# obeychoi0120/wseg

Measured on AMD Instinct MI355X. Metric: training images/sec at B=16x448x448 (contrast_train step), higher is better.
Workload: dtype bf16; 1 GPU; ResNet-38 contrast, synthetic VOC 448x448, B=16/GPU, procedural weights, dropout on, fused HIP loss; global_batch=16, parallelism=dp1, seed=0

## Files before the change

include/wseg_hip.h:

```cpp
#ifndef WSEG_HIP_H
#define WSEG_HIP_H
#include <stddef.h>
#include <stdint.h>
#ifdef __cplusplus
extern "C" {
#endif

#define WSEG_F32 0
#define WSEG_BF16 1
#define WSEG_F32X3 2

int wseg_version(void);
size_t wseg_sizeof_conv_desc(void);
size_t wseg_sizeof_wgrad_desc(void);
const char* wseg_last_error(void);

typedef struct wseg_conv_desc {
  const void* in;  const void* w;  void* out;  void* out2;
  const void* r_pre;  const void* r_post;  const void* mask;
  const float* scale;  const float* shift;  const float* drop;
  int32_t N, IH, IW, IC, ld_in;
  int32_t OH, OW, OC, ld_out, ld_out2;
  int32_t ld_rpre, ld_rpost, ld_mask;
  int32_t KH, KW, stride, dil, pad;
  int32_t mode, epi, dtype;
  int32_t relu_out2;
  int32_t relu_lt;
  int32_t bm_hint;
  int32_t IH2, IW2, OH2, OW2;
  const void* in2;
  int32_t ld_in2, IC2;
  int32_t w_rows;
} wseg_conv_desc;
int wseg_conv_igemm(const wseg_conv_desc* d, void* stream);

typedef struct wseg_wgrad_desc {
  const void* x;  const void* dy;  float* dw;
  int32_t N, IH, IW, IC, ld_x;
  int32_t OH, OW, OC, ld_dy;
  int32_t KH, KW, stride, dil, pad;
  int32_t dtype, split_k;
  int32_t IC_dw, OC_dw;
  int32_t tile_hint;
  int32_t IH2, IW2, OH2, OW2;
  int32_t dw_rot;
} wseg_wgrad_desc;
int wseg_conv_wgrad(const wseg_wgrad_desc* d, void* stream);

#define WSEG_CONV_64x128 1
#define WSEG_CONV_128x128 2
#define WSEG_CONV_224x256 3
#define WSEG_CONV_256x256 4
#define WSEG_CONV_512x128 5
#define WSEG_WGRAD_128x128 6
#define WSEG_WGRAD_256x256 7
typedef struct wseg_launch_plan {
  int32_t family;
  int32_t tile_rows, tile_cols;
  int32_t nwg;
  int32_t perm;
  int32_t tapf;
  int32_t nsplit;
  int32_t unit;
} wseg_launch_plan;
int wseg_conv_plan(const wseg_conv_desc* d, wseg_launch_plan* out);
int wseg_wgrad_plan(const wseg_wgrad_desc* d, wseg_launch_plan* out);

int wseg_conv_bwd_pair(const wseg_conv_desc* dg, const wseg_wgrad_desc* wg, void* stream);
int wseg_conv_bwd_pair_plan(const wseg_conv_desc* dg, const wseg_wgrad_desc* wg, wseg_launch_plan* dg_plan, wseg_launch_plan* wg_plan);

int wseg_pack_weights(const float* master, void* fwd, void* tr, int OC, int T, int IC,
                      int OCp, int ICp, int ic_rot, int dtype, void* stream);
int wseg_copy2d_batch(const void* src, void* dst, const long* table, int npieces, long total_chunks, void* stream);
int wseg_pack_transposed_batch(const float* master, void* out, const long* table, int nlayers, long total_tiles, int dtype, void* stream);
int wseg_pack_transposed_batch_bf16(const void* mirror, void* out, const long* table, int nlayers, long total_tiles, void* stream);
int wseg_dropout_scale(const float* u, float* out, long total, long split_at, float p0, float p1, void* stream);

int wseg_stem_conv(const float* x_nchw, const float* w ,
                   const float* scale, const float* shift, void* raw, void* act,
                   int N, int H, int W, int dtype, void* stream);
int wseg_stem_conv_kc(const float* x, const float* w_kc, const float* scale, const float* shift,
                      void* raw, void* act, int N, int H, int W, int dtype, void* stream);

int wseg_head_split(const void* head, int ld, int c0, float* cam_low, float* cmax, int N, int hw, int dtype, void* stream);
int wseg_cam_gate(const float* cam_low, const float* cmax, float* G, int N, int hw, void* stream);
int wseg_pcm_xs(const float* x_nchw, void* feat, int ld, int c_xs, int c_end, int N, int H, int W, int h, int w, int dtype, void* stream);
int wseg_head_grad_rows(const float* d_fproj, const float* d_cam_low, const void* head, void* d_head, int ld, int N, int hw, int dtype, void* stream);

int wseg_resize_planar_fwd(const float* in, float* out, const float* plane_mul, long planes, int ih, int iw, int oh, int ow, int align,
                           int flip_x, int accumulate, void* stream);
int wseg_resize_planar_bwd(const float* d_out, float* d_in, const float* plane_mul, const float* plane_add, long planes, int ih, int iw, int oh, int ow, int align, int accumulate, void* stream);

int wseg_infer_finish(const float* sum_cam, const float* stats, float alpha, float* norm_cam, unsigned char* pred, int npix, void* stream);

int wseg_l2norm_forward(const void* F, int ldf, float* Fh, float* nrm, long rows, int dtype, void* stream);
int wseg_l2norm_backward(const void* F, int ldf, const float* dFh, const float* nrm, void* dF, int lddf, long rows, int dtype, void* stream);
int wseg_pcm_forward(const float* Fh, const float* G, float* cam_rv, float* den, int N, int hw, void* stream);
int wseg_pcm_backward(const float* Fh, const float* G, const float* d_cam_rv, const float* cam_rv, const float* den,
                      float* DN, float* dFh, int N, int hw, void* stream);
int wseg_pack_x3(const float* src, void* dst, long numel, void* stream);
int wseg_split_bf16(const float* in, void* hi, void* lo, long total, void* stream);
int wseg_to_bf16(const float* in, void* out, long total, void* stream);
int wseg_pcm_forward_bf16(const void* Fb, const void* Gb, float* cam_rv, float* den, int N, int hw, void* stream);
int wseg_pcm_backward_bf16(const void* Fb, const void* Gb, const void* Gl, const float* d_cam_rv, const float* cam_rv, const float* den,
                           float* DN, void* DNb, void* DNl, float* dFh, int N, int hw, void* stream);

size_t wseg_plane_stats_workspace_bytes(long planes);
int wseg_plane_stats(const float* U, float* stats, long planes, int npix, void* workspace, void* stream);
int wseg_up_plane_stats(const float* low, float* stats, long planes, int h, int w, int S, const float* label20 , void* workspace, void* stream);
int wseg_up_rvmin_values(const float* low, const float* label20, float* q, unsigned char* argc, int N, int h, int w, int S, void* stream);
int wseg_up_norm_resize_forward(const float* low, const float* stats, const float* label20, float* out, int N, int h, int w, int S, int OS, void* stream);
int wseg_resize_adjoint_ones(float* wvec, int h, int S, void* stream);
int wseg_up_maps_backward(const float* G, const float* low, const float* stats, const float* label20, const float* plane_bias,
                          const float* wvec_y, const float* wvec_x, const float* q, const unsigned char* argc, const float* res,
                          int k, float coef, float* d_low, int N, int h, int w, int S, int OS, void* stream);
int wseg_cls_loss(const float* stats, const float* label20, float* loss_out, float* plane_bias, int N, int npix, float coef, void* stream);
size_t wseg_select_workspace_bytes(int rows);
int wseg_select_kth(const float* vals, int rows, int n, int k, int largest, int use_abs, int relu_vals, float* res, void* workspace, void* stream);
int wseg_select_finish(const float* res, int rows, int k, int relu_vals, float scale, float* loss_out, void* stream);
int wseg_loss_finish(const float* acc, float er_coef, float* out8, void* stream);
int wseg_er_ecr_prep(const float* c1, const float* c2, const float* r1, const float* r2, float* Gc1, float* Gc2, float* dlt1, float* dlt2,
                     float* er_sum, int N, int npix, float er_coef, void* stream);
int wseg_ecr_backward(const float* dlt, const float* res, float* Gr, int N, int per_row, int k, float coef, void* stream);
int wseg_rows_resize_forward(const void* head, int ld, float* F, int N, int ih, int iw, int oh, int ow, int dtype, void* stream);
int wseg_head_grad_fused(const float* dF, const float* d_cam_low, const void* head, void* d_head, int ld, int N, int ih, int iw, int oh, int ow, int dtype, void* stream);
int wseg_pseudo_label(const float* R, const float* label20, float bg_thr, int* y, float* ncam, int N, int npix, void* stream);
int wseg_proto_candidates(const float* ncam, const float* F, const int* tie_idx, float* cand_val, float* cand_feat, int* cand_const, int N, int npix, int K, void* stream);
int wseg_proto_merge(const float* cand_val, const float* cand_feat, const int* cand_const, float* protos, int world, int K,
                     long rank_stride , void* stream);
int wseg_intra_weights(const int* y, const float* S_own, int ld_s, const float* rkey, const unsigned char* rand_flag, float* w, int P, void* stream);
int wseg_intra_weights_global(const float* rec, float* w, int P, int ranks, int own_rank, float scale, long rank_stride, void* stream);

typedef struct {
  const float* F;
  const float* p_own;
  const float* p_oth;
  const int32_t* y_own;
  const int32_t* y_oth;
  const float* w_intra;
  const float* rkey;
  float* rec;
  float* dF;
} wseg_nce_view;
int wseg_nce_records(const wseg_nce_view* views, int nviews, int P, int split_bf16, void* stream);
int wseg_nce_fused(const wseg_nce_view* views, int nviews, int P, float coef_cross, float coef_intra, float* sums , void* stream);

typedef struct {
  const uint8_t* src; int32_t H, W;
  int32_t rh, rw;
  const int32_t* xb; const int32_t* xk; int32_t xks;
  const int32_t* yb; const int32_t* yk; int32_t yks;
  uint8_t* tmp; uint8_t* img;
  int32_t flip;
  int32_t op[4];
  float factor[4];
  int32_t hue_shift;
  int32_t cont_top, cont_left, img_top, img_left, ch, cw;
  float* out;
} wseg_aug_desc;
size_t wseg_sizeof_aug_desc(void);
int wseg_augment_batch(const wseg_aug_desc* descs_dev, int n, int max_pixels , const float* lut ,
                       int crop, unsigned long long* lum_sums , void* stream);

int wseg_sgd_step(float* params, const float* grads, float* momentum_buf, long numel,
                  const long* seg_begin, const long* seg_end, const float* seg_lr, const float* seg_wd, int nseg,
                  float momentum, float grad_scale, int first_step, void* bf16_mirror, void* stream);

#define WSEG_AFF_MAX_OFFSETS 64
#define WSEG_RW_MAX_PLANE 8192
int wseg_aff_num_offsets(int radius);
int wseg_aff_pairs(const void* feat, int ld, int C, float* aff, int N, int h, int w, int radius, int dtype, void* stream);
int wseg_aff_to_dense(const float* aff, float* dense, int h, int w, int radius, void* stream);
int wseg_rw_prepare(const float* aff, float* wgt, float* rsum, int N, int h, int w, int radius, int beta, void* stream);
int wseg_random_walk(const float* wgt, const float* rsum, const float* v_in, float* v_out, int N, int planes, int h, int w, int radius,
                     int logt, void* stream);
int wseg_rw_pool(const float* cams, const int* src, float bg, float* pooled, int H, int W, int dh, int dw, void* stream);
int wseg_rw_finish(const float* cam_rw, unsigned char* pred, int planes, int dh, int dw, int H, int W, void* stream);

long wseg_aff_loss_workspace_bytes(int N, int h, int w, int radius);
int wseg_aff_loss_forward(const void* feat, int ld, int C, const unsigned char* label, float* aff, void* workspace, float* out7, int N,
                          int h, int w, int radius, int dtype, void* stream);
int wseg_aff_loss_backward(const void* feat, int ld, int C, const unsigned char* label, const float* aff, const float* out7,
                           const float* gscale, float* d_feat, int ld_d, int N, int h, int w, int radius, int dtype, void* stream);

int wseg_elu_backward_rows(const void* g, int ld_g, int g_dtype, const void* y, int ld_y, int y_dtype, const float* gscale, void* dz,
                           int ld_dz, int dz_dtype, long M, int C, void* stream);

#define WSEG_CRF_PIX_ALIGN 128
#define WSEG_CRF_MAX_LABELS 32
#define WSEG_CRF_MAX_COLUMNS 64
#define WSEG_CRF_MAX_RADIUS 128
#define WSEG_CRF_BG_CONST 0
#define WSEG_CRF_BG_POWER 1
int wseg_crf_padded_pixels(int npix);
int wseg_crf_columns(int S, int n_labels);
int wseg_crf_labels(const float* cams, const int* src, int n_labels, int rule, float param, unsigned char* labels, int npix, void* stream);
int wseg_crf_prepare(const unsigned char* img, int H, int W, float gauss_sxy, float* feat, float* ones, float* ng, void* stream);
int wseg_crf_bilateral(const float* feat, const float* Qn, float* out, int npix, int ncols, float sxy, float srgb, void* stream);
int wseg_crf_rsqrt(const float* sums, int stride, float* n, int npix, void* stream);
int wseg_crf_gaussian(const float* in, float* tmp, float* out, int planes, int H, int W, float sxy, void* stream);
int wseg_crf_update(const unsigned char* labels, const float* outb, const float* outg, const float* nb, const float* ng, float* Qn,
                    float* Qg, float* Qout, float* logits, unsigned char* amax, int S, int n_labels, int npix, float gt_prob,
                    float w_bilateral, float w_gaussian, void* stream);

#ifdef __cplusplus
}
#endif
#endif
```

wseg_amd/_lib.py:

```python
import contextlib
import ctypes as C
import os

import torch

_HERE = os.path.dirname(os.path.abspath(__file__))
LIB_PATH = os.environ.get("WSEG_LIB") or os.path.join(_HERE, "libwseg_hip.so")

F32, BF16, F32X3 = 0, 1, 2
PROFILE_WGRAD = None
PROFILE = None
PROFILE_STRIDE = 1
_profile_idx = 0
_profile_phase = 0


def profile_begin_step(step):
    global _profile_idx, _profile_phase
    _profile_idx, _profile_phase = 0, step % max(1, PROFILE_STRIDE)


def _profile_sample():
    global _profile_idx
    i = _profile_idx
    _profile_idx += 1
    return (i + _profile_phase) % max(1, PROFILE_STRIDE) == 0, i
TORCH_DTYPE = {F32: torch.float32, BF16: torch.bfloat16, F32X3: torch.float32}


class ConvDesc(C.Structure):
    _fields_ = [("inp", C.c_void_p), ("w", C.c_void_p), ("out", C.c_void_p), ("out2", C.c_void_p),
                ("r_pre", C.c_void_p), ("r_post", C.c_void_p), ("mask", C.c_void_p),
                ("scale", C.c_void_p), ("shift", C.c_void_p), ("drop", C.c_void_p),
                ("N", C.c_int32), ("IH", C.c_int32), ("IW", C.c_int32), ("IC", C.c_int32), ("ld_in", C.c_int32),
                ("OH", C.c_int32), ("OW", C.c_int32), ("OC", C.c_int32), ("ld_out", C.c_int32), ("ld_out2", C.c_int32),
                ("ld_rpre", C.c_int32), ("ld_rpost", C.c_int32), ("ld_mask", C.c_int32),
                ("KH", C.c_int32), ("KW", C.c_int32), ("stride", C.c_int32), ("dil", C.c_int32), ("pad", C.c_int32),
                ("mode", C.c_int32), ("epi", C.c_int32), ("dtype", C.c_int32), ("relu_out2", C.c_int32),
                ("relu_lt", C.c_int32), ("bm_hint", C.c_int32),
                ("IH2", C.c_int32), ("IW2", C.c_int32), ("OH2", C.c_int32), ("OW2", C.c_int32),
                ("in2", C.c_void_p), ("ld_in2", C.c_int32), ("IC2", C.c_int32), ("w_rows", C.c_int32)]


class WgradDesc(C.Structure):
    _fields_ = [("x", C.c_void_p), ("dy", C.c_void_p), ("dw", C.c_void_p),
                ("N", C.c_int32), ("IH", C.c_int32), ("IW", C.c_int32), ("IC", C.c_int32), ("ld_x", C.c_int32),
                ("OH", C.c_int32), ("OW", C.c_int32), ("OC", C.c_int32), ("ld_dy", C.c_int32),
                ("KH", C.c_int32), ("KW", C.c_int32), ("stride", C.c_int32), ("dil", C.c_int32), ("pad", C.c_int32),
                ("dtype", C.c_int32), ("split_k", C.c_int32), ("IC_dw", C.c_int32), ("OC_dw", C.c_int32),
                ("tile_hint", C.c_int32),
                ("IH2", C.c_int32), ("IW2", C.c_int32), ("OH2", C.c_int32), ("OW2", C.c_int32), ("dw_rot", C.c_int32)]


def _load():
    if not os.path.exists(LIB_PATH):
        raise ImportError(
            f"{LIB_PATH} not found: build it with `python -c 'import __graft_entry__ as g; g.build()'` "
            "(wseg_amd has no CPU/eager fallback)")
    lib = C.CDLL(LIB_PATH)
    lib.wseg_last_error.restype = C.c_char_p
    lib.wseg_version.restype = C.c_int
    for fn in ("wseg_sizeof_conv_desc", "wseg_sizeof_wgrad_desc", "wseg_select_workspace_bytes", "wseg_plane_stats_workspace_bytes"):
        getattr(lib, fn).restype = C.c_size_t
    if lib.wseg_sizeof_conv_desc() != C.sizeof(ConvDesc) or lib.wseg_sizeof_wgrad_desc() != C.sizeof(WgradDesc):
        raise ImportError(f"{LIB_PATH} was built from another include/wseg_hip.h (descriptor sizes "
                          f"{lib.wseg_sizeof_conv_desc()}/{lib.wseg_sizeof_wgrad_desc()} vs {C.sizeof(ConvDesc)}/{C.sizeof(WgradDesc)}): rebuild it")
    return lib


lib = _load()


def _ptr(t):
    return t.data_ptr() if torch.is_tensor(t) else t


def stream_ptr():
    return torch.cuda.current_stream().cuda_stream


def check(status, what):
    if status != 0:
        raise RuntimeError(f"{what} failed ({status}): {lib.wseg_last_error().decode()}")


def _v(x):
    return C.c_void_p(_ptr(x))


def _s():
    return C.c_void_p(stream_ptr())


def _f(x):
    return C.c_float(x)


def _call(name, *args):
    check(getattr(lib, name)(*args, _s()), name)


def dtype_code(t):
    if t.dtype == torch.float32:
        return F32
    if t.dtype == torch.bfloat16:
        return BF16
    raise TypeError(f"unsupported dtype {t.dtype}")


def _flops_label(kind, *, N, IH, IW, IC, OH, OW, OC, KH, KW, stride=1, dil=1, seg2=None, mode=0, IC2=None, **_):
    oh, ow = (OH, OW) if mode == 0 else (IH, IW)
    pix = N * oh * ow
    if seg2 is not None:
        pix += N * (seg2[2] * seg2[3] if mode == 0 else seg2[0] * seg2[1])
    kin = IC * KH * KW + (IC2 or 0)
    return 2.0 * pix * kin * OC, f"{kind} {IC}{('+%d' % IC2) if IC2 else ''}->{OC} k{KH} s{stride} d{dil} {OH}x{OW}"


@contextlib.contextmanager
def _timed(sink, entry):
    if sink is None:
        yield
        return
    ev0, ev1 = torch.cuda.Event(enable_timing=True), torch.cuda.Event(enable_timing=True)
    ev0.record()
    yield
    ev1.record()
    sink.append((ev0, ev1) + tuple(entry()))


def conv_igemm(inp, w, out=None, out2=None, *, pair_wgrad=None, **kw):
    d = _conv_desc(inp, w, out, out2, **kw)
    ic2 = (d.IC2 or d.IC) if d.in2 else 0
    krow, wrows = d.KH * d.KW * d.IC + ic2, max(d.OC, d.w_rows)
    if w.numel() < wrows * krow:
        raise RuntimeError(f"conv_igemm: weight buffer has {w.numel()} elements, the launch reads {wrows} x {krow}")
    sampled, launch_idx = _profile_sample() if PROFILE is not None else (False, 0)

    def entry():
        kind = "fwd" if d.mode == 0 else ("dgrad+wgrad" if pair_wgrad is not None else "dgrad")
        flops, label = _flops_label(kind, **{**kw, "IC2": ic2})
        wflops = _flops_label("wgrad", **pair_wgrad[3])[0] if pair_wgrad is not None else 0.0
        return flops + wflops, label, launch_idx

    with _timed(PROFILE if sampled else None, entry):
        if pair_wgrad is not None:
            wx, wdy, wdw, wkw = pair_wgrad
            _call("wseg_conv_bwd_pair", C.byref(d), C.byref(_wgrad_desc(wx, wdy, wdw, **wkw)))
        else:
            _call("wseg_conv_igemm", C.byref(d))


def _conv_desc(inp, w, out, out2, *, N, IH, IW, IC, OH, OW, OC, KH, KW, stride=1, dil=1, pad=0,
               mode=0, epi=0, r_pre=None, r_post=None, mask=None, scale=None, shift=None, drop=None,
               ld_in=None, ld_out=None, ld_out2=None, ld_rpre=None, ld_rpost=None, ld_mask=None, relu_out2=1,
               relu_lt=0, bm_hint=0, seg2=None, in2=None, ld_in2=None, IC2=0, dtype=None, w_rows=0):
    d = ConvDesc()
    d.inp, d.w, d.out, d.out2 = _ptr(inp), _ptr(w), _ptr(out), _ptr(out2)
    d.r_pre, d.r_post, d.mask = _ptr(r_pre), _ptr(r_post), _ptr(mask)
    d.scale, d.shift, d.drop = _ptr(scale), _ptr(shift), _ptr(drop)
    d.N, d.IH, d.IW, d.IC, d.ld_in = N, IH, IW, IC, ld_in or IC
    d.OH, d.OW, d.OC, d.ld_out, d.ld_out2 = OH, OW, OC, ld_out or OC, ld_out2 or OC
    d.ld_rpre, d.ld_rpost, d.ld_mask = ld_rpre or OC, ld_rpost or OC, ld_mask or OC
    d.KH, d.KW, d.stride, d.dil, d.pad = KH, KW, stride, dil, pad
    d.mode, d.epi, d.dtype, d.relu_out2, d.relu_lt, d.bm_hint = mode, epi, (dtype_code(inp) if dtype is None else dtype), relu_out2, relu_lt, bm_hint
    if seg2 is not None:
        d.IH2, d.IW2, d.OH2, d.OW2 = seg2
    ic2 = (IC2 or IC) if in2 is not None else 0
    if in2 is not None:
        d.in2, d.IC2, d.ld_in2 = _ptr(in2), IC2, ld_in2 or ic2
    d.w_rows = w_rows
    return d


def _wgrad_desc(x, dy, dw, *, N, IH, IW, IC, OH, OW, OC, KH, KW, stride=1, dil=1, pad=0,
                ld_x=None, ld_dy=None, split_k=0, IC_dw=None, OC_dw=None, tile_hint=0, seg2=None, dtype=None, dw_rot=0):
    d = WgradDesc()
    d.x, d.dy, d.dw = _ptr(x), _ptr(dy), _ptr(dw)
    d.N, d.IH, d.IW, d.IC, d.ld_x = N, IH, IW, IC, ld_x or IC
    d.OH, d.OW, d.OC, d.ld_dy = OH, OW, OC, ld_dy or OC
    d.KH, d.KW, d.stride, d.dil, d.pad = KH, KW, stride, dil, pad
    d.dtype, d.split_k = (dtype_code(x) if dtype is None else dtype), split_k
    d.IC_dw, d.OC_dw, d.tile_hint = IC_dw or IC, OC_dw or OC, tile_hint
    d.dw_rot = dw_rot
    if seg2 is not None:
        d.IH2, d.IW2, d.OH2, d.OW2 = seg2
    assert not torch.is_tensor(dw) or dw.dtype == torch.float32
    return d


def conv_wgrad(x, dy, dw, **kw):
    d = _wgrad_desc(x, dy, dw, **kw)
    with _timed(PROFILE_WGRAD, lambda: _flops_label("wgrad", **kw)):
        _call("wseg_conv_wgrad", C.byref(d))


CONV_64x128, CONV_128x128, CONV_224x256, CONV_256x256, CONV_512x128, WGRAD_128x128, WGRAD_256x256 = range(1, 8)
_ANY = 64


class LaunchPlan(C.Structure):
    _fields_ = [(k, C.c_int32) for k in ("family", "tile_rows", "tile_cols", "nwg", "perm", "tapf", "nsplit", "unit")]

    def __repr__(self):
        return "LaunchPlan(" + ", ".join(f"{k}={getattr(self, k)}" for k, _t in self._fields_) + ")"


def _plan_dtype(t, dtype):
    return dtype if dtype is not None else (dtype_code(t) if torch.is_tensor(t) else BF16)


def conv_plan(inp=_ANY, w=_ANY, out=_ANY, out2=None, *, dtype=None, **kw):
    plan = LaunchPlan()
    check(lib.wseg_conv_plan(C.byref(_conv_desc(inp, w, out, out2, dtype=_plan_dtype(inp, dtype), **kw)), C.byref(plan)), "wseg_conv_plan")
    return plan


def wgrad_plan(x=_ANY, dy=_ANY, dw=_ANY, *, dtype=None, **kw):
    plan = LaunchPlan()
    check(lib.wseg_wgrad_plan(C.byref(_wgrad_desc(x, dy, dw, dtype=_plan_dtype(x, dtype), **kw)), C.byref(plan)), "wseg_wgrad_plan")
    return plan


def conv_pair_plan(wgrad_kw, inp=_ANY, w=_ANY, out=_ANY, out2=None, *, dtype=None, **kw):
    dg, wg = LaunchPlan(), LaunchPlan()
    dtype = _plan_dtype(inp, dtype)
    wdtype = dtype if wgrad_kw.get("dtype") is None else wgrad_kw["dtype"]
    fused = lib.wseg_conv_bwd_pair_plan(C.byref(_conv_desc(inp, w, out, out2, dtype=dtype, **kw)),
                                        C.byref(_wgrad_desc(_ANY, _ANY, _ANY, **{**wgrad_kw, "dtype": wdtype})), C.byref(dg), C.byref(wg))
    if fused < 0:
        check(fused, "wseg_conv_bwd_pair_plan")
    return fused, dg, wg


def pack_weights(master, fwd, tr, OC, T, IC, OCp, ICp, dtype, ic_rot=0):
    _call("wseg_pack_weights", _v(master), _v(fwd), _v(tr), OC, T, IC, OCp, ICp, ic_rot, dtype)


def copy2d_batch(src, dst, table, npieces, total_chunks):
    _call("wseg_copy2d_batch", _v(src), _v(dst), _v(table), npieces, C.c_long(total_chunks))


def pack_transposed_batch(master, out, table, nlayers, total_tiles, dtype):
    _call("wseg_pack_transposed_batch", _v(master), _v(out), _v(table), nlayers, C.c_long(total_tiles), dtype)


def pack_transposed_batch_bf16(mirror, out, table, nlayers, total_tiles):
    _call("wseg_pack_transposed_batch_bf16", _v(mirror), _v(out), _v(table), nlayers, C.c_long(total_tiles))


def dropout_scale(u, out, split_at, p0, p1):
    _call("wseg_dropout_scale", _v(u), _v(out), C.c_long(u.numel()), C.c_long(split_at), _f(p0), _f(p1))


def stem_conv_kc(x, w_kc, scale, shift, raw, act, N, H, W, dtype):
    if w_kc.numel() != 27 * 64 or w_kc.dtype != torch.float32:
        raise RuntimeError("stem_conv_kc: weights must be f32 [27][64]")
    _call("wseg_stem_conv_kc", _v(x), _v(w_kc), _v(scale), _v(shift), _v(raw), _v(act), N, H, W, dtype)


def stem_conv(x, w, scale, shift, raw, act, N, H, W, dtype):
    _call("wseg_stem_conv", _v(x), _v(w), _v(scale), _v(shift), _v(raw), _v(act), N, H, W, dtype)


def head_split(head, ld, c0, cam_low, cmax, N, hw):
    check(lib.wseg_head_split(_v(head), ld, c0, _v(cam_low), _v(cmax), N, hw, dtype_code(head), _s()), "wseg_head_split")


def cam_gate(cam_low, cmax, G, N, hw):
    check(lib.wseg_cam_gate(_v(cam_low), _v(cmax), _v(G), N, hw, _s()), "wseg_cam_gate")


def pcm_xs(x, feat, ld, c_xs, c_end, N, H, W, h, w):
    check(lib.wseg_pcm_xs(_v(x), _v(feat), ld, c_xs, c_end, N, H, W, h, w, dtype_code(feat), _s()), "wseg_pcm_xs")


def head_grad_rows(d_fproj, d_cam_low, head, d_head, ld, N, hw):
    check(lib.wseg_head_grad_rows(_v(d_fproj), _v(d_cam_low), _v(head), _v(d_head), ld, N, hw, dtype_code(head), _s()), "wseg_head_grad_rows")


def resize_planar_fwd(inp, out, planes, ih, iw, oh, ow, align, plane_mul=None, flip_x=False, accumulate=False):
    check(lib.wseg_resize_planar_fwd(_v(inp), _v(out), _v(plane_mul), C.c_long(planes), ih, iw, oh, ow, int(align), int(flip_x), int(accumulate), _s()), "wseg_resize_planar_fwd")


def infer_finish(sum_cam, stats, alpha, norm_cam, pred, npix):
    check(lib.wseg_infer_finish(_v(sum_cam), _v(stats), C.c_float(alpha), _v(norm_cam), _v(pred), npix, _s()), "wseg_infer_finish")


def resize_planar_bwd(d_out, d_in, planes, ih, iw, oh, ow, align, accumulate=False, plane_mul=None, plane_add=None):
    check(lib.wseg_resize_planar_bwd(_v(d_out), _v(d_in), _v(plane_mul), _v(plane_add), C.c_long(planes), ih, iw, oh, ow, int(align), int(accumulate), _s()), "wseg_resize_planar_bwd")


def l2norm_forward(F, ldf, Fh, nrm, rows):
    check(lib.wseg_l2norm_forward(_v(F), ldf, _v(Fh), _v(nrm), C.c_long(rows), dtype_code(F), _s()), "wseg_l2norm_forward")


def l2norm_backward(F, ldf, dFh, nrm, dF, lddf, rows):
    check(lib.wseg_l2norm_backward(_v(F), ldf, _v(dFh), _v(nrm), _v(dF), lddf, C.c_long(rows), dtype_code(F), _s()), "wseg_l2norm_backward")


def pcm_forward(Fh, G, cam_rv, den, N, hw):
    check(lib.wseg_pcm_forward(_v(Fh), _v(G), _v(cam_rv), _v(den), N, hw, _s()), "wseg_pcm_forward")


def pcm_backward(Fh, G, d_cam_rv, cam_rv, den, DN, dFh, N, hw):
    check(lib.wseg_pcm_backward(_v(Fh), _v(G), _v(d_cam_rv), _v(cam_rv), _v(den), _v(DN), _v(dFh), N, hw, _s()), "wseg_pcm_backward")


def sgd_step(params, grads, buf, segs, momentum, grad_scale, first_step, bf16_mirror=None):
    n = len(segs)
    LongArr, FloatArr = C.c_long * n, C.c_float * n
    b = LongArr(*[s[0] for s in segs]); e = LongArr(*[s[1] for s in segs])
    lr = FloatArr(*[s[2] for s in segs]); wd = FloatArr(*[s[3] for s in segs])
    check(lib.wseg_sgd_step(_v(params), _v(grads), _v(buf), C.c_long(params.numel()), b, e, lr, wd, n,
                            C.c_float(momentum), C.c_float(grad_scale), int(first_step), _v(bf16_mirror), _s()), "wseg_sgd_step")


def plane_stats(U, stats, planes, npix):
    ws = torch.empty(int(lib.wseg_plane_stats_workspace_bytes(C.c_long(planes))), device=U.device, dtype=torch.uint8)
    _call("wseg_plane_stats", _v(U), _v(stats), C.c_long(planes), npix, _v(ws))
def cls_loss(stats, label20, loss_out, plane_bias, N, npix, coef): _call("wseg_cls_loss", _v(stats), _v(label20), _v(loss_out), _v(plane_bias), N, npix, _f(coef))
def select_workspace_bytes(rows): return int(lib.wseg_select_workspace_bytes(rows))
def select_kth(vals, rows, n, k, largest, use_abs, relu_vals, res, ws): _call("wseg_select_kth", _v(vals), rows, n, k, int(largest), int(use_abs), int(relu_vals), _v(res), _v(ws))
def loss_finish(acc, er_coef, out8): _call("wseg_loss_finish", _v(acc), _f(er_coef), _v(out8))
def select_finish(res, rows, k, relu_vals, scale, loss_out): _call("wseg_select_finish", _v(res), rows, k, int(relu_vals), _f(scale), _v(loss_out))
def er_ecr_prep(c1, c2, r1, r2, Gc1, Gc2, dlt1, dlt2, er_sum, N, npix, er_coef): _call("wseg_er_ecr_prep", _v(c1), _v(c2), _v(r1), _v(r2), _v(Gc1), _v(Gc2), _v(dlt1), _v(dlt2), _v(er_sum), N, npix, _f(er_coef))
def ecr_backward(dlt, res, Gr, N, per_row, k, coef): _call("wseg_ecr_backward", _v(dlt), _v(res), _v(Gr), N, per_row, k, _f(coef))
def rows_resize_forward(head, ld, F, N, ih, iw, oh, ow): _call("wseg_rows_resize_forward", _v(head), ld, _v(F), N, ih, iw, oh, ow, dtype_code(head))
def head_grad_fused(dF, d_cam_low, head, d_head, ld, N, ih, iw, oh, ow): _call("wseg_head_grad_fused", _v(dF), _v(d_cam_low), _v(head), _v(d_head), ld, N, ih, iw, oh, ow, dtype_code(head))
def pseudo_label(R, label20, bg_thr, y, ncam, N, npix): _call("wseg_pseudo_label", _v(R), _v(label20), _f(bg_thr), _v(y), _v(ncam), N, npix)
def proto_candidates(ncam, F, tie_idx, cand_val, cand_feat, cand_const, N, npix, K): _call("wseg_proto_candidates", _v(ncam), _v(F), _v(tie_idx), _v(cand_val), _v(cand_feat), _v(cand_const), N, npix, K)
def proto_merge(cand_val, cand_feat, cand_const, protos, world, K, rank_stride=0): _call("wseg_proto_merge", _v(cand_val), _v(cand_feat), _v(cand_const), _v(protos), world, K, C.c_long(rank_stride))
def intra_weights(y, S_own, rkey, rand_flag, w, P, ld_s=21): _call("wseg_intra_weights", _v(y), _v(S_own), ld_s, _v(rkey), _v(rand_flag), _v(w), P)
def intra_weights_global(rec, w, P, ranks, own_rank, scale, rank_stride): _call("wseg_intra_weights_global", _v(rec), _v(w), P, ranks, own_rank, _f(scale), C.c_long(rank_stride))


class NceView(C.Structure):
    _fields_ = [("F", C.c_void_p), ("p_own", C.c_void_p), ("p_oth", C.c_void_p), ("y_own", C.c_void_p), ("y_oth", C.c_void_p),
                ("w_intra", C.c_void_p), ("rkey", C.c_void_p), ("rec", C.c_void_p), ("dF", C.c_void_p)]


def _nce_views(views):
    arr = (NceView * len(views))()
    for i, v in enumerate(views):
        for k, _t in NceView._fields_:
            setattr(arr[i], k, _ptr(v.get(k)))
    return arr


def nce_records(views, P, split_bf16=False):
    _call("wseg_nce_records", _nce_views(views), len(views), P, int(split_bf16))


def nce_fused(views, P, coef_cross, coef_intra, sums):
    _call("wseg_nce_fused", _nce_views(views), len(views), P, _f(coef_cross), _f(coef_intra), _v(sums))


def up_plane_stats(low, stats, planes, h, w, S, label20=None):
    ws = torch.empty(int(lib.wseg_plane_stats_workspace_bytes(C.c_long(planes))), device=low.device, dtype=torch.uint8)
    _call("wseg_up_plane_stats", _v(low), _v(stats), C.c_long(planes), h, w, S, _v(label20), _v(ws))
def up_rvmin_values(low, label20, q, argc, N, h, w, S): _call("wseg_up_rvmin_values", _v(low), _v(label20), _v(q), _v(argc), N, h, w, S)
def up_norm_resize_forward(low, stats, label20, out, N, h, w, S, OS): _call("wseg_up_norm_resize_forward", _v(low), _v(stats), _v(label20), _v(out), N, h, w, S, OS)
def resize_adjoint_ones(wvec, h, S): _call("wseg_resize_adjoint_ones", _v(wvec), h, S)
def up_maps_backward(G, low, stats, label20, plane_bias, wvec_y, wvec_x, q, argc, res, k, coef, d_low, N, h, w, S, OS):
    _call("wseg_up_maps_backward", _v(G), _v(low), _v(stats), _v(label20), _v(plane_bias), _v(wvec_y), _v(wvec_x), _v(q), _v(argc), _v(res),
          k, _f(coef), _v(d_low), N, h, w, S, OS)


def gemm256_probe(A, B, Cout, M, N, K, variant=0):
    if not hasattr(lib, "wseg_gemm256_probe"):
        raise RuntimeError("wseg_gemm256_probe is a development probe: rebuild with `WSEG_PROBES=1 bash wseg_amd/csrc/build.sh`")
    check(lib.wseg_gemm256_probe(_v(A), _v(B), _v(Cout), M, N, K, variant, _s()), "wseg_gemm256_probe")


def debug_stamps(n_wg):
    if not hasattr(lib, "wseg_debug_stamps"):
        raise RuntimeError("wseg_debug_stamps exists in probe builds only: rebuild with `WSEG_PROBES=1 bash wseg_amd/csrc/build.sh`")
    import numpy as np
    torch.cuda.synchronize()
    buf = np.zeros((min(n_wg, 4096), 24), dtype=np.uint64)
    lib.wseg_debug_stamps.argtypes = [C.c_void_p, C.c_size_t]
    check(lib.wseg_debug_stamps(buf.ctypes.data_as(C.c_void_p), C.c_size_t(buf.nbytes)), "wseg_debug_stamps")
    return buf


def debug_set_diag(v):
    if not hasattr(lib, "wseg_debug_set_diag"):
        raise RuntimeError("wseg_debug_set_diag exists in probe builds only")
    check(lib.wseg_debug_set_diag(int(v)), "wseg_debug_set_diag")


def to_bf16(inp, out): _call("wseg_to_bf16", _v(inp), _v(out), C.c_long(inp.numel()))
def split_bf16(inp, hi, lo): _call("wseg_split_bf16", _v(inp), _v(hi), _v(lo), C.c_long(inp.numel()))
def pack_x3(src, dst): _call("wseg_pack_x3", _v(src), _v(dst), C.c_long(src.numel()))
def pcm_forward_bf16(Fb, Gb, cam_rv, den, N, hw): _call("wseg_pcm_forward_bf16", _v(Fb), _v(Gb), _v(cam_rv), _v(den), N, hw)
def pcm_backward_bf16(Fb, Gb, Gl, d_cam_rv, cam_rv, den, DN, DNb, DNl, dFh, N, hw): _call("wseg_pcm_backward_bf16", _v(Fb), _v(Gb), _v(Gl), _v(d_cam_rv), _v(cam_rv), _v(den), _v(DN), _v(DNb), _v(DNl), _v(dFh), N, hw)


RW_MAX_PLANE = 8192


def aff_num_offsets(radius): return int(lib.wseg_aff_num_offsets(radius))
def aff_pairs(feat, ld, C_, aff, N, h, w, radius): _call("wseg_aff_pairs", _v(feat), ld, C_, _v(aff), N, h, w, radius, dtype_code(feat))
def aff_to_dense(aff, dense, h, w, radius): _call("wseg_aff_to_dense", _v(aff), _v(dense), h, w, radius)
def rw_prepare(aff, wgt, rsum, N, h, w, radius, beta): _call("wseg_rw_prepare", _v(aff), _v(wgt), _v(rsum), N, h, w, radius, int(beta))
def random_walk(wgt, rsum, v_in, v_out, N, planes, h, w, radius, logt):
    _call("wseg_random_walk", _v(wgt), _v(rsum), _v(v_in), _v(v_out), N, planes, h, w, radius, int(logt))
def rw_pool(cams, src, bg, pooled, H, W, dh, dw):
    _call("wseg_rw_pool", _v(cams), (C.c_int * 21)(*[int(s) for s in src]), _f(bg), _v(pooled), H, W, dh, dw)
def rw_finish(cam_rw, pred, planes, dh, dw, H, W): _call("wseg_rw_finish", _v(cam_rw), _v(pred), planes, dh, dw, H, W)



lib.wseg_aff_loss_workspace_bytes.restype = C.c_long


def aff_loss_workspace_bytes(N, h, w, radius): return int(lib.wseg_aff_loss_workspace_bytes(N, h, w, radius))
def aff_loss_forward(feat, ld, C_, label, aff, ws, out7, N, h, w, radius, dtype=None):
    _call("wseg_aff_loss_forward", _v(feat), ld, C_, _v(label), _v(aff), _v(ws), _v(out7), N, h, w, radius, dtype_code(feat) if dtype is None else dtype)
def aff_loss_backward(feat, ld, C_, label, aff, out7, gscale, d_feat, ld_d, N, h, w, radius, dtype=None):
    _call("wseg_aff_loss_backward", _v(feat), ld, C_, _v(label), _v(aff), _v(out7), _v(gscale), _v(d_feat), ld_d, N, h, w, radius,
          dtype_code(feat) if dtype is None else dtype)


def elu_backward_rows(g, ld_g, y, ld_y, gscale, dz, ld_dz, M, C_):
    for name, t_, ld in (("g", g, ld_g), ("y", y, ld_y), ("dz", dz, ld_dz)):
        if t_.numel() < (M - 1) * ld + C_:
            raise RuntimeError(f"elu_backward_rows: {name} has {t_.numel()} elements, {M} rows of ld {ld} with {C_} columns need {(M - 1) * ld + C_}")
    _call("wseg_elu_backward_rows", _v(g), ld_g, dtype_code(g), _v(y), ld_y, dtype_code(y), _v(gscale), _v(dz), ld_dz, dtype_code(dz), C.c_long(M), C_)


CRF_PIX_ALIGN, CRF_MAX_LABELS, CRF_MAX_COLUMNS = 128, 32, 64
CRF_BG_CONST, CRF_BG_POWER = 0, 1


def crf_padded_pixels(npix): return int(lib.wseg_crf_padded_pixels(int(npix)))
def crf_columns(S, n_labels): return int(lib.wseg_crf_columns(int(S), int(n_labels)))
def crf_labels(cams, src, n_labels, rule, param, labels, npix):
    _call("wseg_crf_labels", _v(cams), (C.c_int * n_labels)(*[int(s) for s in src]), n_labels, int(rule), _f(param), _v(labels), npix)
def crf_prepare(img, H, W, gauss_sxy, feat, ones, ng): _call("wseg_crf_prepare", _v(img), H, W, _f(gauss_sxy), _v(feat), _v(ones), _v(ng))
def crf_bilateral(feat, Qn, out, npix, ncols, sxy, srgb): _call("wseg_crf_bilateral", _v(feat), _v(Qn), _v(out), npix, ncols, _f(sxy), _f(srgb))
def crf_rsqrt(sums, stride, n, npix): _call("wseg_crf_rsqrt", _v(sums), stride, _v(n), npix)
def crf_gaussian(inp, tmp, out, planes, H, W, sxy): _call("wseg_crf_gaussian", _v(inp), _v(tmp), _v(out), planes, H, W, _f(sxy))
def crf_update(labels, outb, outg, nb, ng, Qn, Qg, Qout, logits, amax, S, n_labels, npix, gt_prob, w_bilateral, w_gaussian):
    _call("wseg_crf_update", _v(labels), _v(outb), _v(outg), _v(nb), _v(ng), _v(Qn), _v(Qg), _v(Qout), _v(logits), _v(amax), S, n_labels, npix,
          _f(gt_prob), _f(w_bilateral), _f(w_gaussian))
```

wseg_amd/csrc/loss.hip:

```cpp
#include <algorithm>
#include "loss_helpers.h"

namespace {

__global__ void cls_loss_kernel(const float* __restrict__ stats, const float* __restrict__ label20, float* __restrict__ loss_out,
                                float* __restrict__ plane_bias, int N, int npix, float coef) {
  __shared__ float red[4];
  float acc = 0.f;
  for (int i = threadIdx.x; i < N * 21; i += blockDim.x) {
    const int n = i / 21, c = i - n * 21;
    float bias = 0.f;
    if (c >= 1) {
      const float z = stats[(size_t)i * 6 + 2] / npix;
      const float y = label20[n * 20 + c - 1];
      const float l1p = log1pf(expf(-fabsf(z)));
      const float ls_p = fminf(z, 0.f) - l1p, ls_n = fminf(-z, 0.f) - l1p;
      acc += -(y * ls_p + (1.f - y) * ls_n);
      const float sg = 1.f / (1.f + expf(-z));
      bias = coef * (sg - y) / (20.f * N) / npix;
    }
    plane_bias[i] = bias;
  }
  const float tot = block_sum(acc, red);
  if (threadIdx.x == 0) atomicAdd(loss_out, tot / (20.f * N));
}

__global__ __launch_bounds__(256) void select_hist_kernel(const float* __restrict__ vals, int n, int use_abs, const unsigned* __restrict__ state,
                                                          unsigned* __restrict__ hist, int shift) {
  __shared__ unsigned h[4][256];
  const int row = blockIdx.y, wv = threadIdx.x >> 6;
#pragma unroll
  for (int w = 0; w < 4; ++w) h[w][threadIdx.x] = 0;
  __syncthreads();
  const unsigned prefix = state[row * 4 + 0], mask = state[row * 4 + 1];
  const float* v = vals + (size_t)row * n;
  auto count = [&](float f) {
    if (use_abs) f = fabsf(f);
    const unsigned k = f2key(f);
    if ((k & mask) == prefix) atomicAdd(&h[wv][(k >> shift) & 255u], 1u);
  };
  if ((n & 3) == 0) {
    const float4* v4 = reinterpret_cast<const float4*>(v);
    for (int i = blockIdx.x * 256 + threadIdx.x; i < (n >> 2); i += gridDim.x * 256) {
      const float4 q = v4[i];
      count(q.x); count(q.y); count(q.z); count(q.w);
    }
  } else {
    for (int i = blockIdx.x * 256 + threadIdx.x; i < n; i += gridDim.x * 256) count(v[i]);
  }
  __syncthreads();
  const unsigned t = h[0][threadIdx.x] + h[1][threadIdx.x] + h[2][threadIdx.x] + h[3][threadIdx.x];
  if (t) atomicAdd(&hist[row * 256 + threadIdx.x], t);
}
__global__ __launch_bounds__(64) void select_scan_kernel(unsigned* __restrict__ state, unsigned* __restrict__ hist, int shift, int rows) {
  const int row = blockIdx.x, lane = threadIdx.x;
  if (row >= rows) return;
  const unsigned k = state[row * 4 + 2];
  uint4* hrow = reinterpret_cast<uint4*>(hist + (size_t)row * 256);
  const uint4 c = hrow[lane];
  const unsigned s = c.x + c.y + c.z + c.w;
  unsigned inc = s;
#pragma unroll
  for (int o = 1; o < 64; o <<= 1) {
    const unsigned t = __shfl_up(inc, o, 64);
    if (lane >= o) inc += t;
  }
  const unsigned exc = inc - s;
  const unsigned total = __shfl(inc, 63, 64);
  hrow[lane] = make_uint4(0u, 0u, 0u, 0u);
  int b = -1; unsigned cum = exc;
  if (exc < k && inc >= k) {
    const unsigned cs[4] = {c.x, c.y, c.z, c.w};
#pragma unroll
    for (int j = 0; j < 4; ++j) {
      if (b < 0) { if (cum + cs[j] >= k) b = lane * 4 + j; else cum += cs[j]; }
    }
  } else if (lane == 63 && total < k) {
    b = 255; cum = total;
  }
  if (b >= 0) {
    state[row * 4 + 0] |= ((unsigned)b << shift);
    state[row * 4 + 1] |= (255u << shift);
    state[row * 4 + 2] = k - cum;
  }
}
__global__ void select_init_kernel(unsigned* __restrict__ state, unsigned* __restrict__ hist, int rows, unsigned rank_small, float* __restrict__ res) {
  const int i = blockIdx.x * blockDim.x + threadIdx.x;
  if (i < rows) { state[i * 4 + 0] = 0; state[i * 4 + 1] = 0; state[i * 4 + 2] = rank_small; state[i * 4 + 3] = 0; }
  if (i < rows * 4) res[i] = 0.f;
  if (i < rows * 256) hist[i] = 0;
}
__global__ __launch_bounds__(256) void select_sum_kernel(const float* __restrict__ vals, int n, int use_abs, int largest, int relu_vals,
                                                         const unsigned* __restrict__ state, float* __restrict__ res) {
  __shared__ float red[4];
  const int row = blockIdx.y;
  const float thr = key2f(state[row * 4 + 0]);
  const float* v = vals + (size_t)row * n;
  float s = 0.f, cs = 0.f, ce = 0.f;
  auto take = [&](float f) {
    if (use_abs) f = fabsf(f);
    const bool beyond = largest ? (f > thr) : (f < thr);
    if (beyond) { s += relu_vals ? fmaxf(f, 0.f) : f; cs += 1.f; }
    else if (f == thr) ce += 1.f;
  };
  if ((n & 3) == 0) {
    const float4* v4 = reinterpret_cast<const float4*>(v);
    for (int i = blockIdx.x * 256 + threadIdx.x; i < (n >> 2); i += gridDim.x * 256) {
      const float4 q = v4[i];
      take(q.x); take(q.y); take(q.z); take(q.w);
    }
  } else {
    for (int i = blockIdx.x * 256 + threadIdx.x; i < n; i += gridDim.x * 256) take(v[i]);
  }
  const float S = block_sum(s, red), CS = block_sum(cs, red), CE = block_sum(ce, red);
  if (threadIdx.x == 0) {
    if (blockIdx.x == 0) res[row * 4 + 0] = thr;
    atomicAdd(&res[row * 4 + 1], S); atomicAdd(&res[row * 4 + 2], CS); atomicAdd(&res[row * 4 + 3], CE);
  }
}
__global__ void select_finish_kernel(const float* __restrict__ res, int rows, int k, int relu_vals, float scale, float* __restrict__ loss_out) {
  if (threadIdx.x == 0 && blockIdx.x == 0) {
    float t = 0.f;
    for (int r = 0; r < rows; ++r) {
      const float thr = relu_vals ? fmaxf(res[r * 4 + 0], 0.f) : res[r * 4 + 0];
      t += res[r * 4 + 1] + ((float)k - res[r * 4 + 2]) * thr;
    }
    atomicAdd(loss_out, t * scale);
  }
}

__global__ void er_ecr_prep_kernel(const float* __restrict__ c1, const float* __restrict__ c2, const float* __restrict__ r1,
                                   const float* __restrict__ r2, float* __restrict__ Gc1, float* __restrict__ Gc2,
                                   float* __restrict__ dlt1, float* __restrict__ dlt2, float* __restrict__ er_out,
                                   int npix, float er_coef, long total) {
  __shared__ float red[4];
  const long idx = (long)blockIdx.x * blockDim.x + threadIdx.x;
  float er = 0.f;
  if (idx < total) {
    const long n = idx / npix; const int p = (int)(idx - n * npix);
    const size_t base = (size_t)n * 21 * npix + p;
    float a[21], b[21];
    float m1 = -INFINITY, m2 = -INFINITY;
    for (int c = 1; c < 21; ++c) {
      a[c] = c1[base + (size_t)c * npix]; b[c] = c2[base + (size_t)c * npix];
      m1 = fmaxf(m1, a[c]); m2 = fmaxf(m2, b[c]);
      const float df = a[c] - b[c];
      er += fabsf(df);
      const float sg = df > 0.f ? 1.f : (df < 0.f ? -1.f : 0.f);
      Gc1[base + (size_t)c * npix] = sg * er_coef;
      Gc2[base + (size_t)c * npix] = -sg * er_coef;
    }
    Gc1[base] = 0.f; Gc2[base] = 0.f;
    a[0] = 1.f - m1; b[0] = 1.f - m2;
    for (int c = 0; c < 21; ++c) {
      const float oh2 = (c == 0 || b[c] == m2) ? b[c] : 0.f;
      const float oh1 = (c == 0 || a[c] == m1) ? a[c] : 0.f;
      dlt1[base + (size_t)c * npix] = r1[base + (size_t)c * npix] - oh2;
      dlt2[base + (size_t)c * npix] = r2[base + (size_t)c * npix] - oh1;
    }
  }
  const float t = block_sum(er, red);
  if (threadIdx.x == 0 && t != 0.f) atomicAdd(er_out, t);
}

__global__ void ecr_bwd_kernel(const float* __restrict__ dlt, const float* __restrict__ res, float* __restrict__ Gr, int per_row, int k, float coef, long total) {
  const long idx = (long)blockIdx.x * blockDim.x + threadIdx.x;
  if (idx >= total) return;
  const long row = idx / per_row;
  const float d = dlt[idx], v = fabsf(d), thr = res[row * 4 + 0];
  float w = 0.f;
  if (v > thr) w = 1.f;
  else if (v == thr) { const float ce = res[row * 4 + 3]; w = ce > 0.f ? ((float)k - res[row * 4 + 2]) / ce : 0.f; }
  const float sg = d > 0.f ? 1.f : (d < 0.f ? -1.f : 0.f);
  Gr[idx] = w * sg * coef;
}

template <int DT>
__global__ void rows_resize_fwd_kernel(const void* __restrict__ head, int ld, float* __restrict__ F, int ih, int iw, int oh, int ow, long total) {
  const long idx = (long)blockIdx.x * blockDim.x + threadIdx.x;
  if (idx >= total) return;
  const int ch = (int)(idx & 127); const long pix = idx >> 7;
  const int ox = (int)(pix % ow); const long r = pix / ow;
  const int oy = (int)(r % oh); const long n = r / oh;
  int y0, y1, x0, x1; float fy, fx;
  src_index(oy, ac_scale(ih, oh), ih, y0, y1, fy); src_index(ox, ac_scale(iw, ow), iw, x0, x1, fx);
  auto f = [&](int y, int x) { return elem<DT>::ld(head, (((size_t)n * ih + y) * iw + x) * ld + ch); };
  F[idx] = (1.f - fy) * ((1.f - fx) * f(y0, x0) + fx * f(y0, x1)) + fy * ((1.f - fx) * f(y1, x0) + fx * f(y1, x1));
}

template <int DT>
__global__ void head_grad_fused_kernel(const float* __restrict__ dF, const float* __restrict__ d_cam, const void* __restrict__ head,
                                       void* __restrict__ d_head, int ld, int ih, int iw, int oh, int ow, long total) {
  const long idx = (long)blockIdx.x * blockDim.x + threadIdx.x;
  if (idx >= total) return;
  const int v8 = ld / 8;
  const long pix = idx / v8; const int c8 = (int)(idx - pix * v8) * 8;
  const int x = (int)(pix % iw); const long r = pix / iw;
  const int y = (int)(r % ih); const long n = r / ih;
  float o[8];
#pragma unroll
  for (int e = 0; e < 8; ++e) o[e] = 0.f;
  if (c8 < 128) {
    const float sy = ac_scale(ih, oh), sx = ac_scale(iw, ow);
    int oy_lo, oy_hi, ox_lo, ox_hi;
    if (sy > 0.f) { oy_lo = max(0, (int)floorf((y - 1) / sy) - 1); oy_hi = min(oh - 1, (int)ceilf((y + 1) / sy) + 1); } else { oy_lo = 0; oy_hi = oh - 1; }
    if (sx > 0.f) { ox_lo = max(0, (int)floorf((x - 1) / sx) - 1); ox_hi = min(ow - 1, (int)ceilf((x + 1) / sx) + 1); } else { ox_lo = 0; ox_hi = ow - 1; }
    for (int oy = oy_lo; oy <= oy_hi; ++oy) {
      int y0, y1; float fy;
      src_index(oy, sy, ih, y0, y1, fy);
      const float wy = (y == y0 ? 1.f - fy : 0.f) + (y == y1 ? fy : 0.f);
      if (wy == 0.f) continue;
      for (int ox = ox_lo; ox <= ox_hi; ++ox) {
        int x0, x1; float fx;
        src_index(ox, sx, iw, x0, x1, fx);
        const float w = wy * ((x == x0 ? 1.f - fx : 0.f) + (x == x1 ? fx : 0.f));
        if (w == 0.f) continue;
        const float4* g = reinterpret_cast<const float4*>(dF + ((((size_t)n * oh + oy) * ow + ox) << 7) + c8);
        const float4 g0 = g[0], g1 = g[1];
        o[0] += w * g0.x; o[1] += w * g0.y; o[2] += w * g0.z; o[3] += w * g0.w;
        o[4] += w * g1.x; o[5] += w * g1.y; o[6] += w * g1.z; o[7] += w * g1.w;
      }
    }
    float hv[8];
    load8<DT>(head, (size_t)pix * ld + c8, hv);
#pragma unroll
    for (int e = 0; e < 8; ++e) if (!(hv[e] > 0.f)) o[e] = 0.f;
  } else if (c8 < 152 && d_cam) {
#pragma unroll
    for (int e = 0; e < 8; ++e) {
      const int c = c8 + e - 128;
      if (c < 21) o[e] = d_cam[(((size_t)n * 21 + c) * ih + y) * iw + x];
    }
  }
  store8<DT>(d_head, (size_t)pix * ld + c8, o);
}

__global__ __launch_bounds__(256) void pseudo_label_kernel(const float* __restrict__ R, const float* __restrict__ label20, float bg_thr,
                                                           int* __restrict__ y, float* __restrict__ ncam, int npix) {
  __shared__ float s_mx[21], s_mn[21];
  __shared__ float red_a[256], red_b[256];
  const int n = blockIdx.x, tid = threadIdx.x;
  const float* Rn = R + (size_t)n * 21 * npix;
  for (int c = 0; c < 21; ++c) {
    float mx = 0.f, mn = INFINITY;
    for (int p = tid; p < npix; p += 256) { const float v = fmaxf(Rn[(size_t)c * npix + p], 0.f); mx = fmaxf(mx, v); mn = fminf(mn, v); }
    red_a[tid] = mx; red_b[tid] = mn;
    __syncthreads();
    for (int o = 128; o > 0; o >>= 1) { if (tid < o) { red_a[tid] = fmaxf(red_a[tid], red_a[tid + o]); red_b[tid] = fminf(red_b[tid], red_b[tid + o]); } __syncthreads(); }
    if (tid == 0) { s_mx[c] = red_a[0]; s_mn[c] = red_b[0]; }
    __syncthreads();
  }
  for (int p = tid; p < npix; p += 256) {
    float best = -INFINITY; int bc = 0;
    for (int c = 0; c < 21; ++c) {
      float v = fmaxf(Rn[(size_t)c * npix + p], 0.f);
      if (v < s_mn[c] + 1e-5f) v = 0.f;
      v = (v - s_mn[c] - 1e-5f) / (s_mx[c] - s_mn[c] + 1e-5f);
      if (c == 0) v = bg_thr;
      ncam[((size_t)n * 21 + c) * npix + p] = v;
      const float L = c == 0 ? 1.f : label20[n * 20 + c - 1];
      const float s = v * L;
      if (s > best) { best = s; bc = c; }
    }
    y[(size_t)n * npix + p] = bc;
  }
}

__global__ __launch_bounds__(256) void proto_candidates_kernel(const float* __restrict__ ncam, const float* __restrict__ F, const int* __restrict__ tie_idx,
                                                               float* __restrict__ cand_val, float* __restrict__ cand_feat, int* __restrict__ cand_const,
                                                               int N, int npix, int K) {
  extern __shared__ float sv[];
  __shared__ float r_v[256]; __shared__ int r_i[256];
  __shared__ int sel[64];
  __shared__ float s_gmin;
  const int c = blockIdx.x, tid = threadIdx.x;
  const int P = N * npix;
  float lmx = -INFINITY, lmn = INFINITY;
  for (int p = tid; p < P; p += 256) {
    const int n = p / npix, pix = p - n * npix;
    float v = ncam[((size_t)n * 21 + c) * npix + pix];
    if (v != v) v = -INFINITY;
    sv[p] = v; lmx = fmaxf(lmx, v); lmn = fminf(lmn, v);
  }
  r_v[tid] = lmx; __syncthreads();
  for (int o = 128; o > 0; o >>= 1) { if (tid < o) r_v[tid] = fmaxf(r_v[tid], r_v[tid + o]); __syncthreads(); }
  const float gmx = r_v[0]; __syncthreads();
  r_v[tid] = lmn; __syncthreads();
  for (int o = 128; o > 0; o >>= 1) { if (tid < o) r_v[tid] = fminf(r_v[tid], r_v[tid + o]); __syncthreads(); }
  if (tid == 0) s_gmin = r_v[0];
  __syncthreads();
  const bool is_const = (gmx == s_gmin);
  if (is_const) {
    if (tid < K) sel[tid] = min(max(tie_idx[tid], 0), P - 1);
    __syncthreads();
  } else {
    for (int k = 0; k < K; ++k) {
      float bv = -INFINITY; int bi = 0x7fffffff;
      for (int p = tid; p < P; p += 256) { const float v = sv[p]; if (v > bv || (v == bv && p < bi)) { bv = v; bi = p; } }
#pragma unroll
      for (int o = 32; o > 0; o >>= 1) {
        const float ov = __shfl_xor(bv, o, 64); const int oi = __shfl_xor(bi, o, 64);
        if (ov > bv || (ov == bv && oi < bi)) { bv = ov; bi = oi; }
      }
      if ((tid & 63) == 0) { r_v[tid >> 6] = bv; r_i[tid >> 6] = bi; }
      __syncthreads();
      if (tid == 0) {
#pragma unroll
        for (int w = 1; w < 4; ++w) if (r_v[w] > bv || (r_v[w] == bv && r_i[w] < bi)) { bv = r_v[w]; bi = r_i[w]; }
        if (bi >= P) bi = 0;
        sel[k] = bi; sv[bi] = NAN;
      }
      __syncthreads();
    }
  }
  if (tid == 0) cand_const[c] = is_const ? 1 : 0;
  for (int k = 0; k < K; ++k) {
    const int p = sel[k];
    const int n = p / npix, pix = p - n * npix;
    if (tid == 0) cand_val[c * K + k] = ncam[((size_t)n * 21 + c) * npix + pix];
    if (tid < 128) cand_feat[((size_t)c * K + k) * 128 + tid] = F[(size_t)p * 128 + tid];
  }
}
__global__ __launch_bounds__(128) void proto_merge_kernel(const float* __restrict__ cand_val, const float* __restrict__ cand_feat, const int* __restrict__ cand_const,
                                                          float* __restrict__ protos, int world, int K, long rs_val, long rs_feat, long rs_const) {
  __shared__ float vals[512]; __shared__ int order[64]; __shared__ float red[2]; __shared__ int cst_s;
  const int c = blockIdx.x, tid = threadIdx.x;
  const int M = world * K;
  for (int i = tid; i < M; i += 128) {
    const int w = i / K, k = i - w * K;
    const float v = cand_val[(size_t)w * rs_val + c * K + k];
    vals[i] = v != v ? -INFINITY : v;
  }
  if (tid < K) order[tid] = tid;
  if (tid == 0) {
    bool cst = true;
    for (int w = 0; w < world; ++w) cst = cst && cand_const[(size_t)w * rs_const + c];
    cst_s = cst ? 1 : 0;
  }
  __syncthreads();
  if (!cst_s) {
    for (int i = tid; i < M; i += 128) {
      const float v = vals[i];
      int r = 0;
      for (int j = 0; j < M; ++j) { const float u = vals[j]; r += (u > v || (u == v && j < i)) ? 1 : 0; }
      if (r < K) order[r] = i;
    }
  }
  __syncthreads();
  float acc = 0.f, wsum = 0.f;
  for (int k = 0; k < K; ++k) {
    const int i = order[k]; const int w = i / K, kk = i - w * K;
    const float v = cand_val[(size_t)w * rs_val + c * K + kk];
    acc += v * cand_feat[(size_t)w * rs_feat + ((size_t)c * K + kk) * 128 + tid];
    wsum += v;
  }
  const float pr = acc / wsum;
  const float ss = block_sum(pr * pr, red);
  protos[c * 128 + tid] = pr / fmaxf(sqrtf(ss), 1e-12f);
}

}

#define GRID1(total) dim3((unsigned)(((total) + 255) / 256)), dim3(256)
#define ST ((hipStream_t)stream)

extern "C" int wseg_cls_loss(const float* stats, const float* label20, float* loss_out, float* plane_bias, int N, int npix, float coef, void* stream) {
  WSEG_CHECK(stats && label20 && loss_out && plane_bias && N > 0, "cls_loss: bad arguments");
  hipLaunchKernelGGL(cls_loss_kernel, dim3(1), dim3(256), 0, ST, stats, label20, loss_out, plane_bias, N, npix, coef);
  WSEG_LAUNCH_CHECK();
  return 0;
}

extern "C" size_t wseg_select_workspace_bytes(int rows) { return (size_t)rows * (4 + 256) * sizeof(unsigned); }
extern "C" int wseg_select_kth(const float* vals, int rows, int n, int k, int largest, int use_abs, int relu_vals,
                               float* res, void* workspace, void* stream) {
  WSEG_CHECK(vals && res && workspace && rows > 0 && n > 0 && k >= 1 && k <= n, "select_kth: bad arguments (rows=%d n=%d k=%d)", rows, n, k);
  unsigned* state = (unsigned*)workspace;
  unsigned* hist = state + (size_t)rows * 4;
  const unsigned rank_small = largest ? (unsigned)(n - k + 1) : (unsigned)k;
  hipLaunchKernelGGL(select_init_kernel, dim3((rows * 256 + 255) / 256), dim3(256), 0, ST, state, hist, rows, rank_small, res);
  const int gx = std::max(1, std::min(128, (n + 4095) / 4096));
  const int gs = std::max(1, std::min(32, (n + 8191) / 8192));
  for (int shift = 24; shift >= 0; shift -= 8) {
    hipLaunchKernelGGL(select_hist_kernel, dim3(gx, rows), dim3(256), 0, ST, vals, n, use_abs, state, hist, shift);
    hipLaunchKernelGGL(select_scan_kernel, dim3(rows), dim3(64), 0, ST, state, hist, shift, rows);
  }
  hipLaunchKernelGGL(select_sum_kernel, dim3(gs, rows), dim3(256), 0, ST, vals, n, use_abs, largest, relu_vals, state, res);
  WSEG_LAUNCH_CHECK();
  return 0;
}
extern "C" int wseg_select_finish(const float* res, int rows, int k, int relu_vals, float scale, float* loss_out, void* stream) {
  WSEG_CHECK(res && loss_out && rows > 0, "select_finish: bad arguments");
  hipLaunchKernelGGL(select_finish_kernel, dim3(1), dim3(64), 0, ST, res, rows, k, relu_vals, scale, loss_out);
  WSEG_LAUNCH_CHECK();
  return 0;
}

static __global__ void loss_finish_kernel(const float* __restrict__ acc, float er_coef, float* __restrict__ out) {
  if (threadIdx.x != 0) return;
  const float cls = acc[0] * 0.5f + acc[1], er = acc[2] * er_coef, ecr = acc[3], nce = acc[4] + acc[5] + acc[6];
  out[0] = cls + er + ecr + nce; out[1] = cls; out[2] = er; out[3] = ecr; out[4] = nce; out[5] = acc[6]; out[6] = acc[4]; out[7] = acc[5];
}
extern "C" int wseg_loss_finish(const float* acc, float er_coef, float* out8, void* stream) {
  WSEG_CHECK(acc && out8, "loss_finish: bad arguments");
  hipLaunchKernelGGL(loss_finish_kernel, dim3(1), dim3(64), 0, ST, acc, er_coef, out8);
  WSEG_LAUNCH_CHECK();
  return 0;
}

extern "C" int wseg_er_ecr_prep(const float* c1, const float* c2, const float* r1, const float* r2, float* Gc1, float* Gc2,
                                float* dlt1, float* dlt2, float* er_sum, int N, int npix, float er_coef, void* stream) {
  WSEG_CHECK(c1 && c2 && r1 && r2 && Gc1 && Gc2 && dlt1 && dlt2 && er_sum, "er_ecr_prep: bad arguments");
  const long total = (long)N * npix;
  hipLaunchKernelGGL(er_ecr_prep_kernel, GRID1(total), 0, ST, c1, c2, r1, r2, Gc1, Gc2, dlt1, dlt2, er_sum, npix, er_coef, total);
  WSEG_LAUNCH_CHECK();
  return 0;
}
extern "C" int wseg_ecr_backward(const float* dlt, const float* res, float* Gr, int N, int per_row, int k, float coef, void* stream) {
  WSEG_CHECK(dlt && res && Gr, "ecr_backward: bad arguments");
  const long total = (long)N * per_row;
  hipLaunchKernelGGL(ecr_bwd_kernel, GRID1(total), 0, ST, dlt, res, Gr, per_row, k, coef, total);
  WSEG_LAUNCH_CHECK();
  return 0;
}

extern "C" int wseg_rows_resize_forward(const void* head, int ld, float* F, int N, int ih, int iw, int oh, int ow, int dtype, void* stream) {
  WSEG_CHECK(head && F && ld >= 128, "rows_resize_forward: bad arguments");
  const long total = (long)N * oh * ow * 128;
  if (dtype == WSEG_BF16) hipLaunchKernelGGL(rows_resize_fwd_kernel<WSEG_BF16>, GRID1(total), 0, ST, head, ld, F, ih, iw, oh, ow, total);
  else hipLaunchKernelGGL(rows_resize_fwd_kernel<WSEG_F32>, GRID1(total), 0, ST, head, ld, F, ih, iw, oh, ow, total);
  WSEG_LAUNCH_CHECK();
  return 0;
}
extern "C" int wseg_head_grad_fused(const float* dF, const float* d_cam_low, const void* head, void* d_head, int ld,
                                    int N, int ih, int iw, int oh, int ow, int dtype, void* stream) {
  WSEG_CHECK(dF && head && d_head && ld % 8 == 0 && ld >= 152, "head_grad_fused: bad arguments");
  const long total = (long)N * ih * iw * (ld / 8);
  if (dtype == WSEG_BF16) hipLaunchKernelGGL(head_grad_fused_kernel<WSEG_BF16>, GRID1(total), 0, ST, dF, d_cam_low, head, d_head, ld, ih, iw, oh, ow, total);
  else hipLaunchKernelGGL(head_grad_fused_kernel<WSEG_F32>, GRID1(total), 0, ST, dF, d_cam_low, head, d_head, ld, ih, iw, oh, ow, total);
  WSEG_LAUNCH_CHECK();
  return 0;
}

extern "C" int wseg_pseudo_label(const float* R, const float* label20, float bg_thr, int* y, float* ncam, int N, int npix, void* stream) {
  WSEG_CHECK(R && label20 && y && ncam && N > 0 && npix > 0, "pseudo_label: bad arguments");
  hipLaunchKernelGGL(pseudo_label_kernel, dim3(N), dim3(256), 0, ST, R, label20, bg_thr, y, ncam, npix);
  WSEG_LAUNCH_CHECK();
  return 0;
}
extern "C" int wseg_proto_candidates(const float* ncam, const float* F, const int* tie_idx, float* cand_val, float* cand_feat, int* cand_const,
                                     int N, int npix, int K, void* stream) {
  WSEG_CHECK(ncam && F && tie_idx && cand_val && cand_feat && cand_const && K >= 1 && K <= 64, "proto_candidates: bad arguments");
  const size_t P = (size_t)N * npix;
  WSEG_CHECK(P * 4 <= 128 * 1024 && (size_t)K <= P, "proto_candidates: P=%zu too large for one workgroup's LDS", P);
  hipLaunchKernelGGL(proto_candidates_kernel, dim3(21), dim3(256), P * 4, ST, ncam, F, tie_idx, cand_val, cand_feat, cand_const, N, npix, K);
  WSEG_LAUNCH_CHECK();
  return 0;
}
extern "C" int wseg_proto_merge(const float* cand_val, const float* cand_feat, const int* cand_const, float* protos, int world, int K,
                                long rank_stride, void* stream) {
  WSEG_CHECK(cand_val && cand_feat && cand_const && protos && world >= 1 && world * K <= 512 && K <= 64, "proto_merge: bad arguments");
  const long rv = rank_stride ? rank_stride : 21L * K, rf = rank_stride ? rank_stride : 21L * K * 128, rc = rank_stride ? rank_stride : 21L;
  hipLaunchKernelGGL(proto_merge_kernel, dim3(21), dim3(128), 0, ST, cand_val, cand_feat, cand_const, protos, world, K, rv, rf, rc);
  WSEG_LAUNCH_CHECK();
  return 0;
}
```

wseg_amd/csrc/maps.hip:

```cpp
#include <algorithm>
#include "loss_helpers.h"

namespace {

__device__ __forceinline__ float up_value(const float* __restrict__ p, int w, int y0, int y1, int x0, int x1, float fy, float fx) {
  const float a = __fmaf_rn(fx, p[y0 * w + x1], __fmul_rn(1.f - fx, p[y0 * w + x0]));
  const float b = __fmaf_rn(fx, p[y1 * w + x1], __fmul_rn(1.f - fx, p[y1 * w + x0]));
  return __fmaf_rn(fy, b, __fmul_rn(1.f - fy, a));
}
__device__ __forceinline__ float up_at(const float* __restrict__ p, int h, int w, float sy, float sx, int oy, int ox) {
  int y0, y1, x0, x1; float fy, fx;
  src_index(oy, sy, h, y0, y1, fy); src_index(ox, sx, w, x0, x1, fx);
  return up_value(p, w, y0, y1, x0, x1, fy, fx);
}
__device__ __forceinline__ int threads_per_row(int S) { return S > 128 ? 256 : (S > 64 ? 128 : 64); }

__global__ __launch_bounds__(256) void plane_stats_partial_kernel(const float* __restrict__ U, unsigned long long* __restrict__ kmax,
                                                                  unsigned long long* __restrict__ kmin, float* __restrict__ ksum,
                                                                  int npix, int chunks) {
  __shared__ unsigned long long s_mx[256], s_mn[256];
  __shared__ float s_sum[256];
  const int pl = blockIdx.x / chunks, ck = blockIdx.x - pl * chunks, tid = threadIdx.x;
  const float* p = U + (size_t)pl * npix;
  const int per = (npix + chunks - 1) / chunks;
  const int i0 = ck * per, i1 = min(npix, i0 + per);
  unsigned long long mx = 0ull, mn = ~0ull;
  float sum = 0.f;
  for (int i = i0 + tid; i < i1; i += 256) {
    const float u = p[i];
    const unsigned rb = __float_as_uint(fmaxf(u, 0.f));
    sum += u;
    const unsigned long long a = ((unsigned long long)rb << 32) | (unsigned)(~i), b = ((unsigned long long)rb << 32) | (unsigned)i;
    mx = a > mx ? a : mx; mn = b < mn ? b : mn;
  }
  s_mx[tid] = mx; s_mn[tid] = mn; s_sum[tid] = sum;
  __syncthreads();
  for (int o = 128; o > 0; o >>= 1) {
    if (tid < o) {
      if (s_mx[tid + o] > s_mx[tid]) s_mx[tid] = s_mx[tid + o];
      if (s_mn[tid + o] < s_mn[tid]) s_mn[tid] = s_mn[tid + o];
      s_sum[tid] += s_sum[tid + o];
    }
    __syncthreads();
  }
  if (tid == 0) { atomicMax(&kmax[pl], s_mx[0]); atomicMin(&kmin[pl], s_mn[0]); atomicAdd(&ksum[pl], s_sum[0]); }
}

__global__ __launch_bounds__(256) void up_stats_partial_kernel(const float* __restrict__ low, unsigned long long* __restrict__ kmax,
                                                              unsigned long long* __restrict__ kmin, float* __restrict__ ksum,
                                                              int h, int w, int S, int chunks, const float* __restrict__ label20) {
  __shared__ unsigned long long s_mx[256], s_mn[256];
  __shared__ float s_sum[256];
  const int pl = blockIdx.x / chunks, ck = blockIdx.x - pl * chunks, tid = threadIdx.x;
  if (label20) {
    const int c = pl % 21;
    if (c >= 1 && label20[(pl / 21) * 20 + c - 1] == 0.f) return;
  }
  const float* p = low + (size_t)pl * h * w;
  const float sy = ac_scale(h, S), sx = ac_scale(w, S);
  const int per = (S + chunks - 1) / chunks;
  const int r0 = ck * per, r1 = min(S, r0 + per);
  const int tpr = threads_per_row(S), rpi = 256 / tpr;
  const int tr = tid / tpr, tx = tid & (tpr - 1);
  constexpr int MAXC = 4;
  int x0[MAXC], x1[MAXC]; float fx[MAXC], ra[MAXC], rb[MAXC];
  int nc = 0;
  for (int ox = tx; ox < S && nc < MAXC; ox += tpr, ++nc) src_index(ox, sx, w, x0[nc], x1[nc], fx[nc]);
  unsigned mxv = 0u, mxi = 0u, mnv = 0xFFFFFFFFu, mni = 0xFFFFFFFFu;
  bool any = false;
  float sum = 0.f;
  int cy0 = -1, cy1 = -1;
  for (int oy = r0 + tr; oy < r1; oy += rpi) {
    int y0, y1; float fy;
    src_index(oy, sy, h, y0, y1, fy);
    if (y0 != cy0 || y1 != cy1) {
#pragma unroll
      for (int j = 0; j < MAXC; ++j)
        if (j < nc) {
          ra[j] = (y0 == cy1) ? rb[j] : __fmaf_rn(fx[j], p[y0 * w + x1[j]], __fmul_rn(1.f - fx[j], p[y0 * w + x0[j]]));
          rb[j] = (y1 == y0) ? ra[j] : __fmaf_rn(fx[j], p[y1 * w + x1[j]], __fmul_rn(1.f - fx[j], p[y1 * w + x0[j]]));
        }
      cy0 = y0; cy1 = y1;
    }
#pragma unroll
    for (int j = 0; j < MAXC; ++j)
      if (j < nc) {
        const float u = __fmaf_rn(fy, rb[j], __fmul_rn(1.f - fy, ra[j]));
        const unsigned i = (unsigned)(oy * S + tx + j * tpr);
        const unsigned vb = __float_as_uint(fmaxf(u, 0.f));
        sum += u;
        if (!any || vb > mxv) { mxv = vb; mxi = i; }
        if (!any || vb < mnv) { mnv = vb; mni = i; }
        any = true;
      }
  }
  for (int oy = r0 + tr; oy < r1; oy += rpi) {
    int y0, y1; float fy;
    src_index(oy, sy, h, y0, y1, fy);
    for (int ox = tx + MAXC * tpr; ox < S; ox += tpr) {
      int xa, xb; float f;
      src_index(ox, sx, w, xa, xb, f);
      const float u = up_value(p, w, y0, y1, xa, xb, fy, f);
      const unsigned i = (unsigned)(oy * S + ox);
      const unsigned vb = __float_as_uint(fmaxf(u, 0.f));
      sum += u;
      if (!any || vb > mxv || (vb == mxv && i < mxi)) { mxv = vb; mxi = i; }
      if (!any || vb < mnv || (vb == mnv && i < mni)) { mnv = vb; mni = i; }
      any = true;
    }
  }
  s_mx[tid] = any ? (((unsigned long long)mxv << 32) | (unsigned)(~mxi)) : 0ull;
  s_mn[tid] = any ? (((unsigned long long)mnv << 32) | mni) : ~0ull;
  s_sum[tid] = sum;
  __syncthreads();
  for (int o = 128; o > 0; o >>= 1) {
    if (tid < o) {
      if (s_mx[tid + o] > s_mx[tid]) s_mx[tid] = s_mx[tid + o];
      if (s_mn[tid + o] < s_mn[tid]) s_mn[tid] = s_mn[tid + o];
      s_sum[tid] += s_sum[tid + o];
    }
    __syncthreads();
  }
  if (tid == 0) { atomicMax(&kmax[pl], s_mx[0]); atomicMin(&kmin[pl], s_mn[0]); atomicAdd(&ksum[pl], s_sum[0]); }
}
__global__ void up_stats_init_kernel(unsigned long long* __restrict__ kmax, unsigned long long* __restrict__ kmin, float* __restrict__ ksum, long planes) {
  const long pl = (long)blockIdx.x * blockDim.x + threadIdx.x;
  if (pl < planes) { kmax[pl] = 0ull; kmin[pl] = ~0ull; ksum[pl] = 0.f; }
}
__global__ void up_stats_final_kernel(const unsigned long long* __restrict__ kmax, const unsigned long long* __restrict__ kmin,
                                      const float* __restrict__ ksum, float* __restrict__ stats, long planes) {
  const long pl = (long)blockIdx.x * blockDim.x + threadIdx.x;
  if (pl >= planes) return;
  float* o = stats + pl * 6;
  o[0] = __uint_as_float((unsigned)(kmax[pl] >> 32)); o[1] = __uint_as_float((unsigned)(kmin[pl] >> 32)); o[2] = ksum[pl];
  o[3] = __int_as_float((int)(~(unsigned)(kmax[pl] & 0xFFFFFFFFull))); o[4] = __int_as_float((int)(unsigned)(kmin[pl] & 0xFFFFFFFFull)); o[5] = 0.f;
}

__global__ __launch_bounds__(256) void up_rvmin_values_kernel(const float* __restrict__ low, const float* __restrict__ label20,
                                                             float* __restrict__ q, unsigned char* __restrict__ argc,
                                                             int h, int w, int S, int rows_per_block) {
  const int n = blockIdx.y, tid = threadIdx.x;
  const float sy = ac_scale(h, S), sx = ac_scale(w, S);
  const int r0 = blockIdx.x * rows_per_block, r1 = min(S, r0 + rows_per_block);
  const int tpr = threads_per_row(S), rpi = 256 / tpr;
  const int tr = tid / tpr, tx = tid & (tpr - 1);
  const float* lab = label20 + n * 20;
  for (int oy = r0 + tr; oy < r1; oy += rpi) {
    int y0, y1; float fy;
    src_index(oy, sy, h, y0, y1, fy);
    for (int ox = tx; ox < S; ox += tpr) {
      int x0, x1; float fx;
      src_index(ox, sx, w, x0, x1, fx);
      float best = -INFINITY; int bc = 1;
      for (int c = 1; c < 21; ++c) {
        const float L = lab[c - 1];
        float v = 0.f;
        if (L != 0.f) v = up_value(low + ((size_t)n * 21 + c) * h * w, w, y0, y1, x0, x1, fy, fx) * L;
        if (v > best) { best = v; bc = c; }
      }
      const size_t idx = (size_t)n * S * S + (size_t)oy * S + ox;
      q[idx] = best; argc[idx] = (unsigned char)bc;
    }
  }
}

__global__ void up_norm_resize_fwd_kernel(const float* __restrict__ low, const float* __restrict__ stats, const float* __restrict__ label20,
                                          float* __restrict__ out, int h, int w, int S, int OS, long total) {
  const long idx = (long)blockIdx.x * blockDim.x + threadIdx.x;
  if (idx >= total) return;
  const int ox = (int)(idx % OS); const long r = idx / OS;
  const int oy = (int)(r % OS); const long pl = r / OS;
  const int c = (int)(pl % 21); const long n = pl / 21;
  const float L = c == 0 ? 1.f : label20[n * 20 + c - 1];
  float v = 0.f;
  if (L != 0.f) {
    const float mx = stats[pl * 6 + 0], mn = stats[pl * 6 + 1];
    const float invD = 1.f / (mx - mn + 1e-5f);
    int y0, y1, x0, x1; float fy, fx;
    const float sc = ac_scale(S, OS);
    src_index(oy, sc, S, y0, y1, fy); src_index(ox, sc, S, x0, x1, fx);
    const float* p = low + (size_t)pl * h * w;
    const float sy = ac_scale(h, S), sx = ac_scale(w, S);
    auto f = [&](int y, int x) { return fmaxf(fmaxf(up_at(p, h, w, sy, sx, y, x), 0.f) - mn - 1e-5f, 0.f) * invD; };
    v = (1.f - fy) * ((1.f - fx) * f(y0, x0) + fx * f(y0, x1)) + fy * ((1.f - fx) * f(y1, x0) + fx * f(y1, x1));
    v *= L;
  }
  out[idx] = v;
}

__global__ void resize_adjoint_ones_kernel(float* __restrict__ wvec, int h, int S) {
  const int y = blockIdx.x * blockDim.x + threadIdx.x;
  if (y >= h) return;
  const float sc = ac_scale(h, S);
  float acc = 0.f;
  for (int o = 0; o < S; ++o) {
    int y0, y1; float f;
    src_index(o, sc, h, y0, y1, f);
    acc += (y == y0 ? 1.f - f : 0.f) + (y == y1 ? f : 0.f);
  }
  wvec[y] = acc;
}

__global__ __launch_bounds__(256) void up_maps_bwd_kernel(const float* __restrict__ G, const float* __restrict__ low, const float* __restrict__ stats,
                                                         const float* __restrict__ label20, const float* __restrict__ plane_bias,
                                                         const float* __restrict__ wvec_y, const float* __restrict__ wvec_x,
                                                         const float* __restrict__ q, const unsigned char* __restrict__ argc,
                                                         const float* __restrict__ res, int k, float coef,
                                                         float* __restrict__ d_low, int h, int w, int S, int OS, int chunks) {
  extern __shared__ float dl[];
  __shared__ float red[4];
  const int pl = blockIdx.x / chunks, ck = blockIdx.x - pl * chunks, tid = threadIdx.x;
  const int c = pl % 21; const int n = pl / 21;
  const float L = c == 0 ? 1.f : label20[n * 20 + c - 1];
  const float bias = (plane_bias && ck == 0) ? plane_bias[pl] : 0.f;
  const bool do_norm = L != 0.f && G != nullptr, do_sel = q != nullptr && c >= 1 && L != 0.f;
  if (!do_norm && !do_sel && bias == 0.f) return;
  const float* p = low + (size_t)pl * h * w;
  const float sy = ac_scale(h, S), sx = ac_scale(w, S);
  for (int i = tid; i < h * w; i += 256) dl[i] = 0.f;
  __syncthreads();
  auto scatter = [&](int oy, int ox, float t) {
    int y0, y1, x0, x1; float fy, fx;
    src_index(oy, sy, h, y0, y1, fy); src_index(ox, sx, w, x0, x1, fx);
    atomicAdd(&dl[y0 * w + x0], t * (1.f - fy) * (1.f - fx));
    atomicAdd(&dl[y0 * w + x1], t * (1.f - fy) * fx);
    atomicAdd(&dl[y1 * w + x0], t * fy * (1.f - fx));
    atomicAdd(&dl[y1 * w + x1], t * fy * fx);
  };
  if (do_norm) {
    const float mx = stats[(size_t)pl * 6 + 0], mn = stats[(size_t)pl * 6 + 1];
    const float invD = 1.f / (mx - mn + 1e-5f);
    const float sc = ac_scale(S, OS);
    const float* g = G + (size_t)pl * OS * OS;
    const int per = (OS * OS + chunks - 1) / chunks;
    const int o_end = min(OS * OS, (ck + 1) * per);
    float A = 0.f, B = 0.f;
    for (int o = ck * per + tid; o < o_end; o += 256) {
      const float go = g[o] * L;
      if (go == 0.f) continue;
      const int oy = o / OS, ox = o - oy * OS;
      int y0, y1, x0, x1; float fy, fx;
      src_index(oy, sc, S, y0, y1, fy); src_index(ox, sc, S, x0, x1, fx);
      const int ys[2] = {y0, y1}, xs[2] = {x0, x1};
      const float wy[2] = {1.f - fy, fy}, wx[2] = {1.f - fx, fx};
#pragma unroll
      for (int a = 0; a < 2; ++a)
#pragma unroll
        for (int b = 0; b < 2; ++b) {
          const float wgt = wy[a] * wx[b];
          if (wgt == 0.f) continue;
          const float u = up_at(p, h, w, sy, sx, ys[a], xs[b]);
          const float av = fmaxf(fmaxf(u, 0.f) - mn - 1e-5f, 0.f);
          if (av > 0.f) {
            const float t = go * wgt * invD;
            scatter(ys[a], xs[b], t);
            B += t;
            A += t * av * invD;
          }
        }
    }
    const float At = block_sum(A, red), Bt = block_sum(B, red);
    if (tid == 0) {
      const int imx = __float_as_int(stats[(size_t)pl * 6 + 3]), imn = __float_as_int(stats[(size_t)pl * 6 + 4]);
      const int ymx = imx / S, xmx = imx - ymx * S, ymn = imn / S, xmn = imn - ymn * S;
      if (up_at(p, h, w, sy, sx, ymx, xmx) > 0.f) scatter(ymx, xmx, -At);
      if (up_at(p, h, w, sy, sx, ymn, xmn) > 0.f) scatter(ymn, xmn, At - Bt);
    }
  }
  if (do_sel) {
    const float thr = res[n * 4 + 0];
    const float ce = res[n * 4 + 3];
    const float wtie = ce > 0.f ? ((float)k - res[n * 4 + 2]) / ce : 0.f;
    const float* qn = q + (size_t)n * S * S;
    const unsigned char* an = argc + (size_t)n * S * S;
    const float val = coef * L;
    const int npix = S * S;
    const int per = ((npix + chunks - 1) / chunks + 3) & ~3;
    const int i_end = min(npix, (ck + 1) * per);
    auto one = [&](int i, unsigned char ac, float v) {
      if (ac != (unsigned char)c) return;
      float wsel = 0.f;
      if (v < thr) wsel = 1.f; else if (v == thr) wsel = wtie;
      if (wsel > 0.f && v > 0.f) { const int oy = i / S; scatter(oy, i - oy * S, wsel * val); }
    };
    if ((npix & 3) == 0) {
      for (int i = ck * per + tid * 4; i < i_end; i += 1024) {
        const unsigned a4 = *reinterpret_cast<const unsigned*>(an + i);
        const unsigned cc = (unsigned)c;
        if (((a4 & 255u) != cc) && (((a4 >> 8) & 255u) != cc) && (((a4 >> 16) & 255u) != cc) && ((a4 >> 24) != cc)) continue;
        const float4 v4 = *reinterpret_cast<const float4*>(qn + i);
        one(i, (unsigned char)(a4 & 255u), v4.x); one(i + 1, (unsigned char)((a4 >> 8) & 255u), v4.y);
        one(i + 2, (unsigned char)((a4 >> 16) & 255u), v4.z); one(i + 3, (unsigned char)(a4 >> 24), v4.w);
      }
    } else {
      for (int i = ck * per + tid; i < i_end; i += 256) one(i, an[i], qn[i]);
    }
  }
  __syncthreads();
  float* o = d_low + (size_t)pl * h * w;
  for (int i = tid; i < h * w; i += 256) {
    const int y = i / w;
    const float v = dl[i] + (bias != 0.f ? bias * wvec_y[y] * wvec_x[i - y * w] : 0.f);
    if (v != 0.f) atomicAdd(&o[i], v);
  }
}

}

#define GRID1(total) dim3((unsigned)(((total) + 255) / 256)), dim3(256)
#define ST ((hipStream_t)stream)

extern "C" size_t wseg_plane_stats_workspace_bytes(long planes) { return (size_t)planes * 24; }
extern "C" int wseg_plane_stats(const float* U, float* stats, long planes, int npix, void* workspace, void* stream) {
  WSEG_CHECK(U && stats && workspace && planes > 0 && npix > 0, "plane_stats: bad arguments");
  unsigned long long* kmax = (unsigned long long*)workspace;
  unsigned long long* kmin = kmax + planes;
  float* ksum = (float*)(kmin + planes);
  (void)hipMemsetAsync(kmax, 0x00, sizeof(unsigned long long) * planes, ST);
  (void)hipMemsetAsync(kmin, 0xFF, sizeof(unsigned long long) * planes, ST);
  (void)hipMemsetAsync(ksum, 0x00, sizeof(float) * planes, ST);
  const int chunks = std::max(1, std::min(std::min(64, (int)((long)npix / 8192)), (int)std::max(1L, 2048 / planes)));
  hipLaunchKernelGGL(plane_stats_partial_kernel, dim3((unsigned)(planes * chunks)), dim3(256), 0, ST, U, kmax, kmin, ksum, npix, chunks);
  hipLaunchKernelGGL(up_stats_final_kernel, dim3((unsigned)((planes + 255) / 256)), dim3(256), 0, ST, kmax, kmin, ksum, stats, planes);
  WSEG_LAUNCH_CHECK();
  return 0;
}

extern "C" int wseg_up_plane_stats(const float* low, float* stats, long planes, int h, int w, int S, const float* label20, void* workspace, void* stream) {
  WSEG_CHECK(low && stats && workspace && planes > 0 && h > 0 && w > 0 && S > 0 && S <= 32768, "up_plane_stats: bad arguments");
  unsigned long long* kmax = (unsigned long long*)workspace;
  unsigned long long* kmin = kmax + planes;
  float* ksum = (float*)(kmin + planes);
  hipLaunchKernelGGL(up_stats_init_kernel, dim3((unsigned)((planes + 255) / 256)), dim3(256), 0, ST, kmax, kmin, ksum, planes);
  const int chunks = std::max(1, std::min(std::min(16, S / 16), (int)std::max(1L, 4096 / planes)));
  hipLaunchKernelGGL(up_stats_partial_kernel, dim3((unsigned)(planes * chunks)), dim3(256), 0, ST, low, kmax, kmin, ksum, h, w, S, chunks, label20);
  hipLaunchKernelGGL(up_stats_final_kernel, dim3((unsigned)((planes + 255) / 256)), dim3(256), 0, ST, kmax, kmin, ksum, stats, planes);
  WSEG_LAUNCH_CHECK();
  return 0;
}

extern "C" int wseg_up_rvmin_values(const float* low, const float* label20, float* q, unsigned char* argc, int N, int h, int w, int S, void* stream) {
  WSEG_CHECK(low && label20 && q && argc && N > 0 && h > 0 && w > 0 && S > 0, "up_rvmin_values: bad arguments");
  const int rpb = 8;
  hipLaunchKernelGGL(up_rvmin_values_kernel, dim3((S + rpb - 1) / rpb, N), dim3(256), 0, ST, low, label20, q, argc, h, w, S, rpb);
  WSEG_LAUNCH_CHECK();
  return 0;
}

extern "C" int wseg_up_norm_resize_forward(const float* low, const float* stats, const float* label20, float* out, int N, int h, int w, int S, int OS, void* stream) {
  WSEG_CHECK(low && stats && label20 && out && N > 0 && h > 0 && w > 0 && S > 0 && OS > 0, "up_norm_resize_forward: bad arguments");
  const long total = (long)N * 21 * OS * OS;
  hipLaunchKernelGGL(up_norm_resize_fwd_kernel, GRID1(total), 0, ST, low, stats, label20, out, h, w, S, OS, total);
  WSEG_LAUNCH_CHECK();
  return 0;
}

extern "C" int wseg_resize_adjoint_ones(float* wvec, int h, int S, void* stream) {
  WSEG_CHECK(wvec && h > 0 && S > 0, "resize_adjoint_ones: bad arguments");
  hipLaunchKernelGGL(resize_adjoint_ones_kernel, dim3((h + 63) / 64), dim3(64), 0, ST, wvec, h, S);
  WSEG_LAUNCH_CHECK();
  return 0;
}

extern "C" int wseg_up_maps_backward(const float* G, const float* low, const float* stats, const float* label20, const float* plane_bias,
                                     const float* wvec_y, const float* wvec_x, const float* q, const unsigned char* argc, const float* res,
                                     int k, float coef, float* d_low, int N, int h, int w, int S, int OS, void* stream) {
  WSEG_CHECK(low && stats && label20 && d_low && N > 0 && h > 0 && w > 0 && S > 0 && OS > 0, "up_maps_backward: bad arguments");
  WSEG_CHECK((size_t)h * w * 4 <= 60000, "up_maps_backward: low-res plane %dx%d does not fit the LDS image", h, w);
  WSEG_CHECK(plane_bias == nullptr || (wvec_y && wvec_x), "up_maps_backward: plane_bias needs the adjoint-of-ones vectors");
  WSEG_CHECK(q == nullptr || (argc && res), "up_maps_backward: q needs argc and res");
  (void)hipMemsetAsync(d_low, 0, sizeof(float) * (size_t)N * 21 * h * w, ST);
  const int chunks = std::max(1, std::min(64, (S * S) / 2048));
  hipLaunchKernelGGL(up_maps_bwd_kernel, dim3((unsigned)(N * 21 * chunks)), dim3(256), (size_t)h * w * 4, ST, G, low, stats, label20, plane_bias,
                     wvec_y, wvec_x, q, argc, res, k, coef, d_low, h, w, S, OS, chunks);
  WSEG_LAUNCH_CHECK();
  return 0;
}
```

wseg_amd/engine.py:

```python
import threading
import weakref
from typing import NamedTuple

import torch

from . import arch
from . import _lib as L

HEAD_LD = 192
FEAT_LD = 256
AFF_FEAT_C = 448
AFF_FEAT_SLICES = {"f8_3": (0, 64), "f8_4": (64, 192), "f8_5": (192, 448)}


CONTRAST_FLAT_HEAD_ORDER = ("fc_proj", "fc8", "f8_3", "f8_4", "f9")
DT_OF = {"bf16": L.BF16, "fp32": L.F32, "bf16x3": L.F32X3}


def _cdt(dt):
    return L.F32X3 if dt == L.F32X3 else None


class Conv(NamedTuple):
    name: str
    cin: int
    cout: int
    k: int
    stride: int
    dil: int
    din: list
    dout: list

    def _kw(self, N, ic, oc, di, do):
        seg2 = (di[1][0], di[1][1], do[1][0], do[1][1]) if len(di) == 2 else None
        return dict(N=N, IH=di[0][0], IW=di[0][1], IC=ic, OH=do[0][0], OW=do[0][1], OC=oc, KH=self.k, KW=self.k,
                    stride=self.stride, dil=self.dil, pad=self.dil * (self.k // 2), seg2=seg2)

    def fwd_kw(self, N):
        return self._kw(N, self.cin, self.cout, self.din, self.dout)

    def dgrad_kw(self, N):
        return dict(self._kw(N, self.cout, self.cin, self.dout, self.din), mode=1)

    wgrad_kw = fwd_kw


class _Pass:

    def __init__(self, N, dev, dt, P):
        self.N, self.dev, self.dt, self.P = N, dev, dt, P

    def rows_of(self, dims):
        return sum(self.N * h * w for (h, w) in dims)

    def offs_of(self, dims):
        o, out = 0, []
        for (h, w) in dims:
            out.append(o)
            o += self.N * h * w
        return out

    def E(self, m, c):
        return torch.empty((m, c), device=self.dev, dtype=L.TORCH_DTYPE[self.dt])

    def conv(self, c, inp, out, out2=None, **kw):
        L.conv_igemm(inp, self.P["w"][c.name], out, out2, dtype=_cdt(self.dt), **c.fwd_kw(self.N), **kw)


class Engine:

    def __init__(self, net, parent=None):
        self._net_ref = weakref.ref(net)
        self.parent = parent
        self.lock = threading.RLock()
        self.delegate = None
        self.flat_w = None
        self.flat_g = None
        self.packs = None
        self.pack_key = None
        self.injected_masks = None
        self._order = None
        self.flat_w_version = 0
        self.flat_wb = None
        self.flat_wb_version = None
        self.block_done_hook = None
        self.capture_ctx = False
        self.last_ctx = None
        self.last_loss_views = None
        self.offsets = None
        self.flat_w3 = None
        self.flat_wt = self.flat_wt3 = None
        self._wt_table = self._wt_table64 = None
        self._wt_tiles = self._wt_tiles64 = 0
        self._wt_pending = None
        self._frozen_packs = self._frozen_key = None
        self._head_bufs = None
        self._fused = None
        self._late_ev = None
        self._mirror_pversions = None
        self._streams = {}

    @property
    def net(self):
        net = self._net_ref()
        if net is None:
            raise RuntimeError("wseg_amd.Engine outlived its Net")
        return net

    def conv_param(self, name):
        mod = self.net
        for part in name.split("."):
            mod = getattr(mod, part)
        return mod.weight

    def bn_module(self, name):
        mod = self.net
        for part in name.split("."):
            mod = getattr(mod, part)
        return mod

    def trainable_order(self):
        if self._order is None:
            names = []
            for b in arch.BLOCKS:
                if b[0] in arch.FROZEN_BLOCKS:
                    continue
                names += [c[0] for c in arch.block_convs(b)]
            names += list(getattr(self.net, "FLAT_HEAD_ORDER", CONTRAST_FLAT_HEAD_ORDER))
            self._order = names
        return self._order

    def __deepcopy__(self, memo):
        return None

    def __reduce__(self):
        return (type(None), ())

    def ensure_flat(self, device):
        with self.lock:
            return self._ensure_flat(device)

    def active(self, device):
        return self.ensure_flat(device)

    def _ensure_flat(self, device):
        names = self.trainable_order()
        first = self.conv_param(names[0])
        par = self.parent
        if par is not None:
            with par.lock:
                if (par.flat_w is not None and first.device == par.flat_w.device == device
                        and first.data_ptr() == par.flat_w.data_ptr()):
                    self.delegate = par
                    return par
        if (self.flat_w is not None and self.flat_w.device == first.device
                and first.data_ptr() == self.flat_w.data_ptr() and first.device == device):
            self.delegate = None
            return self
        total = sum(self.conv_param(n).numel() for n in names)
        flat_w = torch.empty(total, device=device, dtype=torch.float32)
        flat_g = torch.zeros(total, device=device, dtype=torch.float32)
        off = 0
        self.offsets = {}
        for n in names:
            p = self.conv_param(n)
            oc, ic, kh, kw = p.shape
            view = flat_w[off:off + p.numel()].view(oc, kh, kw, ic).permute(0, 3, 1, 2)
            view.copy_(p.data.to(device))
            p.data = view
            p._wseg_flat = (self, off, p.numel())
            self.offsets[n] = (off, p.numel())
            off += p.numel()
        for n in ["conv1a"] + [c[0] for b in arch.BLOCKS if b[0] in arch.FROZEN_BLOCKS for c in arch.block_convs(b)]:
            p = self.conv_param(n)
            p.data = p.data.to(device).contiguous(memory_format=torch.channels_last)
        self.flat_w, self.flat_g = flat_w, flat_g
        self.packs = None
        self.flat_wb_version = None
        self.delegate = None
        return self

    def _mirror_fresh(self, names):
        return self._mirror_pversions == tuple(self.conv_param(n_)._version for n_ in names)

    def grad_buckets(self, after=("b7", "b5", "b4", "b3")):
        firsts = {}
        for b in arch.BLOCKS:
            if b[0] in arch.FROZEN_BLOCKS:
                continue
            firsts[b[0]] = min(self.offsets[c[0]][0] for c in arch.block_convs(b))
        out, end = {}, self.flat_g.numel()
        for name in after:
            out[name] = (firsts[name], end)
            end = firsts[name]
        assert end == 0, "the last bucket must reach the start of the flat buffer"
        return out

    def grad_slice(self, name, numel=None):
        off, n = self.offsets[name]
        return self.flat_g[off:off + (numel or n)]

    def grad_view(self, name):
        oc, ic, kh, kw = self.conv_param(name).shape
        return self.grad_slice(name).view(oc, kh, kw, ic).permute(0, 3, 1, 2)

    def stream(self, role, device):
        st = self._streams.get(role)
        if st is None or st.device != device:
            st = self._streams[role] = torch.cuda.Stream(device)
        return st

    def _flat_like(self, buf, dtype, device):
        if buf is not None and buf.dtype == dtype and buf.device == device and buf.numel() == self.flat_w.numel():
            return buf
        return torch.empty(self.flat_w.numel(), device=device, dtype=dtype)

    def attach_grads(self):
        names = self.trainable_order()
        p0 = self.conv_param(names[0])
        if p0.grad is not None and p0.grad.data_ptr() == self.flat_g.data_ptr():
            return
        self.flat_g.zero_()
        for n in names:
            p = self.conv_param(n)
            if p.requires_grad:
                p.grad = self.grad_view(n)

    def _bn_fold(self, name, device):
        bn = self.bn_module(name)
        scale = (bn.weight.detach().float() / torch.sqrt(bn.running_var.float() + arch.BN_EPS)).to(device)
        shift = (bn.bias.detach().float() - bn.running_mean.float() * scale).to(device)
        return scale.contiguous(), shift.contiguous()

    @staticmethod
    def _x3(w32):
        out = torch.empty_like(w32)
        L.pack_x3(w32.contiguous(), out)
        return out

    def frozen_key(self, device, dt):
        net = self.net
        frozen_names = [c[0] for b in arch.BLOCKS if b[0] in arch.FROZEN_BLOCKS for c in arch.block_convs(b)]
        return (dt, str(device)) + tuple(b._version for b in net.buffers()) + \
            tuple(p._version for n_, p in net.named_parameters() if ".bn" in n_ or n_.startswith("bn7")) + \
            tuple((self.conv_param(n_)._version, self.conv_param(n_).data_ptr()) for n_ in frozen_names) + \
            (net.conv1a.weight._version, net.conv1a.weight.data_ptr())

    def ensure_packs(self, device, dt, defer_wt=False, late_stream=None):
        with self.lock:
            return self._ensure_packs(device, dt, defer_wt, late_stream)

    def _ensure_packs(self, device, dt, defer_wt=False, late_stream=None):
        net = self.net
        tdt = L.TORCH_DTYPE[dt]
        fkey = self.frozen_key(device, dt)
        if self._frozen_packs is None or self._frozen_key != fkey:
            F_ = {"w": {}, "bn": {}}
            for b in arch.BLOCKS:
                for (bname, c) in arch.block_bns(b):
                    F_["bn"][bname] = self._bn_fold(bname, device)
                if b[0] in arch.FROZEN_BLOCKS:
                    for (cname, ci, co, k, s, d) in arch.block_convs(b):
                        wf = torch.empty(co, k * k, ci, device=device, dtype=tdt)
                        L.pack_weights(self.conv_param(cname).detach(), wf, None, co, k * k, ci, co, ci, L.F32 if dt == L.F32X3 else dt)
                        F_["w"][cname] = self._x3(wf) if dt == L.F32X3 else wf
            F_["bn"]["bn7"] = self._bn_fold("bn7", device)
            F_["w"]["conv1a_kc"] = net.conv1a.weight.detach().to(device).float().permute(2, 3, 1, 0).reshape(27, 64).contiguous()
            self._frozen_packs, self._frozen_key = F_, fkey
            self.packs = None
        names = self.trainable_order()
        key = (dt, str(device), self.flat_w_version) + tuple(self.conv_param(n_)._version for n_ in names)
        if self.packs is not None and key == self.pack_key:
            return self.packs
        P = {"w": dict(self._frozen_packs["w"]), "wt": {}, "bn": self._frozen_packs["bn"]}
        no_dgrad = {"b3.conv_branch1", "b3.conv_branch2a"}
        if dt == L.BF16:
            wb = self._flat_like(self.flat_wb, torch.bfloat16, device)
            if wb is not self.flat_wb:
                self.flat_wb, self.flat_wb_version = wb, None
            if self.flat_wb_version != self.flat_w_version or not self._mirror_fresh(names):
                L.to_bf16(self.flat_w, self.flat_wb)
                self.flat_wb_version = self.flat_w_version
            self._mirror_pversions = tuple(self.conv_param(n_)._version for n_ in names)
            mirror = self.flat_wb
        elif dt == L.F32X3:
            self.flat_w3 = self._flat_like(self.flat_w3, torch.float32, device)
            L.pack_x3(self.flat_w, self.flat_w3)
            mirror = self.flat_w3
        else:
            mirror = self.flat_w
        wt = self._flat_like(self.flat_wt, tdt, device)
        if wt is not self.flat_wt:
            self.flat_wt = wt
            rows, tiles = [], 0
            for b in arch.BLOCKS:
                if b[0] in arch.FROZEN_BLOCKS:
                    continue
                for (cname, ci, co, k, s, d) in arch.block_convs(b):
                    if cname in no_dgrad:
                        continue
                    off, n = self.offsets[cname]
                    rows.append([tiles, off, off, co, k * k, ci])
                    tiles += ((co + 31) // 32) * ((ci + 31) // 32) * k * k
            self._wt_table = torch.tensor(rows, dtype=torch.int64, device=device)
            self._wt_tiles = tiles
            rows64, t64 = [], 0
            for (_t, off_i, off_o, co, T_, ci) in rows:
                rows64.append([t64, off_i, off_o, co, T_, ci])
                t64 += ((co + 63) // 64) * ((ci + 63) // 64) * T_
            self._wt_table64 = torch.tensor(rows64, dtype=torch.int64, device=device)
            self._wt_tiles64 = t64
        self._wt_pending = (dt, mirror)
        if dt == L.F32X3:
            self.flat_wt3 = self._flat_like(self.flat_wt3, torch.float32, device)
        for b in arch.BLOCKS:
            if b[0] in arch.FROZEN_BLOCKS:
                continue
            for (cname, ci, co, k, s, d) in arch.block_convs(b):
                T = k * k
                off, n = self.offsets[cname]
                P["w"][cname] = mirror[off:off + n].view(co, T, ci)
                if cname not in no_dgrad:
                    P["wt"][cname] = (self.flat_wt3 if dt == L.F32X3 else self.flat_wt)[off:off + n].view(ci, T, co)
        def late():
            if dt == L.BF16:
                plan = self._fused_plan(device)
                for nm, buf in plan["fwd_bufs"].items():
                    P["w"][nm + ".skip_fused"] = buf
                L.copy2d_batch(mirror, plan["fwd_flat"], plan["fwd_table"], plan["fwd_table"].shape[0], plan["fwd_chunks"])
            if getattr(net, "HEAD_KIND", "contrast") == "aff":
                for nm, (co, ci) in net.HEAD_CONVS.items():
                    off, n = self.offsets[nm]
                    P["w"][nm] = mirror[off:off + n].view(co, 1, ci)
                return
            hb = self._head_bufs
            if hb is None or hb[0] != (dt, str(device)):
                hb = self._head_bufs = ((dt, str(device)), torch.zeros(256, 1, 4096, device=device, dtype=tdt),
                                        torch.zeros(4096, 1, HEAD_LD, device=device, dtype=tdt),
                                        torch.empty(192, 1, FEAT_LD, device=device, dtype=tdt), torch.empty(FEAT_LD, 1, 192, device=device, dtype=tdt))
            wh, wht = hb[1], hb[2]
            pdt = L.F32 if dt == L.F32X3 else dt
            L.pack_weights(net.fc_proj.weight.detach(), wh, None, 128, 1, 4096, 128, 4096, pdt)
            L.pack_weights(net.fc8.weight.detach(), wh[128:], None, 21, 1, 4096, 21, 4096, pdt)
            off, _ = self.offsets["fc_proj"]
            L.pack_weights(self.flat_w[off:off + 149 * 4096], None, wht, 149, 1, 4096, HEAD_LD, 4096, pdt)
            if dt == L.F32X3:
                wh, wht = self._x3(wh), self._x3(wht)
            P["w"]["head"], P["wt"]["head"] = wh, wht
            for nm, (co, ci) in (("f8_3", (64, 512)), ("f8_4", (128, 1024))):
                off, n = self.offsets[nm]
                P["w"][nm] = mirror[off:off + n].view(co, 1, ci)
            off9, n9 = self.offsets["f9"]
            wf, wt = hb[3], hb[4]
            L.pack_weights(self.flat_w[off9:off9 + n9], wf, wt, 192, 1, 195, 192, FEAT_LD, pdt, ic_rot=3)
            if dt == L.F32X3:
                wf, wt = self._x3(wf), self._x3(wt)
            P["w"]["f9"], P["wt"]["f9"] = wf, wt

        self._late_ev = None
        if late_stream is not None:
            cur = torch.cuda.current_stream(device)
            late_stream.wait_stream(cur)
            with torch.cuda.stream(late_stream):
                late()
            self._late_ev = late_stream.record_event()
        else:
            late()
        self.packs, self.pack_key = P, key
        if not defer_wt:
            self.finish_packs()
        return P

    def _join_late_packs(self, device):
        if self._late_ev is not None:
            torch.cuda.current_stream(device).wait_event(self._late_ev)
            self._late_ev = None

    def finish_packs(self):
        if self._wt_pending is None:
            return
        (dt, mirror), self._wt_pending = self._wt_pending, None
        P = self.packs
        if dt == L.BF16:
            L.pack_transposed_batch_bf16(mirror, self.flat_wt, self._wt_table64, self._wt_table64.shape[0], self._wt_tiles64)
        else:
            L.pack_transposed_batch(self.flat_w, self.flat_wt, self._wt_table, self._wt_table.shape[0], self._wt_tiles, L.F32 if dt == L.F32X3 else dt)
            if dt == L.F32X3:
                L.pack_x3(self.flat_wt, self.flat_wt3)
        if dt == L.BF16 and any(k.endswith(".skip_fused") for k in P["w"]):
            plan = self._fused_plan(self.flat_wt.device)
            for nm, buf in plan["bwd_bufs"].items():
                P["wt"][nm + ".skip_fused"] = buf
            L.copy2d_batch(self.flat_wt, plan["bwd_flat"], plan["bwd_table"], plan["bwd_table"].shape[0], plan["bwd_chunks"])

    def _fused_blocks(self):
        out = []
        for b in arch.BLOCKS:
            nm, kind, cin_, mid_, cout_, stride = b[0], b[1], b[2], b[3], b[4], b[5]
            if nm in arch.FROZEN_BLOCKS or stride != 1 or cout_ % 256:
                continue
            if kind == "res" and not arch.block_same_shape(b) and cin_ % 256 == 0:
                out.append((nm, kind, cin_, mid_, cout_))
            elif kind != "res" and cin_ == cout_ // 2:
                out.append((nm, kind, cin_, mid_, cout_))
        return out

    def _fused_plan(self, device):
        plan = self._fused
        if plan is not None and plan["device"] == device:
            return plan

        def build(pieces_of):
            rows_tab, bufs, sizes, chunk0, base = [], {}, [], 0, 0
            for (nm, kind, cin_, mid_, cout_) in self._fused_blocks():
                nrows, width, pieces = pieces_of(nm, kind, cin_, mid_, cout_)
                for (pname, cols, coff) in pieces:
                    off, n = self.offsets[pname]
                    assert n == nrows * cols and off % 8 == 0 and cols % 8 == 0 and coff % 8 == 0 and width % 8 == 0 and base % 8 == 0
                    rows_tab.append([chunk0, off // 8, (base + coff) // 8, nrows, cols // 8, cols // 8, width // 8])
                    chunk0 += nrows * (cols // 8)
                sizes.append((nm, base, nrows, width))
                base += nrows * width
            flat = torch.empty(base, device=device, dtype=torch.bfloat16)
            for nm, b0, nrows, width in sizes:
                bufs[nm] = flat[b0:b0 + nrows * width].view(nrows, width)
            return flat, bufs, torch.tensor(rows_tab, dtype=torch.int64, device=device), chunk0

        def fwd_pieces(nm, kind, cin_, mid_, cout_):
            if kind == "res":
                return cout_, 9 * mid_ + cin_, [(nm + ".conv_branch2b1", 9 * mid_, 0), (nm + ".conv_branch1", cin_, 9 * mid_)]
            return cout_, cin_ + cout_ // 2, [(nm + ".conv_branch1", cin_, 0), (nm + ".conv_branch2b2", cout_ // 2, cin_)]

        def bwd_pieces(nm, kind, cin_, mid_, cout_):
            if kind == "res":
                return cin_, 9 * mid_ + cout_, [(nm + ".conv_branch2a", 9 * mid_, 0), (nm + ".conv_branch1", cout_, 9 * mid_)]
            return cin_, cout_ + cout_ // 4, [(nm + ".conv_branch1", cout_, 0), (nm + ".conv_branch2a", cout_ // 4, cout_)]

        ff, fb, ft, fc = build(fwd_pieces)
        bf, bb, bt, bc = build(bwd_pieces)
        self._fused = dict(device=device, fwd_flat=ff, fwd_bufs=fb, fwd_table=ft, fwd_chunks=fc, bwd_flat=bf, bwd_bufs=bb, bwd_table=bt, bwd_chunks=bc)
        return self._fused

    MASK_SPECS = (("b6.dropout_2b1", 512, 0.3), ("b6.dropout_2b2", 1024, 0.3),
                  ("b7.dropout_2b1", 1024, 0.5), ("b7.dropout_2b2", 2048, 0.5), ("dropout7", 4096, 0.5))

    def _masks(self, n, views, device):
        net = self.net
        if not net.training:
            return None
        if self.injected_masks:
            per_view = []
            for _ in range(views):
                m = self.injected_masks.pop(0)
                per_view.append({k: v.to(device=device, dtype=torch.float32) for k, v in m.items()})
            return {k: torch.cat([m[k] for m in per_view], dim=0).contiguous() for k in per_view[0]}
        rows = views * n
        total = sum(c for _, c, _ in self.MASK_SPECS)
        u = torch.rand(rows * total, device=device)
        flat = torch.empty_like(u)
        L.dropout_scale(u, flat, rows * (512 + 1024), 0.3, 0.5)
        out, off = {}, 0
        for key, c, _p in self.MASK_SPECS:
            out[key] = flat[off:off + rows * c].view(rows, c)
            off += rows * c
        return out

    def forward(self, x, lowres=False):
        if not x.is_cuda:
            raise RuntimeError("wseg_amd.Net runs only on an MI355X (HIP) device; there is no CPU fallback")
        x = x.contiguous().float()
        act = self.ensure_flat(x.device)
        if act is not self:
            return act.forward(x, lowres)
        need_grad = torch.is_grad_enabled() and any(p.requires_grad for p in self.net.parameters())
        if need_grad:
            anchor = self.flat_w.new_zeros((), requires_grad=True)
            return _NetFunction.apply(x, anchor, self, lowres)
        outs, _ = self.run_forward([x], save=False, lowres=lowres)
        return outs[0]

    def _run_blocks(self, xs, state, first, last, save, S, final_t=None):
        net = self.net
        V = len(xs)
        dev = xs[0].device
        dt = DT_OF[net.precision]
        P = self.ensure_packs(dev, dt)
        N = xs[0].shape[0]
        masks = S["masks"] if S is not None else None
        ps = _Pass(N, dev, dt, P)
        E, conv, rows_of = ps.E, ps.conv, ps.rows_of

        def next_bn(i):
            if i + 1 < len(arch.BLOCKS):
                return P["bn"][arch.BLOCKS[i + 1][0] + ".bn_branch2a"], None
            return P["bn"]["bn7"], (masks["dropout7"] if masks else None)

        sdims = {}
        conv4 = conv5 = None
        if first == 0:
            dims = [(x.shape[2], x.shape[3]) for x in xs]
            sc, sh = P["bn"]["b2.bn_branch2a"]
            t = E(rows_of(dims), 64)
            for x, off, (H, W) in zip(xs, ps.offs_of(dims), dims):
                L.stem_conv_kc(x, P["w"]["conv1a_kc"], sc, sh, None, t[off:], N, H, W, L.F32 if dt == L.F32X3 else dt)
            xraw = None
        else:
            t, xraw, dims = state["t"], state["xraw"], state["dims"]
        for i in range(first, last):
            b = arch.BLOCKS[i]
            name, kind, cin, mid, cout, stride, fd, d, p = b
            same = arch.block_same_shape(b)
            if (name + ".skip_fused") in P["w"]:
                self._join_late_packs(dev)
            (nsc, nsh), ndrop = next_bn(i)
            nxt_same = i + 1 < len(arch.BLOCKS) and arch.block_same_shape(arch.BLOCKS[i + 1])
            odims = arch.block_out_dims(b, dims)
            Mo = rows_of(odims)
            skip = Conv(name + ".conv_branch1", cin, cout, 1, stride, 1, dims, odims)
            if kind == "res":
                s1, sh1 = P["bn"][name + ".bn_branch2b1"]
                v = E(Mo, mid)
                conv(Conv(name + ".conv_branch2a", cin, mid, 3, stride, fd, dims, odims), t, None, v, scale=s1, shift=sh1)
                xn = E(Mo, cout) if nxt_same else None
                tn = final_t if (final_t is not None and i == last - 1) else E(Mo, cout)
                assert tn.shape == (Mo, cout) and tn.dtype == L.TORCH_DTYPE[dt]
                c2b1 = Conv(name + ".conv_branch2b1", mid, cout, 3, 1, d, odims, odims)
                if (name + ".skip_fused") in P["w"]:
                    conv(c2b1._replace(name=name + ".skip_fused"), v, xn, tn, in2=t, IC2=cin, scale=nsc, shift=nsh, drop=ndrop)
                else:
                    if same:
                        rpost = xraw
                    else:
                        rpost = E(Mo, cout)
                        conv(skip, t, rpost)
                    conv(c2b1, v, xn, tn, r_post=rpost, scale=nsc, shift=nsh, drop=ndrop)
                if save:
                    S[name] = dict(t=t, v=v)
            else:
                c4, c2 = cout // 4, cout // 2
                s1, sh1 = P["bn"][name + ".bn_branch2b1"]
                s2, sh2 = P["bn"][name + ".bn_branch2b2"]
                d1 = masks[name + ".dropout_2b1"] if masks else None
                d2 = masks[name + ".dropout_2b2"] if masks else None
                v1 = E(Mo, c4)
                conv(Conv(name + ".conv_branch2a", cin, c4, 1, stride, 1, dims, odims), t, None, v1, scale=s1, shift=sh1, drop=d1)
                v2 = E(Mo, c2)
                conv(Conv(name + ".conv_branch2b1", c4, c2, 3, 1, d, odims, odims), v1, None, v2, scale=s2, shift=sh2, drop=d2)
                xn = None
                tn = E(Mo, cout)
                if (name + ".skip_fused") in P["w"]:
                    conv(Conv(name + ".skip_fused", cin, cout, 1, 1, 1, odims, odims), t, xn, tn, in2=v2, scale=nsc, shift=nsh, drop=ndrop)
                else:
                    b1 = E(Mo, cout)
                    conv(skip, t, b1)
                    conv(Conv(name + ".conv_branch2b2", c2, cout, 1, 1, 1, odims, odims), v2, xn, tn, r_post=b1, scale=nsc, shift=nsh, drop=ndrop)
                if save:
                    S[name] = dict(t=t, v1=v1, v2=v2)
            sdims[name] = (dims, odims)
            if S is not None:
                S["dims"][name] = (dims, odims)
            if name == "b5":
                conv4 = t
            if name == "b6":
                conv5 = t
            t, xraw, dims = tn, xn, odims
        return dict(t=t, xraw=xraw, dims=dims, conv4=conv4, conv5=conv5, sdims=sdims, N=N, V=V, dt=dt,
                    in_dims=state["in_dims"] if state is not None else [tuple(x.shape[2:]) for x in xs])

    def prefix_out_shape(self, xs):
        N = xs[0].shape[0]
        dims = [tuple(x.shape[2:]) for x in xs]
        for b in arch.BLOCKS[:arch.N_FROZEN_BLOCKS]:
            dims = arch.block_out_dims(b, dims)
        return sum(N * h * w for (h, w) in dims), arch.BLOCKS[arch.N_FROZEN_BLOCKS - 1][4]

    def run_prefix(self, xs, out=None):
        return self._run_blocks(xs, None, 0, arch.N_FROZEN_BLOCKS, False, None, final_t=out)

    def run_backbone(self, xs):
        st = self._run_blocks(xs, None, 0, len(arch.BLOCKS), False, None)
        self._join_late_packs(xs[0].device)
        return st, _Pass(st["N"], xs[0].device, st["dt"], self.packs)

    def run_aff_head(self, conv4, conv5, t, dims, N, ps=None):
        if ps is None:
            dev = t.device
            P = self.ensure_packs(dev, DT_OF[self.net.precision])
            self._join_late_packs(dev)
            ps = _Pass(N, dev, DT_OF[self.net.precision], P)
        M = ps.rows_of(dims)
        C = AFF_FEAT_C

        def conv(inp, name, out, cin, cout):
            ps.conv(Conv(name, cin, cout, 1, 1, 1, dims, dims), inp, out, epi=3, ld_out=C)

        feat = ps.E(M, C)
        for name, inp in (("f8_3", conv4), ("f8_4", conv5), ("f8_5", t)):
            (cout, cin), c0 = arch.AFF_HEAD_CONVS[name], AFF_FEAT_SLICES[name][0]
            conv(inp, name, feat.view(-1)[c0:] if c0 else feat, cin, cout)
        f9 = ps.E(M, C)
        conv(feat, "f9", f9, C, C)
        return feat, f9

    def aff_head_wt(self, device):
        dt = DT_OF[self.net.precision]
        with self.lock:
            P = self._ensure_packs(device, dt)
            if "f9" not in P["wt"]:
                pdt = L.F32 if dt == L.F32X3 else dt
                for nm, off, n, (ci, _t, co) in self.aff_head_wt_specs():
                    wt = torch.empty(ci, 1, co, device=device, dtype=L.TORCH_DTYPE[dt])
                    L.pack_weights(self.flat_w[off:off + n], None, wt, co, 1, ci, co, ci, pdt)
                    P["wt"][nm] = self._x3(wt) if dt == L.F32X3 else wt
        self._join_late_packs(device)
        return P

    def aff_head_wt_specs(self):
        return [(nm, *self.offsets[nm], (ci, 1, co)) for nm, (co, ci) in self.net.HEAD_CONVS.items()]

    def run_forward(self, xs, save, lowres=False, prefix=None):
        net = self.net
        V = len(xs)
        assert V in (1, 2)
        dev = xs[0].device
        dt = DT_OF[net.precision]
        P = self.ensure_packs(dev, dt)
        N = xs[0].shape[0]
        assert all(x.shape[0] == N for x in xs)
        masks = self._masks(N, V, dev)
        S = {"masks": masks, "dims": {}, "N": N, "V": V, "dt": dt, "xs": xs, "lowres": lowres}
        if prefix is None:
            prefix = self._run_blocks(xs, None, 0, arch.N_FROZEN_BLOCKS, save and self.capture_ctx, S if (save and self.capture_ctx) else None)
        assert prefix["N"] == N and prefix["V"] == V and prefix["dt"] == dt and prefix["in_dims"] == [tuple(x.shape[2:]) for x in xs], \
            "run_forward: the prefix was computed for another batch shape / precision"
        S["dims"].update(prefix["sdims"])
        st = self._run_blocks(xs, prefix, arch.N_FROZEN_BLOCKS, len(arch.BLOCKS), save, S)
        t, dims, conv4, conv5 = st["t"], st["dims"], st["conv4"], st["conv5"]
        ps = _Pass(N, dev, dt, P)
        E, conv = ps.E, ps.conv

        def head_conv(nm, cin, cout):
            return Conv(nm, cin, cout, 1, 1, 1, dims, dims)

        fea = t
        self._join_late_packs(dev)
        M = ps.rows_of(dims)
        offs = ps.offs_of(dims)
        head = E(M, HEAD_LD)
        conv(head_conv("head", 4096, HEAD_LD), fea, head, relu_lt=128, w_rows=256)
        feat = E(M, FEAT_LD)
        conv(head_conv("f8_3", 512, 64), conv4, feat, epi=2, ld_out=FEAT_LD)
        conv(head_conv("f8_4", 1024, 128), conv5, feat.view(-1)[64:], epi=2, ld_out=FEAT_LD)
        G = torch.empty(M, 32, device=dev, dtype=torch.float32)
        views = []
        for x, off, (h, w) in zip(xs, offs, dims):
            hw = h * w
            cam_low = torch.empty(N, 21, h, w, device=dev, dtype=torch.float32)
            cmax = torch.empty(N, 21, device=dev, dtype=torch.float32)
            L.head_split(head[off:], HEAD_LD, 128, cam_low, cmax, N, hw)
            L.cam_gate(cam_low, cmax, G[off:], N, hw)
            L.pcm_xs(x, feat[off:], FEAT_LD, 192, FEAT_LD, N, x.shape[2], x.shape[3], h, w)
            views.append(dict(h=h, w=w, H=x.shape[2], W=x.shape[3], off=off, rows=N * hw, cam_low=cam_low))
        Fm = E(M, 192)
        conv(head_conv("f9", FEAT_LD, 192), feat, Fm)
        Fh = torch.empty(M, 192, device=dev, dtype=torch.float32)
        nrm = torch.empty(M, device=dev, dtype=torch.float32)
        L.l2norm_forward(Fm, 192, Fh, nrm, M)
        Fb = Gb = Gl = None
        if dt == L.BF16:
            Fb = torch.empty(M, 192, device=dev, dtype=torch.bfloat16)
            Gb = torch.empty(M, 32, device=dev, dtype=torch.bfloat16)
            L.to_bf16(Fh, Fb)
            if save:
                Gl = torch.empty(M, 32, device=dev, dtype=torch.bfloat16)
                L.split_bf16(G, Gb, Gl)
            else:
                L.to_bf16(G, Gb)
        outs = []
        for vw, x in zip(views, xs):
            h, w, off, hw = vw["h"], vw["w"], vw["off"], vw["h"] * vw["w"]
            rvd = torch.empty(N, 21, h, w, device=dev, dtype=torch.float32)
            den = torch.empty(N, hw, device=dev, dtype=torch.float32)
            if dt == L.BF16:
                L.pcm_forward_bf16(Fb[off:], Gb[off:], rvd, den, N, hw)
            else:
                L.pcm_forward(Fh[off:], G[off:], rvd, den, N, hw)
            head_v = head[off:off + N * hw].view(N, h, w, HEAD_LD)
            f_proj = head_v[..., :128].permute(0, 3, 1, 2)
            if lowres:
                outs.append((vw["cam_low"], rvd, f_proj, head_v))
            else:
                H, W = vw["H"], vw["W"]
                cam = torch.empty(N, 21, H, W, device=dev, dtype=torch.float32)
                cam_rv = torch.empty(N, 21, H, W, device=dev, dtype=torch.float32)
                L.resize_planar_fwd(vw["cam_low"], cam, N * 21, h, w, H, W, True)
                L.resize_planar_fwd(rvd, cam_rv, N * 21, h, w, H, W, True)
                outs.append((cam, cam_rv, f_proj.float() if dt == L.BF16 else f_proj, rvd))
            vw.update(rvd=(rvd if lowres else rvd.clone()) if save else None, den=den)
        if save and self.capture_ctx:
            self.last_ctx = S
        if save:
            S.update(fea=fea, head=head, G=G, feat=feat, Fm=Fm, Fh=Fh, Fb=Fb, Gb=Gb, Gl=Gl, nrm=nrm, conv4=conv4, conv5=conv5,
                     views=views, hdims=dims, M=M)
        return outs, S

    def run_backward(self, S, grads, d_head_rows=None):
        self.finish_packs()
        P = self.packs
        dt = S["dt"]
        N, M = S["N"], S["M"]
        hdims = S["hdims"]
        dev = S["fea"].device
        masks = S["masks"]
        self.attach_grads()
        ps = _Pass(N, dev, dt, P)
        E, rows_of = ps.E, ps.rows_of

        def trainable(nm):
            return self.conv_param(nm).requires_grad

        def head_conv(nm, cin, cout):
            return Conv(nm, cin, cout, 1, 1, 1, hdims, hdims)

        main = torch.cuda.current_stream(dev)
        pcm_join = [None]

        planes = {}

        def split(t_):
            key = (t_.data_ptr(), t_.numel())
            if key not in planes:
                hi, lo = torch.empty(t_.shape, device=dev, dtype=torch.bfloat16), torch.empty(t_.shape, device=dev, dtype=torch.bfloat16)
                L.split_bf16(t_, hi, lo)
                planes[key] = (hi, lo, t_)
            return planes[key][:2]

        def wgrad(c, x, dy, **kw):
            if not trainable(c.name):
                return
            dw = self.grad_slice(c.name)
            args = dict(c.wgrad_kw(N), dtype=_cdt(dt), **kw)
            if dt == L.F32X3 and c.cin >= 256 and c.cout >= 256 and not kw and x.is_contiguous() and dy.is_contiguous() \
                    and x.shape[1] == c.cin and dy.shape[1] == c.cout:
                (xh, xl), (dh, dl) = split(x), split(dy)
                args["dtype"] = None
                L.conv_wgrad(xl, dh, dw, **args)
                L.conv_wgrad(xh, dl, dw, **args)
                L.conv_wgrad(xh, dh, dw, **args)
            else:
                L.conv_wgrad(x, dy, dw, **args)

        def block_done(nm):
            if self.block_done_hook is not None:
                if pcm_join[0] is not None:
                    main.wait_stream(pcm_join[0])
                    pcm_join[0] = None
                self.block_done_hook(nm)

        def dgrad(c, dy, out, pair=None, **kw):
            pw = None
            if pair is not None and dt == L.BF16 and trainable(pair[0].name):
                pc, px, pdy = pair
                pw = (px, pdy, self.grad_slice(pc.name), dict(pc.wgrad_kw(N), dtype=_cdt(dt)))
            L.conv_igemm(dy, P["wt"][c.name], out, None, dtype=_cdt(dt), pair_wgrad=pw, **c.dgrad_kw(N), **kw)
            if pair is not None and pw is None:
                wgrad(*pair)

        d_cam_low, d_rvd = [], []
        for vw, (g_cam, g_cam_rv, g_fproj, g_rvd) in zip(S["views"], grads):
            h, w, H, W = vw["h"], vw["w"], vw["H"], vw["W"]
            if S["lowres"]:
                d_cam_low.append(g_cam)
                d_rvd.append(g_cam_rv)
                continue
            dc = None
            if g_cam is not None:
                dc = torch.empty(N, 21, h, w, device=dev, dtype=torch.float32)
                L.resize_planar_bwd(g_cam.contiguous().float(), dc, N * 21, h, w, H, W, True)
            dr = None
            if g_cam_rv is not None:
                dr = torch.empty(N, 21, h, w, device=dev, dtype=torch.float32)
                L.resize_planar_bwd(g_cam_rv.contiguous().float(), dr, N * 21, h, w, H, W, True)
            if g_rvd is not None:
                dr = g_rvd.contiguous().float() if dr is None else dr + g_rvd
            d_cam_low.append(dc)
            d_rvd.append(dr)
        pcm_stream = None
        if any(d is not None for d in d_rvd):
            pcm_stream = self.stream("pcm", dev)
            pcm_stream.wait_stream(main)
            with torch.cuda.stream(pcm_stream):
                DN = torch.empty(M, 32, device=dev, dtype=torch.float32)
                dFh = torch.zeros(M, 192, device=dev, dtype=torch.float32)
                DNb = torch.empty(M, 32, device=dev, dtype=torch.bfloat16) if S["Fb"] is not None else None
                DNl = torch.empty(M, 32, device=dev, dtype=torch.bfloat16) if S["Fb"] is not None else None
                for vw, dr in zip(S["views"], d_rvd):
                    if dr is None:
                        continue
                    off, hw = vw["off"], vw["h"] * vw["w"]
                    if S["Fb"] is not None:
                        L.pcm_backward_bf16(S["Fb"][off:], S["Gb"][off:], S["Gl"][off:], dr.contiguous(), vw["rvd"], vw["den"], DN[off:], DNb[off:],
                                            DNl[off:], dFh[off:], N, hw)
                    else:
                        L.pcm_backward(S["Fh"][off:], S["G"][off:], dr.contiguous(), vw["rvd"], vw["den"], DN[off:], dFh[off:], N, hw)
                dF = E(M, 192)
                L.l2norm_backward(S["Fm"], 192, dFh, S["nrm"], dF, 192, M)
                wgrad(head_conv("f9", FEAT_LD, 192), S["feat"], dF, IC_dw=195, dw_rot=3)
                if trainable("f8_3") or trainable("f8_4"):
                    d_feat = E(M, FEAT_LD)
                    dgrad(head_conv("f9", FEAT_LD, 192), dF, d_feat, epi=1, mask=S["feat"])
                    wgrad(head_conv("f8_3", 512, 64), S["conv4"], d_feat, ld_dy=FEAT_LD)
                    wgrad(head_conv("f8_4", 1024, 128), S["conv5"], d_feat.view(-1)[64:], ld_dy=FEAT_LD)
        pcm_join[0] = pcm_stream
        if d_head_rows is None:
            if all(dc is None for dc in d_cam_low) and all(g[2] is None for g in grads):
                if pcm_stream is not None:
                    main.wait_stream(pcm_stream)
                return
            d_head_rows = E(M, HEAD_LD)
            for vw, dc, g in zip(S["views"], d_cam_low, grads):
                off, hw = vw["off"], vw["h"] * vw["w"]
                gf = g[2].contiguous().float() if g[2] is not None else None
                L.head_grad_rows(gf, dc.contiguous() if dc is not None else None, S["head"][off:], d_head_rows[off:], HEAD_LD, N, hw)
        chead = head_conv("head", 4096, HEAD_LD)
        if trainable("fc_proj") or trainable("fc8"):
            L.conv_wgrad(S["fea"], d_head_rows, self.grad_slice("fc_proj", 149 * 4096), OC_dw=149, dtype=_cdt(dt), **chead.wgrad_kw(N))
        s7, _ = P["bn"]["bn7"]
        D = E(M, 4096)
        dgrad(chead, d_head_rows, D, epi=1, scale=s7, drop=masks["dropout7"] if masks else None, mask=S["fea"])
        for i in range(len(arch.BLOCKS) - 1, -1, -1):
            b = arch.BLOCKS[i]
            name, kind, cin, mid, cout, stride, fd, d, p = b
            if name in arch.FROZEN_BLOCKS:
                break
            same = arch.block_same_shape(b)
            din, dout = S["dims"][name]
            Mi = rows_of(din)
            Mo = rows_of(dout)
            sv = S[name]
            sa, _ = P["bn"][name + ".bn_branch2a"]
            first_trainable = name == "b3"
            c1 = Conv(name + ".conv_branch1", cin, cout, 1, stride, 1, din, dout)
            if kind == "res":
                s1, _ = P["bn"][name + ".bn_branch2b1"]
                c2a = Conv(name + ".conv_branch2a", cin, mid, 3, stride, fd, din, dout)
                c2b1 = Conv(name + ".conv_branch2b1", mid, cout, 3, 1, d, dout, dout)
                du = E(Mo, mid)
                dgrad(c2b1, D, du, epi=1, scale=s1, mask=sv["v"], pair=(c2b1, sv["v"], D))
                fused_skip = (name + ".skip_fused") in P["wt"] and not first_trainable
                if not (same and not first_trainable):
                    wgrad(c2a, sv["t"], du)
                if not same and not fused_skip:
                    wgrad(c1, sv["t"], D)
                if first_trainable:
                    block_done(name)
                    break
                Din = E(Mi, cin)
                if same:
                    dgrad(c2a, du, Din, epi=1, scale=sa, mask=sv["t"], r_post=D, pair=(c2a, sv["t"], du))
                elif fused_skip:
                    dgrad(c2a._replace(name=name + ".skip_fused"), du, Din, in2=D, IC2=cout, epi=1, scale=sa, mask=sv["t"], pair=(c1, sv["t"], D))
                else:
                    tmp = E(Mi, cin)
                    dgrad(c1, D, tmp)
                    dgrad(c2a, du, Din, epi=1, scale=sa, mask=sv["t"], r_pre=tmp)
                D = Din
                block_done(name)
            else:
                c4, c2 = cout // 4, cout // 2
                s1, _ = P["bn"][name + ".bn_branch2b1"]
                s2, _ = P["bn"][name + ".bn_branch2b2"]
                d1 = masks[name + ".dropout_2b1"] if masks else None
                d2 = masks[name + ".dropout_2b2"] if masks else None
                c2a = Conv(name + ".conv_branch2a", cin, c4, 1, stride, 1, din, dout)
                c2b1 = Conv(name + ".conv_branch2b1", c4, c2, 3, 1, d, dout, dout)
                c2b2 = Conv(name + ".conv_branch2b2", c2, cout, 1, 1, 1, dout, dout)
                du2 = E(Mo, c2)
                dgrad(c2b2, D, du2, epi=1, scale=s2, drop=d2, mask=sv["v2"], pair=(c2b2, sv["v2"], D))
                du1 = E(Mo, c4)
                dgrad(c2b1, du2, du1, epi=1, scale=s1, drop=d1, mask=sv["v1"], pair=(c2b1, sv["v1"], du2))
                wgrad(c2a, sv["t"], du1)
                Din = E(Mi, cin)
                if (name + ".skip_fused") in P["wt"]:
                    dgrad(Conv(name + ".skip_fused", cin, cout, 1, 1, 1, din, dout), D, Din, epi=1, scale=sa, mask=sv["t"], in2=du1, IC2=c4,
                          pair=(c1, sv["t"], D))
                else:
                    tmp = E(Mi, cin)
                    dgrad(c1, D, tmp, pair=(c1, sv["t"], D))
                    dgrad(c2a, du1, Din, epi=1, scale=sa, mask=sv["t"], r_pre=tmp)
                D = Din
                block_done(name)
        planes.clear()
        if pcm_join[0] is not None:
            main.wait_stream(pcm_join[0])


class _NetFunction(torch.autograd.Function):
    @staticmethod
    def forward(ctx, x, anchor, eng, lowres):
        outs, S = eng.run_forward([x], save=True, lowres=lowres)
        ctx.eng, ctx.S = eng, S
        ctx.set_materialize_grads(False)
        if lowres:
            ctx.mark_non_differentiable(outs[0][3])
        return outs[0]

    @staticmethod
    def backward(ctx, g0, g1, g2, g3):
        S = ctx.S
        ctx.eng.run_backward(S, [(g0, g1, g2, None if S["lowres"] else g3)])
        ctx.S = None
        return None, None, None, None
```

wseg_amd/loss_hip.py:

```python
import os

import torch
import torch.distributed as dist

from . import _lib as L
from .engine import DT_OF, HEAD_LD

_TIE_CACHE = {}


def cpu_tie_pattern(P, k, device=None):
    key = (P, k)
    if key not in _TIE_CACHE:
        _TIE_CACHE[key] = torch.topk(torch.full((1, P), 0.2), k, dim=-1)[1][0].to(torch.int32)
    if device is None:
        return _TIE_CACHE[key]
    dkey = (P, k, str(device))
    if dkey not in _TIE_CACHE:
        _TIE_CACHE[dkey] = _TIE_CACHE[key].to(device)
    return _TIE_CACHE[dkey]


def _f32(*shape, dev):
    return torch.empty(shape, device=dev, dtype=torch.float32)


class _View:
    pass


_WVEC = {}


def _adjoint_ones(h, S, dev):
    key = (h, S, str(dev))
    if key not in _WVEC:
        wv = torch.empty(h, device=dev, dtype=torch.float32)
        L.resize_adjoint_ones(wv, h, S)
        _WVEC[key] = wv
    return _WVEC[key]


def _maps_forward(v, label20, acc, N):
    dev = v.cam_low.device
    S, h, w = v.S, v.h, v.w
    npix = S * S
    v.st_cam = _f32(N * 21, 6, dev=dev)
    v.st_rv = _f32(N * 21, 6, dev=dev)
    L.up_plane_stats(v.cam_low, v.st_cam, N * 21, h, w, S)
    L.up_plane_stats(v.rvd, v.st_rv, N * 21, h, w, S, label20)
    v.bias = _f32(N * 21, dev=dev)
    L.cls_loss(v.st_cam, label20, acc[0:1], v.bias, N, npix, 0.5)
    v.q = _f32(N, npix, dev=dev)
    v.argc = torch.empty(N, npix, device=dev, dtype=torch.uint8)
    L.up_rvmin_values(v.rvd, label20, v.q, v.argc, N, h, w, S)
    v.k_min = npix // 4
    v.res_min = _f32(N, 4, dev=dev)
    ws = torch.empty(L.select_workspace_bytes(N), device=dev, dtype=torch.uint8)
    L.select_kth(v.q, N, npix, v.k_min, False, False, True, v.res_min, ws)
    L.select_finish(v.res_min, N, v.k_min, True, 0.5 / (v.k_min * N), acc[1:2])
    v.c = _f32(N, 21, 128, 128, dev=dev)
    v.r = _f32(N, 21, 128, 128, dev=dev)
    L.up_norm_resize_forward(v.cam_low, v.st_cam, label20, v.c, N, h, w, S, 128)
    L.up_norm_resize_forward(v.rvd, v.st_rv, label20, v.r, N, h, w, S, 128)


def _maps_backward_cam(v, label20, N):
    dev = v.cam_low.device
    S, h, w = v.S, v.h, v.w
    wy, wx = _adjoint_ones(h, S, dev), _adjoint_ones(w, S, dev)
    v.d_cam_low = _f32(N, 21, h, w, dev=dev)
    L.up_maps_backward(v.Gc, v.cam_low, v.st_cam, label20, v.bias, wy, wx, None, None, None, 0, 0.0, v.d_cam_low, N, h, w, S, 128)


def _maps_backward_rv(v, label20, N):
    dev = v.cam_low.device
    S, h, w = v.S, v.h, v.w
    v.d_rvd = _f32(N, 21, h, w, dev=dev)
    L.up_maps_backward(v.Gr, v.rvd, v.st_rv, label20, None, None, None, v.q, v.argc, v.res_min, v.k_min, 0.5 / (v.k_min * N),
                       v.d_rvd, N, h, w, S, 128)


_CAND_K = 256 // 8
_CAND_L = 21 * _CAND_K * 129 + 32


def _candidates(v, label20, bg_threshold, tie_idx, N, block):
    dev = v.cam_low.device
    P = N * 256
    K = _CAND_K
    v.F = _f32(P, 128, dev=dev)
    L.rows_resize_forward(v.head, HEAD_LD, v.F, N, v.h, v.w, 16, 16)
    if (v.h, v.w) == (16, 16):
        R = v.rvd
    else:
        R = _f32(N, 21, 16, 16, dev=dev)
        L.resize_planar_fwd(v.rvd, R, N * 21, v.h, v.w, 16, 16, True)
    v.y = torch.empty(P, device=dev, dtype=torch.int32)
    v.ncam = _f32(N, 21, 256, dev=dev)
    L.pseudo_label(R, label20, bg_threshold, v.y, v.ncam, N, 256)
    cv, cf = block[:21 * K], block[21 * K:21 * K * 129]
    cc = block[21 * K * 129:21 * K * 129 + 21].view(torch.int32)
    L.proto_candidates(v.ncam, v.F, tie_idx, cv, cf, cc, N, 256, K)


def _merge_prototypes(v, gathered, view_idx, world):
    K = _CAND_K
    base = gathered.view(-1)[view_idx * _CAND_L:]
    v.protos = _f32(21, 128, dev=gathered.device)
    L.proto_merge(base, base[21 * K:], base[21 * K * 129:].view(torch.int32), v.protos, world, K, 2 * _CAND_L)


def _random_keys(P, rank, view_idx, dev):
    seed = os.environ.get("WSEG_INTRA_KEY_SEED")
    if seed is None:
        return torch.rand(P, device=dev)
    g = torch.arange(rank * P, (rank + 1) * P, device=dev, dtype=torch.int64)
    h = (g * 2654435761 + int(seed) * 40503 + view_idx * 97) % 16777213
    return (h * 48271 % 16777213).float() / 16777213.0


def _rand_flags(y_dev, rng, P):
    y = y_dev.cpu()
    for _ in range(P):
        rng.sample(range(21), 10)
    flags = torch.zeros(P, dtype=torch.uint8)
    for cls in torch.unique(y).tolist():
        members = (y == cls).nonzero(as_tuple=True)[0]
        n_c = members.numel()
        if n_c < 2:
            continue
        flags[members[torch.tensor(rng.sample(range(n_c), n_c // 2), dtype=torch.long)]] = 1
    return flags.to(y_dev.device)


def step(model, img1, img2, label20, bg_threshold=0.20, rng=None, rng_parity=False, bg_topk_idx=None, zero_grads=False, prefix=None, lookahead=None):
    eng = model._engine
    dev = img1.device
    N = img1.shape[0]
    from .train import dist_state
    world, distributed = dist_state()
    label20 = label20.to(dev).float().contiguous()
    eng.ensure_flat(dev)
    eng.attach_grads()
    aux = eng.stream("aux", dev)
    eng.ensure_packs(dev, DT_OF[model.precision], defer_wt=True, late_stream=aux)
    acc = torch.zeros(8, device=dev, dtype=torch.float32)
    main = torch.cuda.current_stream(dev)
    side = (eng.stream("side0", dev), eng.stream("side1", dev))
    outs, ctx = eng.run_forward([img1, img2], save=True, lowres=True, prefix=prefix)
    fork = main.record_event()
    pst = None
    if lookahead is not None:
        pst = eng.stream("prefix", dev)
        n1 = lookahead["img1"]
        n2 = torch.empty(n1.shape[0], n1.shape[1], img2.shape[-2], img2.shape[-1], device=dev, dtype=torch.float32)
        rows, ch = eng.prefix_out_shape([n1, n2])
        t_next = torch.empty(rows, ch, device=dev, dtype=L.TORCH_DTYPE[DT_OF[model.precision]])
        pst.wait_event(fork)
        with torch.cuda.stream(pst):
            L.resize_planar_fwd(n1, n2, n1.shape[0] * n1.shape[1], n1.shape[2], n1.shape[3], n2.shape[2], n2.shape[3], True)
            lookahead["img2"], lookahead["prefix"] = n2, eng.run_prefix([n1, n2], out=t_next)
    aux.wait_event(fork)
    with torch.cuda.stream(aux):
        eng.finish_packs()
        if zero_grads:
            eng.flat_g.zero_()
    P = N * 256
    tie_idx = (bg_topk_idx.to(device=dev, dtype=torch.int32) if bg_topk_idx is not None else cpu_tie_pattern(P, 32, dev))
    views = []
    for img, (cam_low, rvd, _fp, head), vw in zip((img1, img2), outs, ctx["views"]):
        v = _View()
        v.S, v.h, v.w, v.off = img.shape[2], vw["h"], vw["w"], vw["off"]
        v.cam_low, v.rvd, v.head = cam_low, rvd, head
        views.append(v)
    v1, v2 = views
    cand = _f32(2, _CAND_L, dev=dev)
    for vi, v in enumerate(views):
        side[vi].wait_event(fork)
        with torch.cuda.stream(side[vi]):
            _maps_forward(v, label20, acc, N)
    for vi, v in enumerate(views):
        _candidates(v, label20, bg_threshold, tie_idx, N, cand[vi])
    gathered = cand
    if distributed:
        gathered = _f32(world, 2, _CAND_L, dev=dev)
        dist.all_gather_into_tensor(gathered.view(world * 2, _CAND_L), cand)
    for vi, v in enumerate(views):
        _merge_prototypes(v, gathered, vi, world)
    npix = 128 * 128
    er_coef = 1.0 / (N * 20 * npix)
    est = side[0]
    est.wait_stream(side[1])
    with torch.cuda.stream(est):
        for v in views:
            v.Gc = _f32(N, 21, 128, 128, dev=dev)
        dlt = _f32(2 * N, 21 * npix, dev=dev)
        L.er_ecr_prep(v1.c, v2.c, v1.r, v2.r, v1.Gc, v2.Gc, dlt[:N], dlt[N:], acc[2:3], N, npix, er_coef)
        prep_done = est.record_event()
        K_ecr = int(21 * npix * 0.2)
        ws = torch.empty(L.select_workspace_bytes(2 * N), device=dev, dtype=torch.uint8)
        res = _f32(2 * N, 4, dev=dev)
        L.select_kth(dlt, 2 * N, 21 * npix, K_ecr, True, True, False, res, ws)
        L.select_finish(res, 2 * N, K_ecr, False, 1.0 / (N * K_ecr), acc[3:4])
        Gr = _f32(2 * N, 21, 128, 128, dev=dev)
        L.ecr_backward(dlt, res, Gr, 2 * N, 21 * npix, K_ecr, 1.0 / (N * K_ecr))
        v1.Gr, v2.Gr = Gr[:N], Gr[N:]
        ecr_done = est.record_event()
        _maps_backward_rv(v1, label20, N)
    side[1].wait_event(prep_done)
    with torch.cuda.stream(side[1]):
        _maps_backward_cam(v1, label20, N)
        _maps_backward_cam(v2, label20, N)
    global_intra = distributed or not rng_parity
    rank = dist.get_rank() if distributed else 0
    nce_x3 = model.precision != "fp32"
    rec = _f32(2, 3, P, dev=dev)
    for vi, v in enumerate(views):
        v.rkey = _random_keys(P, rank, vi, dev) if global_intra else None
    L.nce_records([dict(F=v.F, p_own=v.protos, y_own=v.y, rkey=v.rkey, rec=rec[vi]) for vi, v in enumerate(views)], P, split_bf16=nce_x3)
    grec = rec
    if distributed:
        grec = _f32(world, 2, 3, P, dev=dev)
        dist.all_gather_into_tensor(grec.view(world * 6, P), rec.view(6, P))
    elif not global_intra:
        for vi, v in enumerate(views):
            v.w_intra = _f32(P, dev=dev)
            L.intra_weights(v.y, rec[vi, 1], None, _rand_flags(v.y, rng, P), v.w_intra, P, ld_s=1)
    def weights_of(vi, v):
        if global_intra:
            v.w_intra = _f32(P, dev=dev)
            L.intra_weights_global(grec.view(-1)[vi * 3 * P:], v.w_intra, P, world, rank, float(world), 6 * P)

    fork2 = main.record_event()
    weights_of(0, v1)
    side[1].wait_event(fork2)
    with torch.cuda.stream(side[1]):
        weights_of(1, v2)
        w2_done = side[1].record_event()
        side[1].wait_event(ecr_done)
        _maps_backward_rv(v2, label20, N)
    main.wait_event(w2_done)
    for v in views:
        v.dF = _f32(P, 128, dev=dev)
    L.nce_fused([dict(F=v.F, p_own=v.protos, p_oth=o.protos, y_own=v.y, y_oth=o.y, w_intra=v.w_intra, dF=v.dF) for v, o in ((v1, v2), (v2, v1))],
                P, 0.1 / (2 * P), 0.05, acc[4:7])
    d_head = torch.empty_like(ctx["head"])
    main.wait_stream(side[0])
    main.wait_stream(side[1])
    for v in views:
        L.head_grad_fused(v.dF, v.d_cam_low, v.head, d_head[v.off:], HEAD_LD, N, v.h, v.w, 16, 16)
    main.wait_stream(aux)
    if pst is not None:
        main.wait_stream(pst)
    eng.run_backward(ctx, [(None, v.d_rvd, None, None) for v in views], d_head_rows=d_head)
    if eng.capture_ctx:
        eng.last_loss_views = views
    out8 = torch.empty(8, device=dev, dtype=torch.float32)
    L.loss_finish(acc, er_coef, out8)
    return dict(zip(("loss", "loss_cls", "loss_er", "loss_ecr", "loss_nce", "loss_intra_nce", "loss_cross_nce", "loss_cross_nce2"), out8.unbind(0)))
```

Before: 470.6 images/sec.

## Batch per-view loss map kernels into multi-job launches on a single stream

Adds a job-descriptor interface so that plane stats, cls loss, rvmin, norm-resize, k-th selection and map backward kernels handle both views (and cam/rv maps) in one launch, replacing the separate per-view launches. Map buffers are preallocated contiguously, the forward map work moves onto one side stream, and the cam and rv backward passes are rescheduled across streams. The prefix lookahead now waits on a backbone-done event rather than the end of the forward pass. The aim is to cut launch count and stream synchronisation overhead in the loss; the cost is less cross-stream concurrency between views and more decode logic inside each kernel.

```diff
diff --git a/include/wseg_hip.h b/include/wseg_hip.h
--- a/include/wseg_hip.h
+++ b/include/wseg_hip.h
@@ -118,6 +118,54 @@
 size_t wseg_select_workspace_bytes(int rows);
 int wseg_select_kth(const float* vals, int rows, int n, int k, int largest, int use_abs, int relu_vals, float* res, void* workspace, void* stream);
 int wseg_select_finish(const float* res, int rows, int k, int relu_vals, float scale, float* loss_out, void* stream);
+
+#define WSEG_MAX_JOBS 4
+typedef struct wseg_map_job {
+  const float* low;
+  const float* label20;
+  float* stats;
+  void* workspace;
+  float* out;
+  unsigned char* argc;
+  const float* G;
+  const float* plane_bias;
+  const float* wvec_y;
+  const float* wvec_x;
+  const float* q;
+  const float* res;
+  float* loss_out;
+  int64_t planes;
+  int32_t N, h, w, S, OS;
+  int32_t k;
+  float coef;
+} wseg_map_job;
+#define WSEG_JOBS_STATS_PLANES 0
+#define WSEG_JOBS_STATS 1
+#define WSEG_JOBS_CLS 2
+#define WSEG_JOBS_RVMIN 3
+#define WSEG_JOBS_NORM_RESIZE 4
+#define WSEG_JOBS_BACKWARD 5
+typedef struct wseg_job_plan {
+  int32_t njobs, grid;
+  int32_t block0[WSEG_MAX_JOBS], units[WSEG_MAX_JOBS], chunks[WSEG_MAX_JOBS];
+} wseg_job_plan;
+int wseg_map_jobs_plan(int kind, const wseg_map_job* jobs, int njobs, wseg_job_plan* out);
+int wseg_map_jobs_decode(const wseg_job_plan* plan, int block, int32_t* out3);
+int wseg_up_plane_stats_multi(const wseg_map_job* jobs, int njobs, void* stream);
+int wseg_cls_loss_multi(const wseg_map_job* jobs, int njobs, void* stream);
+int wseg_up_rvmin_values_multi(const wseg_map_job* jobs, int njobs, void* stream);
+int wseg_up_norm_resize_forward_multi(const wseg_map_job* jobs, int njobs, void* stream);
+int wseg_up_maps_backward_multi(const wseg_map_job* jobs, int njobs, void* stream);
+
+typedef struct wseg_select_group {
+  const float* vals;
+  int32_t rows, n, k;
+  float scale;
+} wseg_select_group;
+typedef struct wseg_select_row { int64_t offset; int32_t group, n, rank, hist_blocks, sum_blocks; } wseg_select_row;
+int wseg_select_rows(const wseg_select_group* groups, int ngroups, int largest, wseg_select_row* rows_out, int max_rows, int32_t* grid2);
+int wseg_select_kth_multi(const wseg_select_group* groups, int ngroups, int largest, int use_abs, int relu_vals, float* res, void* workspace, void* stream);
+int wseg_select_finish_multi(const wseg_select_group* groups, int ngroups, const float* res, int relu_vals, float* loss_out, void* stream);
 int wseg_loss_finish(const float* acc, float er_coef, float* out8, void* stream);
 int wseg_er_ecr_prep(const float* c1, const float* c2, const float* r1, const float* r2, float* Gc1, float* Gc2, float* dlt1, float* dlt2,
                      float* er_sum, int N, int npix, float er_coef, void* stream);
diff --git a/wseg_amd/_lib.py b/wseg_amd/_lib.py
--- a/wseg_amd/_lib.py
+++ b/wseg_amd/_lib.py
@@ -367,6 +367,75 @@
           k, _f(coef), _v(d_low), N, h, w, S, OS)
 
 
+MAX_JOBS = 4
+JOBS_STATS_PLANES, JOBS_STATS, JOBS_CLS, JOBS_RVMIN, JOBS_NORM_RESIZE, JOBS_BACKWARD = range(6)
+
+
+class MapJob(C.Structure):
+    _fields_ = [(k, C.c_void_p) for k in ("low", "label20", "stats", "workspace", "out", "argc", "G", "plane_bias", "wvec_y", "wvec_x", "q", "res", "loss_out")] + \
+               [("planes", C.c_int64)] + [(k, C.c_int32) for k in ("N", "h", "w", "S", "OS", "k")] + [("coef", C.c_float)]
+
+
+class JobPlan(C.Structure):
+    _fields_ = [("njobs", C.c_int32), ("grid", C.c_int32), ("block0", C.c_int32 * MAX_JOBS), ("units", C.c_int32 * MAX_JOBS), ("chunks", C.c_int32 * MAX_JOBS)]
+
+
+class SelectGroup(C.Structure):
+    _fields_ = [("vals", C.c_void_p), ("rows", C.c_int32), ("n", C.c_int32), ("k", C.c_int32), ("scale", C.c_float)]
+
+
+class SelectRow(C.Structure):
+    _fields_ = [("offset", C.c_int64), ("group", C.c_int32), ("n", C.c_int32), ("rank", C.c_int32), ("hist_blocks", C.c_int32), ("sum_blocks", C.c_int32)]
+
+
+def _map_jobs(jobs):
+    arr = (MapJob * len(jobs))()
+    for i, j in enumerate(jobs):
+        for k, t in MapJob._fields_:
+            x = j.get(k)
+            setattr(arr[i], k, _ptr(x) if t is C.c_void_p else (x or 0))
+    return arr
+
+
+def _select_groups(groups):
+    arr = (SelectGroup * len(groups))()
+    for i, g in enumerate(groups):
+        arr[i].vals, arr[i].rows, arr[i].n, arr[i].k, arr[i].scale = _ptr(g.get("vals")), g["rows"], g["n"], g["k"], g.get("scale", 0.0)
+    return arr
+
+
+def map_jobs_plan(kind, jobs):
+    plan = JobPlan()
+    check(lib.wseg_map_jobs_plan(kind, _map_jobs(jobs), len(jobs), C.byref(plan)), "wseg_map_jobs_plan")
+    return plan
+
+
+def map_jobs_decode(plan, block):
+    out = (C.c_int32 * 3)()
+    check(lib.wseg_map_jobs_decode(C.byref(plan), block, out), "wseg_map_jobs_decode")
+    return tuple(out)
+
+
+def select_rows(groups, largest):
+    cap = sum(g["rows"] for g in groups)
+    rows, grid2 = (SelectRow * max(cap, 1))(), (C.c_int32 * 2)()
+    n = lib.wseg_select_rows(_select_groups(groups), len(groups), int(largest), rows, cap, grid2)
+    check(min(n, 0), "wseg_select_rows")
+    return [rows[i] for i in range(n)], tuple(grid2)
+
+
+def up_plane_stats_multi(jobs):
+    ws = [torch.empty(int(lib.wseg_plane_stats_workspace_bytes(C.c_long(j["N"] * 21))), device=j["low"].device, dtype=torch.uint8) for j in jobs]
+    _call("wseg_up_plane_stats_multi", _map_jobs([dict(j, workspace=w) for j, w in zip(jobs, ws)]), len(jobs))
+def cls_loss_multi(jobs): _call("wseg_cls_loss_multi", _map_jobs(jobs), len(jobs))
+def up_rvmin_values_multi(jobs): _call("wseg_up_rvmin_values_multi", _map_jobs(jobs), len(jobs))
+def up_norm_resize_forward_multi(jobs): _call("wseg_up_norm_resize_forward_multi", _map_jobs(jobs), len(jobs))
+def up_maps_backward_multi(jobs): _call("wseg_up_maps_backward_multi", _map_jobs(jobs), len(jobs))
+def select_kth_multi(groups, largest, use_abs, relu_vals, res, ws):
+    _call("wseg_select_kth_multi", _select_groups(groups), len(groups), int(largest), int(use_abs), int(relu_vals), _v(res), _v(ws))
+def select_finish_multi(groups, res, relu_vals, loss_out): _call("wseg_select_finish_multi", _select_groups(groups), len(groups), _v(res), int(relu_vals), _v(loss_out))
+
+
 def gemm256_probe(A, B, Cout, M, N, K, variant=0):
     if not hasattr(lib, "wseg_gemm256_probe"):
         raise RuntimeError("wseg_gemm256_probe is a development probe: rebuild with `WSEG_PROBES=1 bash wseg_amd/csrc/build.sh`")
diff --git a/wseg_amd/csrc/loss.hip b/wseg_amd/csrc/loss.hip
--- a/wseg_amd/csrc/loss.hip
+++ b/wseg_amd/csrc/loss.hip
@@ -1,11 +1,18 @@
 #include <algorithm>
 #include "loss_helpers.h"
+#include "map_jobs.h"
 
 namespace {
 
-__global__ void cls_loss_kernel(const float* __restrict__ stats, const float* __restrict__ label20, float* __restrict__ loss_out,
-                                float* __restrict__ plane_bias, int N, int npix, float coef) {
+__global__ void cls_loss_kernel(const MapJobs J) {
   __shared__ float red[4];
+  const wseg_map_job& g = J.j[wseg_job_decode(J.plan, blockIdx.x).job];
+  const float* __restrict__ stats = g.stats;
+  const float* __restrict__ label20 = g.label20;
+  float* __restrict__ loss_out = g.loss_out;
+  float* __restrict__ plane_bias = g.out;
+  const int N = g.N, npix = g.k > 0 ? g.k : g.S * g.S;
+  const float coef = g.coef;
   float acc = 0.f;
   for (int i = threadIdx.x; i < N * 21; i += blockDim.x) {
     const int n = i / 21, c = i - n * 21;
@@ -25,15 +32,18 @@
   if (threadIdx.x == 0) atomicAdd(loss_out, tot / (20.f * N));
 }
 
-__global__ __launch_bounds__(256) void select_hist_kernel(const float* __restrict__ vals, int n, int use_abs, const unsigned* __restrict__ state,
+__global__ __launch_bounds__(256) void select_hist_kernel(const wseg_select_groups G, int use_abs, const unsigned* __restrict__ state,
                                                           unsigned* __restrict__ hist, int shift) {
   __shared__ unsigned h[4][256];
   const int row = blockIdx.y, wv = threadIdx.x >> 6;
+  const wseg_select_row R = wseg_select_row_of(G, row, 0);
+  const int n = R.n, nblk = R.hist_blocks;
+  if ((int)blockIdx.x >= nblk) return;
 #pragma unroll
   for (int w = 0; w < 4; ++w) h[w][threadIdx.x] = 0;
   __syncthreads();
   const unsigned prefix = state[row * 4 + 0], mask = state[row * 4 + 1];
-  const float* v = vals + (size_t)row * n;
+  const float* v = G.g[R.group].vals + R.offset;
   auto count = [&](float f) {
     if (use_abs) f = fabsf(f);
     const unsigned k = f2key(f);
@@ -41,12 +51,12 @@
   };
   if ((n & 3) == 0) {
     const float4* v4 = reinterpret_cast<const float4*>(v);
-    for (int i = blockIdx.x * 256 + threadIdx.x; i < (n >> 2); i += gridDim.x * 256) {
+    for (int i = blockIdx.x * 256 + threadIdx.x; i < (n >> 2); i += nblk * 256) {
       const float4 q = v4[i];
       count(q.x); count(q.y); count(q.z); count(q.w);
     }
   } else {
-    for (int i = blockIdx.x * 256 + threadIdx.x; i < n; i += gridDim.x * 256) count(v[i]);
+    for (int i = blockIdx.x * 256 + threadIdx.x; i < n; i += nblk * 256) count(v[i]);
   }
   __syncthreads();
   const unsigned t = h[0][threadIdx.x] + h[1][threadIdx.x] + h[2][threadIdx.x] + h[3][threadIdx.x];
@@ -84,18 +94,22 @@
     state[row * 4 + 2] = k - cum;
   }
 }
-__global__ void select_init_kernel(unsigned* __restrict__ state, unsigned* __restrict__ hist, int rows, unsigned rank_small, float* __restrict__ res) {
+__global__ void select_init_kernel(const wseg_select_groups G, int largest, unsigned* __restrict__ state, unsigned* __restrict__ hist, float* __restrict__ res) {
   const int i = blockIdx.x * blockDim.x + threadIdx.x;
-  if (i < rows) { state[i * 4 + 0] = 0; state[i * 4 + 1] = 0; state[i * 4 + 2] = rank_small; state[i * 4 + 3] = 0; }
+  const int rows = G.row0[G.ngroups];
+  if (i < rows) { state[i * 4 + 0] = 0; state[i * 4 + 1] = 0; state[i * 4 + 2] = (unsigned)wseg_select_row_of(G, i, largest).rank; state[i * 4 + 3] = 0; }
   if (i < rows * 4) res[i] = 0.f;
   if (i < rows * 256) hist[i] = 0;
 }
-__global__ __launch_bounds__(256) void select_sum_kernel(const float* __restrict__ vals, int n, int use_abs, int largest, int relu_vals,
+__global__ __launch_bounds__(256) void select_sum_kernel(const wseg_select_groups G, int use_abs, int largest, int relu_vals,
                                                          const unsigned* __restrict__ state, float* __restrict__ res) {
   __shared__ float red[4];
   const int row = blockIdx.y;
+  const wseg_select_row R = wseg_select_row_of(G, row, largest);
+  const int n = R.n, nblk = R.sum_blocks;
+  if ((int)blockIdx.x >= nblk) return;
   const float thr = key2f(state[row * 4 + 0]);
-  const float* v = vals + (size_t)row * n;
+  const float* v = G.g[R.group].vals + R.offset;
   float s = 0.f, cs = 0.f, ce = 0.f;
   auto take = [&](float f) {
     if (use_abs) f = fabsf(f);
@@ -105,12 +119,12 @@
   };
   if ((n & 3) == 0) {
     const float4* v4 = reinterpret_cast<const float4*>(v);
-    for (int i = blockIdx.x * 256 + threadIdx.x; i < (n >> 2); i += gridDim.x * 256) {
+    for (int i = blockIdx.x * 256 + threadIdx.x; i < (n >> 2); i += nblk * 256) {
       const float4 q = v4[i];
       take(q.x); take(q.y); take(q.z); take(q.w);
     }
   } else {
-    for (int i = blockIdx.x * 256 + threadIdx.x; i < n; i += gridDim.x * 256) take(v[i]);
+    for (int i = blockIdx.x * 256 + threadIdx.x; i < n; i += nblk * 256) take(v[i]);
   }
   const float S = block_sum(s, red), CS = block_sum(cs, red), CE = block_sum(ce, red);
   if (threadIdx.x == 0) {
@@ -118,14 +132,17 @@
     atomicAdd(&res[row * 4 + 1], S); atomicAdd(&res[row * 4 + 2], CS); atomicAdd(&res[row * 4 + 3], CE);
   }
 }
-__global__ void select_finish_kernel(const float* __restrict__ res, int rows, int k, int relu_vals, float scale, float* __restrict__ loss_out) {
+__global__ void select_finish_kernel(const wseg_select_groups G, const float* __restrict__ res, int relu_vals, float* __restrict__ loss_out) {
   if (threadIdx.x == 0 && blockIdx.x == 0) {
-    float t = 0.f;
-    for (int r = 0; r < rows; ++r) {
-      const float thr = relu_vals ? fmaxf(res[r * 4 + 0], 0.f) : res[r * 4 + 0];
-      t += res[r * 4 + 1] + ((float)k - res[r * 4 + 2]) * thr;
-    }
-    atomicAdd(loss_out, t * scale);
+    for (int j = 0; j < G.ngroups; ++j) {
+      const int k = G.g[j].k;
+      float t = 0.f;
+      for (int r = G.row0[j]; r < G.row0[j + 1]; ++r) {
+        const float thr = relu_vals ? fmaxf(res[r * 4 + 0], 0.f) : res[r * 4 + 0];
+        t += res[r * 4 + 1] + ((float)k - res[r * 4 + 2]) * thr;
+      }
+      atomicAdd(loss_out, t * G.g[j].scale);
+    }
   }
 }
 
@@ -364,36 +381,84 @@
 #define GRID1(total) dim3((unsigned)(((total) + 255) / 256)), dim3(256)
 #define ST ((hipStream_t)stream)
 
+extern "C" int wseg_cls_loss_multi(const wseg_map_job* jobs, int njobs, void* stream) {
+  WSEG_CHECK(jobs && njobs >= 1 && njobs <= WSEG_MAX_JOBS, "cls_loss: 1..%d jobs", WSEG_MAX_JOBS);
+  for (int j = 0; j < njobs; ++j)
+    WSEG_CHECK(jobs[j].stats && jobs[j].label20 && jobs[j].loss_out && jobs[j].out && jobs[j].N > 0 && (jobs[j].S > 0 || jobs[j].k > 0), "cls_loss: bad arguments (job %d)", j);
+  const MapJobs J = make_jobs(WSEG_JOBS_CLS, jobs, njobs);
+  hipLaunchKernelGGL(cls_loss_kernel, dim3((unsigned)J.plan.grid), dim3(256), 0, ST, J);
+  WSEG_LAUNCH_CHECK();
+  return 0;
+}
 extern "C" int wseg_cls_loss(const float* stats, const float* label20, float* loss_out, float* plane_bias, int N, int npix, float coef, void* stream) {
   WSEG_CHECK(stats && label20 && loss_out && plane_bias && N > 0, "cls_loss: bad arguments");
-  hipLaunchKernelGGL(cls_loss_kernel, dim3(1), dim3(256), 0, ST, stats, label20, loss_out, plane_bias, N, npix, coef);
-  WSEG_LAUNCH_CHECK();
-  return 0;
+  wseg_map_job job = {};
+  job.stats = const_cast<float*>(stats); job.label20 = label20; job.loss_out = loss_out; job.out = plane_bias; job.N = N; job.k = npix; job.coef = coef;
+  return wseg_cls_loss_multi(&job, 1, stream);
 }
 
 extern "C" size_t wseg_select_workspace_bytes(int rows) { return (size_t)rows * (4 + 256) * sizeof(unsigned); }
+static int select_groups_of(const wseg_select_group* groups, int ngroups, wseg_select_groups* G, const char* what) {
+  WSEG_CHECK(groups && ngroups >= 1 && ngroups <= WSEG_MAX_JOBS, "%s: 1..%d row groups", what, WSEG_MAX_JOBS);
+  *G = {};
+  for (int j = 0; j < ngroups; ++j) {
+    const wseg_select_group& g = groups[j];
+    WSEG_CHECK(g.rows > 0 && g.n > 0 && g.k >= 1 && g.k <= g.n && G->row0[j] + (long)g.rows < (1L << 16), "%s: bad arguments (rows=%d n=%d k=%d)", what, g.rows, g.n, g.k);
+    G->g[j] = g;
+    G->row0[j + 1] = G->row0[j] + g.rows;
+  }
+  G->ngroups = ngroups;
+  return 0;
+}
+extern "C" int wseg_select_rows(const wseg_select_group* groups, int ngroups, int largest, wseg_select_row* rows_out, int max_rows, int32_t* grid2) {
+  wseg_select_groups G;
+  if (int e = select_groups_of(groups, ngroups, &G, "select_rows")) return e;
+  const int rows = G.row0[ngroups];
+  WSEG_CHECK(rows_out && grid2 && rows <= max_rows, "select_rows: room for %d rows needed", rows);
+  grid2[0] = grid2[1] = 0;
+  for (int r = 0; r < rows; ++r) {
+    rows_out[r] = wseg_select_row_of(G, r, largest);
+    grid2[0] = std::max(grid2[0], rows_out[r].hist_blocks); grid2[1] = std::max(grid2[1], rows_out[r].sum_blocks);
+  }
+  return rows;
+}
+extern "C" int wseg_select_kth_multi(const wseg_select_group* groups, int ngroups, int largest, int use_abs, int relu_vals, float* res, void* workspace, void* stream) {
+  wseg_select_groups G;
+  if (int e = select_groups_of(groups, ngroups, &G, "select_kth")) return e;
+  for (int j = 0; j < ngroups; ++j) WSEG_CHECK(groups[j].vals, "select_kth: bad arguments (group %d)", j);
+  WSEG_CHECK(res && workspace, "select_kth: bad arguments");
+  const int rows = G.row0[ngroups];
+  unsigned* state = (unsigned*)workspace;
+  unsigned* hist = state + (size_t)rows * 4;
+  int gx = 1, gs = 1;
+  for (int j = 0; j < ngroups; ++j) { gx = std::max(gx, select_hist_blocks(groups[j].n)); gs = std::max(gs, select_sum_blocks(groups[j].n)); }
+  hipLaunchKernelGGL(select_init_kernel, dim3((rows * 256 + 255) / 256), dim3(256), 0, ST, G, largest, state, hist, res);
+  for (int shift = 24; shift >= 0; shift -= 8) {
+    hipLaunchKernelGGL(select_hist_kernel, dim3(gx, rows), dim3(256), 0, ST, G, use_abs, state, hist, shift);
+    hipLaunchKernelGGL(select_scan_kernel, dim3(rows), dim3(64), 0, ST, state, hist, shift, rows);
+  }
+  hipLaunchKernelGGL(select_sum_kernel, dim3(gs, rows), dim3(256), 0, ST, G, use_abs, largest, relu_vals, state, res);
+  WSEG_LAUNCH_CHECK();
+  return 0;
+}
 extern "C" int wseg_select_kth(const float* vals, int rows, int n, int k, int largest, int use_abs, int relu_vals,
                                float* res, void* workspace, void* stream) {
   WSEG_CHECK(vals && res && workspace && rows > 0 && n > 0 && k >= 1 && k <= n, "select_kth: bad arguments (rows=%d n=%d k=%d)", rows, n, k);
-  unsigned* state = (unsigned*)workspace;
-  unsigned* hist = state + (size_t)rows * 4;
-  const unsigned rank_small = largest ? (unsigned)(n - k + 1) : (unsigned)k;
-  hipLaunchKernelGGL(select_init_kernel, dim3((rows * 256 + 255) / 256), dim3(256), 0, ST, state, hist, rows, rank_small, res);
-  const int gx = std::max(1, std::min(128, (n + 4095) / 4096));
-  const int gs = std::max(1, std::min(32, (n + 8191) / 8192));
-  for (int shift = 24; shift >= 0; shift -= 8) {
-    hipLaunchKernelGGL(select_hist_kernel, dim3(gx, rows), dim3(256), 0, ST, vals, n, use_abs, state, hist, shift);
-    hipLaunchKernelGGL(select_scan_kernel, dim3(rows), dim3(64), 0, ST, state, hist, shift, rows);
-  }
-  hipLaunchKernelGGL(select_sum_kernel, dim3(gs, rows), dim3(256), 0, ST, vals, n, use_abs, largest, relu_vals, state, res);
+  const wseg_select_group g = {vals, rows, n, k, 0.f};
+  return wseg_select_kth_multi(&g, 1, largest, use_abs, relu_vals, res, workspace, stream);
+}
+extern "C" int wseg_select_finish_multi(const wseg_select_group* groups, int ngroups, const float* res, int relu_vals, float* loss_out, void* stream) {
+  wseg_select_groups G;
+  if (int e = select_groups_of(groups, ngroups, &G, "select_finish")) return e;
+  WSEG_CHECK(res && loss_out, "select_finish: bad arguments");
+  hipLaunchKernelGGL(select_finish_kernel, dim3(1), dim3(64), 0, ST, G, res, relu_vals, loss_out);
   WSEG_LAUNCH_CHECK();
   return 0;
 }
 extern "C" int wseg_select_finish(const float* res, int rows, int k, int relu_vals, float scale, float* loss_out, void* stream) {
   WSEG_CHECK(res && loss_out && rows > 0, "select_finish: bad arguments");
-  hipLaunchKernelGGL(select_finish_kernel, dim3(1), dim3(64), 0, ST, res, rows, k, relu_vals, scale, loss_out);
-  WSEG_LAUNCH_CHECK();
-  return 0;
+  const wseg_select_group g = {nullptr, rows, std::max(k, 1), std::max(k, 1), scale};
+  return wseg_select_finish_multi(&g, 1, res, relu_vals, loss_out, stream);
 }
 
 static __global__ void loss_finish_kernel(const float* __restrict__ acc, float er_coef, float* __restrict__ out) {
diff --git a/wseg_amd/csrc/map_jobs.h b/wseg_amd/csrc/map_jobs.h
--- /dev/null
+++ b/wseg_amd/csrc/map_jobs.h
@@ -0,0 +1,75 @@
+#pragma once
+#include "common.h"
+
+struct wseg_job_pos { int job, plane, chunk; };
+
+__host__ __device__ inline void wseg_job_plan_add(wseg_job_plan& p, int units, int chunks) {
+  const int j = p.njobs++;
+  p.block0[j] = p.grid; p.units[j] = units; p.chunks[j] = chunks;
+  p.grid += units * chunks;
+}
+__host__ __device__ inline wseg_job_pos wseg_job_decode(const wseg_job_plan& p, int block) {
+  int j = 0;
+#pragma unroll
+  for (int i = 1; i < WSEG_MAX_JOBS; ++i)
+    if (i < p.njobs && block >= p.block0[i]) j = i;
+  const int local = block - p.block0[j];
+  const int pl = local / p.chunks[j];
+  return {j, pl, local - pl * p.chunks[j]};
+}
+
+__host__ __device__ inline long wseg_job_planes(const wseg_map_job& g) { return g.planes > 0 ? g.planes : (long)g.N * 21; }
+
+__host__ __device__ inline int wseg_imin(int a, int b) { return a < b ? a : b; }
+__host__ __device__ inline int wseg_imax(int a, int b) { return a > b ? a : b; }
+__host__ __device__ inline int up_stats_chunks(long planes, int S) {
+  return wseg_imax(1, wseg_imin(wseg_imin(16, S / 16), (int)(4096 / planes > 1 ? 4096 / planes : 1)));
+}
+__host__ __device__ inline int up_bwd_chunks(int S) { return wseg_imax(1, wseg_imin(64, (S * S) / 2048)); }
+constexpr int RVMIN_ROWS_PER_BLOCK = 8;
+
+__host__ __device__ inline wseg_job_plan wseg_map_jobs_layout(int kind, const wseg_map_job* jobs, int njobs) {
+  wseg_job_plan p = {};
+  for (int j = 0; j < njobs; ++j) {
+    const wseg_map_job& g = jobs[j];
+    const long planes = (long)g.N * 21, sp = wseg_job_planes(g);
+    switch (kind) {
+      case WSEG_JOBS_STATS_PLANES: wseg_job_plan_add(p, (int)((sp + 255) / 256), 1); break;
+      case WSEG_JOBS_STATS: wseg_job_plan_add(p, (int)sp, up_stats_chunks(sp, g.S)); break;
+      case WSEG_JOBS_CLS: wseg_job_plan_add(p, 1, 1); break;
+      case WSEG_JOBS_RVMIN: wseg_job_plan_add(p, g.N, (g.S + RVMIN_ROWS_PER_BLOCK - 1) / RVMIN_ROWS_PER_BLOCK); break;
+      case WSEG_JOBS_NORM_RESIZE: wseg_job_plan_add(p, (int)((planes * g.OS * g.OS + 255) / 256), 1); break;
+      default: wseg_job_plan_add(p, (int)planes, up_bwd_chunks(g.S)); break;
+    }
+  }
+  return p;
+}
+
+struct MapJobs { wseg_map_job j[WSEG_MAX_JOBS]; wseg_job_plan plan; };
+inline MapJobs make_jobs(int kind, const wseg_map_job* jobs, int njobs) {
+  MapJobs J = {};
+  for (int j = 0; j < njobs; ++j) J.j[j] = jobs[j];
+  J.plan = wseg_map_jobs_layout(kind, jobs, njobs);
+  return J;
+}
+
+struct wseg_select_groups {
+  wseg_select_group g[WSEG_MAX_JOBS];
+  int row0[WSEG_MAX_JOBS + 1];
+  int ngroups;
+};
+__host__ __device__ inline int select_hist_blocks(int n) { return wseg_imax(1, wseg_imin(128, (n + 4095) / 4096)); }
+__host__ __device__ inline int select_sum_blocks(int n) { return wseg_imax(1, wseg_imin(32, (n + 8191) / 8192)); }
+__host__ __device__ inline wseg_select_row wseg_select_row_of(const wseg_select_groups& G, int row, int largest) {
+  int j = 0;
+#pragma unroll
+  for (int i = 1; i < WSEG_MAX_JOBS; ++i)
+    if (i < G.ngroups && row >= G.row0[i]) j = i;
+  const wseg_select_group& g = G.g[j];
+  wseg_select_row r;
+  r.group = j; r.n = g.n;
+  r.offset = (int64_t)(row - G.row0[j]) * g.n;
+  r.rank = largest ? g.n - g.k + 1 : g.k;
+  r.hist_blocks = select_hist_blocks(g.n); r.sum_blocks = select_sum_blocks(g.n);
+  return r;
+}
diff --git a/wseg_amd/csrc/maps.hip b/wseg_amd/csrc/maps.hip
--- a/wseg_amd/csrc/maps.hip
+++ b/wseg_amd/csrc/maps.hip
@@ -1,7 +1,14 @@
 #include <algorithm>
 #include "loss_helpers.h"
+#include "map_jobs.h"
 
 namespace {
+
+struct StatsKeys { unsigned long long* kmax; unsigned long long* kmin; float* ksum; };
+__host__ __device__ inline StatsKeys stats_keys(void* workspace, long planes) {
+  unsigned long long* kmax = (unsigned long long*)workspace;
+  return {kmax, kmax + planes, (float*)(kmax + 2 * planes)};
+}
 
 __device__ __forceinline__ float up_value(const float* __restrict__ p, int w, int y0, int y1, int x0, int x1, float fy, float fx) {
   const float a = __fmaf_rn(fx, p[y0 * w + x1], __fmul_rn(1.f - fx, p[y0 * w + x0]));
@@ -46,12 +53,17 @@
   if (tid == 0) { atomicMax(&kmax[pl], s_mx[0]); atomicMin(&kmin[pl], s_mn[0]); atomicAdd(&ksum[pl], s_sum[0]); }
 }
 
-__global__ __launch_bounds__(256) void up_stats_partial_kernel(const float* __restrict__ low, unsigned long long* __restrict__ kmax,
-                                                              unsigned long long* __restrict__ kmin, float* __restrict__ ksum,
-                                                              int h, int w, int S, int chunks, const float* __restrict__ label20) {
+__global__ __launch_bounds__(256) void up_stats_partial_kernel(const MapJobs J) {
   __shared__ unsigned long long s_mx[256], s_mn[256];
   __shared__ float s_sum[256];
-  const int pl = blockIdx.x / chunks, ck = blockIdx.x - pl * chunks, tid = threadIdx.x;
+  const wseg_job_pos pos = wseg_job_decode(J.plan, blockIdx.x);
+  const wseg_map_job& g = J.j[pos.job];
+  const float* __restrict__ low = g.low;
+  const float* __restrict__ label20 = g.label20;
+  const int h = g.h, w = g.w, S = g.S, chunks = J.plan.chunks[pos.job];
+  const StatsKeys K = stats_keys(g.workspace, wseg_job_planes(g));
+  unsigned long long* __restrict__ kmax = K.kmax; unsigned long long* __restrict__ kmin = K.kmin; float* __restrict__ ksum = K.ksum;
+  const int pl = pos.plane, ck = pos.chunk, tid = threadIdx.x;
   if (label20) {
     const int c = pl % 21;
     if (c >= 1 && label20[(pl / 21) * 20 + c - 1] == 0.f) return;
@@ -123,25 +135,43 @@
   }
   if (tid == 0) { atomicMax(&kmax[pl], s_mx[0]); atomicMin(&kmin[pl], s_mn[0]); atomicAdd(&ksum[pl], s_sum[0]); }
 }
-__global__ void up_stats_init_kernel(unsigned long long* __restrict__ kmax, unsigned long long* __restrict__ kmin, float* __restrict__ ksum, long planes) {
-  const long pl = (long)blockIdx.x * blockDim.x + threadIdx.x;
-  if (pl < planes) { kmax[pl] = 0ull; kmin[pl] = ~0ull; ksum[pl] = 0.f; }
-}
-__global__ void up_stats_final_kernel(const unsigned long long* __restrict__ kmax, const unsigned long long* __restrict__ kmin,
-                                      const float* __restrict__ ksum, float* __restrict__ stats, long planes) {
-  const long pl = (long)blockIdx.x * blockDim.x + threadIdx.x;
-  if (pl >= planes) return;
+__global__ void up_stats_init_kernel(const MapJobs J) {
+  const wseg_job_pos pos = wseg_job_decode(J.plan, blockIdx.x);
+  const long planes = wseg_job_planes(J.j[pos.job]);
+  const StatsKeys K = stats_keys(J.j[pos.job].workspace, planes);
+  const long pl = (long)pos.plane * 256 + threadIdx.x;
+  if (pl < planes) { K.kmax[pl] = 0ull; K.kmin[pl] = ~0ull; K.ksum[pl] = 0.f; }
+}
+__device__ __forceinline__ void stats_final_one(const unsigned long long* __restrict__ kmax, const unsigned long long* __restrict__ kmin,
+                                                const float* __restrict__ ksum, float* __restrict__ stats, long pl) {
   float* o = stats + pl * 6;
   o[0] = __uint_as_float((unsigned)(kmax[pl] >> 32)); o[1] = __uint_as_float((unsigned)(kmin[pl] >> 32)); o[2] = ksum[pl];
   o[3] = __int_as_float((int)(~(unsigned)(kmax[pl] & 0xFFFFFFFFull))); o[4] = __int_as_float((int)(unsigned)(kmin[pl] & 0xFFFFFFFFull)); o[5] = 0.f;
 }
-
-__global__ __launch_bounds__(256) void up_rvmin_values_kernel(const float* __restrict__ low, const float* __restrict__ label20,
-                                                             float* __restrict__ q, unsigned char* __restrict__ argc,
-                                                             int h, int w, int S, int rows_per_block) {
-  const int n = blockIdx.y, tid = threadIdx.x;
+__global__ void up_stats_final_kernel(const MapJobs J) {
+  const wseg_job_pos pos = wseg_job_decode(J.plan, blockIdx.x);
+  const long planes = wseg_job_planes(J.j[pos.job]);
+  const StatsKeys K = stats_keys(J.j[pos.job].workspace, planes);
+  const long pl = (long)pos.plane * 256 + threadIdx.x;
+  if (pl < planes) stats_final_one(K.kmax, K.kmin, K.ksum, J.j[pos.job].stats, pl);
+}
+__global__ void plane_stats_final_kernel(const unsigned long long* __restrict__ kmax, const unsigned long long* __restrict__ kmin,
+                                         const float* __restrict__ ksum, float* __restrict__ stats, long planes) {
+  const long pl = (long)blockIdx.x * blockDim.x + threadIdx.x;
+  if (pl < planes) stats_final_one(kmax, kmin, ksum, stats, pl);
+}
+
+__global__ __launch_bounds__(256) void up_rvmin_values_kernel(const MapJobs J) {
+  const wseg_job_pos pos = wseg_job_decode(J.plan, blockIdx.x);
+  const wseg_map_job& g = J.j[pos.job];
+  const float* __restrict__ low = g.low;
+  const float* __restrict__ label20 = g.label20;
+  float* __restrict__ q = g.out;
+  unsigned char* __restrict__ argc = g.argc;
+  const int h = g.h, w = g.w, S = g.S;
+  const int n = pos.plane, tid = threadIdx.x;
   const float sy = ac_scale(h, S), sx = ac_scale(w, S);
-  const int r0 = blockIdx.x * rows_per_block, r1 = min(S, r0 + rows_per_block);
+  const int r0 = pos.chunk * RVMIN_ROWS_PER_BLOCK, r1 = min(S, r0 + RVMIN_ROWS_PER_BLOCK);
   const int tpr = threads_per_row(S), rpi = 256 / tpr;
   const int tr = tid / tpr, tx = tid & (tpr - 1);
   const float* lab = label20 + n * 20;
@@ -164,9 +194,16 @@
   }
 }
 
-__global__ void up_norm_resize_fwd_kernel(const float* __restrict__ low, const float* __restrict__ stats, const float* __restrict__ label20,
-                                          float* __restrict__ out, int h, int w, int S, int OS, long total) {
-  const long idx = (long)blockIdx.x * blockDim.x + threadIdx.x;
+__global__ void up_norm_resize_fwd_kernel(const MapJobs J) {
+  const wseg_job_pos pos = wseg_job_decode(J.plan, blockIdx.x);
+  const wseg_map_job& g = J.j[pos.job];
+  const float* __restrict__ low = g.low;
+  const float* __restrict__ stats = g.stats;
+  const float* __restrict__ label20 = g.label20;
+  float* __restrict__ out = g.out;
+  const int h = g.h, w = g.w, S = g.S, OS = g.OS;
+  const long total = (long)g.N * 21 * OS * OS;
+  const long idx = (long)pos.plane * 256 + threadIdx.x;
   if (idx >= total) return;
   const int ox = (int)(idx % OS); const long r = idx / OS;
   const int oy = (int)(r % OS); const long pl = r / OS;
@@ -201,15 +238,25 @@
   wvec[y] = acc;
 }
 
-__global__ __launch_bounds__(256) void up_maps_bwd_kernel(const float* __restrict__ G, const float* __restrict__ low, const float* __restrict__ stats,
-                                                         const float* __restrict__ label20, const float* __restrict__ plane_bias,
-                                                         const float* __restrict__ wvec_y, const float* __restrict__ wvec_x,
-                                                         const float* __restrict__ q, const unsigned char* __restrict__ argc,
-                                                         const float* __restrict__ res, int k, float coef,
-                                                         float* __restrict__ d_low, int h, int w, int S, int OS, int chunks) {
+__global__ __launch_bounds__(256) void up_maps_bwd_kernel(const MapJobs J) {
   extern __shared__ float dl[];
   __shared__ float red[4];
-  const int pl = blockIdx.x / chunks, ck = blockIdx.x - pl * chunks, tid = threadIdx.x;
+  const wseg_job_pos pos = wseg_job_decode(J.plan, blockIdx.x);
+  const wseg_map_job& jb = J.j[pos.job];
+  const float* __restrict__ G = jb.G;
+  const float* __restrict__ low = jb.low;
+  const float* __restrict__ stats = jb.stats;
+  const float* __restrict__ label20 = jb.label20;
+  const float* __restrict__ plane_bias = jb.plane_bias;
+  const float* __restrict__ wvec_y = jb.wvec_y;
+  const float* __restrict__ wvec_x = jb.wvec_x;
+  const float* __restrict__ q = jb.q;
+  const unsigned char* __restrict__ argc = jb.argc;
+  const float* __restrict__ res = jb.res;
+  float* __restrict__ d_low = jb.out;
+  const int k = jb.k, h = jb.h, w = jb.w, S = jb.S, OS = jb.OS, chunks = J.plan.chunks[pos.job];
+  const float coef = jb.coef;
+  const int pl = pos.plane, ck = pos.chunk, tid = threadIdx.x;
   const int c = pl % 21; const int n = pl / 21;
   const float L = c == 0 ? 1.f : label20[n * 20 + c - 1];
   const float bias = (plane_bias && ck == 0) ? plane_bias[pl] : 0.f;
@@ -321,38 +368,80 @@
   (void)hipMemsetAsync(ksum, 0x00, sizeof(float) * planes, ST);
   const int chunks = std::max(1, std::min(std::min(64, (int)((long)npix / 8192)), (int)std::max(1L, 2048 / planes)));
   hipLaunchKernelGGL(plane_stats_partial_kernel, dim3((unsigned)(planes * chunks)), dim3(256), 0, ST, U, kmax, kmin, ksum, npix, chunks);
-  hipLaunchKernelGGL(up_stats_final_kernel, dim3((unsigned)((planes + 255) / 256)), dim3(256), 0, ST, kmax, kmin, ksum, stats, planes);
-  WSEG_LAUNCH_CHECK();
-  return 0;
-}
-
+  hipLaunchKernelGGL(plane_stats_final_kernel, dim3((unsigned)((planes + 255) / 256)), dim3(256), 0, ST, kmax, kmin, ksum, stats, planes);
+  WSEG_LAUNCH_CHECK();
+  return 0;
+}
+
+static int check_jobs(const wseg_map_job* jobs, int njobs, const char* what) {
+  WSEG_CHECK(jobs && njobs >= 1 && njobs <= WSEG_MAX_JOBS, "%s: 1..%d jobs", what, WSEG_MAX_JOBS);
+  for (int j = 0; j < njobs; ++j)
+    WSEG_CHECK(jobs[j].low && jobs[j].N > 0 && jobs[j].h > 0 && jobs[j].w > 0 && jobs[j].S > 0 && jobs[j].S <= 32768 && (long)jobs[j].N * 21 * 64 < (1L << 30),
+               "%s: bad arguments (job %d)", what, j);
+  return 0;
+}
+extern "C" int wseg_map_jobs_plan(int kind, const wseg_map_job* jobs, int njobs, wseg_job_plan* out) {
+  WSEG_CHECK(out && kind >= WSEG_JOBS_STATS_PLANES && kind <= WSEG_JOBS_BACKWARD, "map_jobs_plan: bad arguments");
+  WSEG_CHECK(jobs && njobs >= 1 && njobs <= WSEG_MAX_JOBS, "map_jobs_plan: 1..%d jobs", WSEG_MAX_JOBS);
+  for (int j = 0; j < njobs; ++j)
+    WSEG_CHECK(jobs[j].N > 0 && jobs[j].h > 0 && jobs[j].w > 0 && jobs[j].S > 0 && (kind != WSEG_JOBS_NORM_RESIZE || jobs[j].OS > 0), "map_jobs_plan: bad geometry (job %d)", j);
+  *out = wseg_map_jobs_layout(kind, jobs, njobs);
+  return 0;
+}
+extern "C" int wseg_map_jobs_decode(const wseg_job_plan* plan, int block, int32_t* out3) {
+  WSEG_CHECK(plan && out3 && plan->njobs >= 1 && plan->njobs <= WSEG_MAX_JOBS && block >= 0 && block < plan->grid, "map_jobs_decode: bad arguments");
+  const wseg_job_pos p = wseg_job_decode(*plan, block);
+  out3[0] = p.job; out3[1] = p.plane; out3[2] = p.chunk;
+  return 0;
+}
+
+extern "C" int wseg_up_plane_stats_multi(const wseg_map_job* jobs, int njobs, void* stream) {
+  if (int e = check_jobs(jobs, njobs, "up_plane_stats")) return e;
+  for (int j = 0; j < njobs; ++j) WSEG_CHECK(jobs[j].stats && jobs[j].workspace, "up_plane_stats: bad arguments (job %d)", j);
+  const MapJobs P = make_jobs(WSEG_JOBS_STATS_PLANES, jobs, njobs), C = make_jobs(WSEG_JOBS_STATS, jobs, njobs);
+  hipLaunchKernelGGL(up_stats_init_kernel, dim3((unsigned)P.plan.grid), dim3(256), 0, ST, P);
+  hipLaunchKernelGGL(up_stats_partial_kernel, dim3((unsigned)C.plan.grid), dim3(256), 0, ST, C);
+  hipLaunchKernelGGL(up_stats_final_kernel, dim3((unsigned)P.plan.grid), dim3(256), 0, ST, P);
+  WSEG_LAUNCH_CHECK();
+  return 0;
+}
 extern "C" int wseg_up_plane_stats(const float* low, float* stats, long planes, int h, int w, int S, const float* label20, void* workspace, void* stream) {
   WSEG_CHECK(low && stats && workspace && planes > 0 && h > 0 && w > 0 && S > 0 && S <= 32768, "up_plane_stats: bad arguments");
-  unsigned long long* kmax = (unsigned long long*)workspace;
-  unsigned long long* kmin = kmax + planes;
-  float* ksum = (float*)(kmin + planes);
-  hipLaunchKernelGGL(up_stats_init_kernel, dim3((unsigned)((planes + 255) / 256)), dim3(256), 0, ST, kmax, kmin, ksum, planes);
-  const int chunks = std::max(1, std::min(std::min(16, S / 16), (int)std::max(1L, 4096 / planes)));
-  hipLaunchKernelGGL(up_stats_partial_kernel, dim3((unsigned)(planes * chunks)), dim3(256), 0, ST, low, kmax, kmin, ksum, h, w, S, chunks, label20);
-  hipLaunchKernelGGL(up_stats_final_kernel, dim3((unsigned)((planes + 255) / 256)), dim3(256), 0, ST, kmax, kmin, ksum, stats, planes);
-  WSEG_LAUNCH_CHECK();
-  return 0;
-}
-
+  wseg_map_job job = {};
+  job.low = low; job.label20 = label20; job.stats = stats; job.workspace = workspace; job.planes = planes; job.N = (int)((planes + 20) / 21); job.h = h; job.w = w; job.S = S;
+  return wseg_up_plane_stats_multi(&job, 1, stream);
+}
+
+extern "C" int wseg_up_rvmin_values_multi(const wseg_map_job* jobs, int njobs, void* stream) {
+  if (int e = check_jobs(jobs, njobs, "up_rvmin_values")) return e;
+  for (int j = 0; j < njobs; ++j) WSEG_CHECK(jobs[j].label20 && jobs[j].out && jobs[j].argc, "up_rvmin_values: bad arguments (job %d)", j);
+  const MapJobs J = make_jobs(WSEG_JOBS_RVMIN, jobs, njobs);
+  hipLaunchKernelGGL(up_rvmin_values_kernel, dim3((unsigned)J.plan.grid), dim3(256), 0, ST, J);
+  WSEG_LAUNCH_CHECK();
+  return 0;
+}
 extern "C" int wseg_up_rvmin_values(const float* low, const float* label20, float* q, unsigned char* argc, int N, int h, int w, int S, void* stream) {
   WSEG_CHECK(low && label20 && q && argc && N > 0 && h > 0 && w > 0 && S > 0, "up_rvmin_values: bad arguments");
-  const int rpb = 8;
-  hipLaunchKernelGGL(up_rvmin_values_kernel, dim3((S + rpb - 1) / rpb, N), dim3(256), 0, ST, low, label20, q, argc, h, w, S, rpb);
-  WSEG_LAUNCH_CHECK();
-  return 0;
-}
-
+  wseg_map_job job = {};
+  job.low = low; job.label20 = label20; job.out = q; job.argc = argc; job.N = N; job.h = h; job.w = w; job.S = S;
+  return wseg_up_rvmin_values_multi(&job, 1, stream);
+}
+
+extern "C" int wseg_up_norm_resize_forward_multi(const wseg_map_job* jobs, int njobs, void* stream) {
+  if (int e = check_jobs(jobs, njobs, "up_norm_resize_forward")) return e;
+  for (int j = 0; j < njobs; ++j)
+    WSEG_CHECK(jobs[j].stats && jobs[j].label20 && jobs[j].out && jobs[j].OS > 0 && (long)jobs[j].N * 21 * jobs[j].OS * jobs[j].OS < (1L << 38),
+               "up_norm_resize_forward: bad arguments (job %d)", j);
+  const MapJobs J = make_jobs(WSEG_JOBS_NORM_RESIZE, jobs, njobs);
+  hipLaunchKernelGGL(up_norm_resize_fwd_kernel, dim3((unsigned)J.plan.grid), dim3(256), 0, ST, J);
+  WSEG_LAUNCH_CHECK();
+  return 0;
+}
 extern "C" int wseg_up_norm_resize_forward(const float* low, const float* stats, const float* label20, float* out, int N, int h, int w, int S, int OS, void* stream) {
   WSEG_CHECK(low && stats && label20 && out && N > 0 && h > 0 && w > 0 && S > 0 && OS > 0, "up_norm_resize_forward: bad arguments");
-  const long total = (long)N * 21 * OS * OS;
-  hipLaunchKernelGGL(up_norm_resize_fwd_kernel, GRID1(total), 0, ST, low, stats, label20, out, h, w, S, OS, total);
-  WSEG_LAUNCH_CHECK();
-  return 0;
+  wseg_map_job job = {};
+  job.low = low; job.stats = const_cast<float*>(stats); job.label20 = label20; job.out = out; job.N = N; job.h = h; job.w = w; job.S = S; job.OS = OS;
+  return wseg_up_norm_resize_forward_multi(&job, 1, stream);
 }
 
 extern "C" int wseg_resize_adjoint_ones(float* wvec, int h, int S, void* stream) {
@@ -362,17 +451,31 @@
   return 0;
 }
 
+extern "C" int wseg_up_maps_backward_multi(const wseg_map_job* jobs, int njobs, void* stream) {
+  if (int e = check_jobs(jobs, njobs, "up_maps_backward")) return e;
+  size_t lds = 0;
+  for (int j = 0; j < njobs; ++j) {
+    const wseg_map_job& g = jobs[j];
+    WSEG_CHECK(g.stats && g.label20 && g.out && g.OS > 0, "up_maps_backward: bad arguments (job %d)", j);
+    WSEG_CHECK((size_t)g.h * g.w * 4 <= 60000, "up_maps_backward: low-res plane %dx%d does not fit the LDS image", g.h, g.w);
+    WSEG_CHECK(g.plane_bias == nullptr || (g.wvec_y && g.wvec_x), "up_maps_backward: plane_bias needs the adjoint-of-ones vectors");
+    WSEG_CHECK(g.q == nullptr || (g.argc && g.res), "up_maps_backward: q needs argc and res");
+    lds = std::max(lds, (size_t)g.h * g.w * 4);
+  }
+  const MapJobs J = make_jobs(WSEG_JOBS_BACKWARD, jobs, njobs);
+  hipLaunchKernelGGL(up_maps_bwd_kernel, dim3((unsigned)J.plan.grid), dim3(256), lds, ST, J);
+  WSEG_LAUNCH_CHECK();
+  return 0;
+}
 extern "C" int wseg_up_maps_backward(const float* G, const float* low, const float* stats, const float* label20, const float* plane_bias,
                                      const float* wvec_y, const float* wvec_x, const float* q, const unsigned char* argc, const float* res,
                                      int k, float coef, float* d_low, int N, int h, int w, int S, int OS, void* stream) {
   WSEG_CHECK(low && stats && label20 && d_low && N > 0 && h > 0 && w > 0 && S > 0 && OS > 0, "up_maps_backward: bad arguments");
-  WSEG_CHECK((size_t)h * w * 4 <= 60000, "up_maps_backward: low-res plane %dx%d does not fit the LDS image", h, w);
-  WSEG_CHECK(plane_bias == nullptr || (wvec_y && wvec_x), "up_maps_backward: plane_bias needs the adjoint-of-ones vectors");
-  WSEG_CHECK(q == nullptr || (argc && res), "up_maps_backward: q needs argc and res");
+  wseg_map_job job = {};
+  job.G = G; job.low = low; job.stats = const_cast<float*>(stats); job.label20 = label20; job.plane_bias = plane_bias; job.wvec_y = wvec_y; job.wvec_x = wvec_x;
+  job.q = q; job.argc = const_cast<unsigned char*>(argc); job.res = res; job.k = k; job.coef = coef; job.out = d_low;
+  job.N = N; job.h = h; job.w = w; job.S = S; job.OS = OS;
+  if (int e = check_jobs(&job, 1, "up_maps_backward")) return e;
   (void)hipMemsetAsync(d_low, 0, sizeof(float) * (size_t)N * 21 * h * w, ST);
-  const int chunks = std::max(1, std::min(64, (S * S) / 2048));
-  hipLaunchKernelGGL(up_maps_bwd_kernel, dim3((unsigned)(N * 21 * chunks)), dim3(256), (size_t)h * w * 4, ST, G, low, stats, label20, plane_bias,
-                     wvec_y, wvec_x, q, argc, res, k, coef, d_low, h, w, S, OS, chunks);
-  WSEG_LAUNCH_CHECK();
-  return 0;
-}
+  return wseg_up_maps_backward_multi(&job, 1, stream);
+}
diff --git a/wseg_amd/engine.py b/wseg_amd/engine.py
--- a/wseg_amd/engine.py
+++ b/wseg_amd/engine.py
@@ -636,6 +636,8 @@
         S["dims"].update(prefix["sdims"])
         st = self._run_blocks(xs, prefix, arch.N_FROZEN_BLOCKS, len(arch.BLOCKS), save, S)
         t, dims, conv4, conv5 = st["t"], st["dims"], st["conv4"], st["conv5"]
+        if save:
+            S["backbone_done"] = torch.cuda.current_stream(dev).record_event()
         ps = _Pass(N, dev, dt, P)
         E, conv = ps.E, ps.conv
 
diff --git a/wseg_amd/loss_hip.py b/wseg_amd/loss_hip.py
--- a/wseg_amd/loss_hip.py
+++ b/wseg_amd/loss_hip.py
@@ -41,44 +41,59 @@
     return _WVEC[key]
 
 
-def _maps_forward(v, label20, acc, N):
-    dev = v.cam_low.device
-    S, h, w = v.S, v.h, v.w
-    npix = S * S
-    v.st_cam = _f32(N * 21, 6, dev=dev)
-    v.st_rv = _f32(N * 21, 6, dev=dev)
-    L.up_plane_stats(v.cam_low, v.st_cam, N * 21, h, w, S)
-    L.up_plane_stats(v.rvd, v.st_rv, N * 21, h, w, S, label20)
-    v.bias = _f32(N * 21, dev=dev)
-    L.cls_loss(v.st_cam, label20, acc[0:1], v.bias, N, npix, 0.5)
-    v.q = _f32(N, npix, dev=dev)
-    v.argc = torch.empty(N, npix, device=dev, dtype=torch.uint8)
-    L.up_rvmin_values(v.rvd, label20, v.q, v.argc, N, h, w, S)
-    v.k_min = npix // 4
-    v.res_min = _f32(N, 4, dev=dev)
-    ws = torch.empty(L.select_workspace_bytes(N), device=dev, dtype=torch.uint8)
-    L.select_kth(v.q, N, npix, v.k_min, False, False, True, v.res_min, ws)
-    L.select_finish(v.res_min, N, v.k_min, True, 0.5 / (v.k_min * N), acc[1:2])
-    v.c = _f32(N, 21, 128, 128, dev=dev)
-    v.r = _f32(N, 21, 128, 128, dev=dev)
-    L.up_norm_resize_forward(v.cam_low, v.st_cam, label20, v.c, N, h, w, S, 128)
-    L.up_norm_resize_forward(v.rvd, v.st_rv, label20, v.r, N, h, w, S, 128)
-
-
-def _maps_backward_cam(v, label20, N):
-    dev = v.cam_low.device
-    S, h, w = v.S, v.h, v.w
-    wy, wx = _adjoint_ones(h, S, dev), _adjoint_ones(w, S, dev)
-    v.d_cam_low = _f32(N, 21, h, w, dev=dev)
-    L.up_maps_backward(v.Gc, v.cam_low, v.st_cam, label20, v.bias, wy, wx, None, None, None, 0, 0.0, v.d_cam_low, N, h, w, S, 128)
-
-
-def _maps_backward_rv(v, label20, N):
-    dev = v.cam_low.device
-    S, h, w = v.S, v.h, v.w
-    v.d_rvd = _f32(N, 21, h, w, dev=dev)
-    L.up_maps_backward(v.Gr, v.rvd, v.st_rv, label20, None, None, None, v.q, v.argc, v.res_min, v.k_min, 0.5 / (v.k_min * N),
-                       v.d_rvd, N, h, w, S, 128)
+def _maps_alloc(views, N, dev):
+    v1, v2 = views
+    st = _f32(4, N * 21, 6, dev=dev)
+    bias = _f32(2, N * 21, dev=dev)
+    npx = [v.S * v.S for v in views]
+    res_min = _f32(2 * N, 4, dev=dev)
+    cr = _f32(4, N, 21, 128, 128, dev=dev)
+    pad = lambda n: (n + 63) & ~63
+    npx_p = [pad(N * n) for n in npx]
+    low = [pad(N * 21 * v.h * v.w) for v in views]
+    q = _f32(sum(npx_p), dev=dev)
+    argc = torch.empty(sum(npx_p), device=dev, dtype=torch.uint8)
+    d_low = _f32(2 * sum(low), dev=dev)
+    for vi, v in enumerate(views):
+        v.st_cam, v.st_rv, v.bias = st[vi], st[2 + vi], bias[vi]
+        o = sum(npx_p[:vi])
+        v.q, v.argc = q[o:o + N * npx[vi]].view(N, npx[vi]), argc[o:o + N * npx[vi]].view(N, npx[vi])
+        v.k_min = npx[vi] // 4
+        v.res_min = res_min[vi * N:(vi + 1) * N]
+        v.c, v.r = cr[vi], cr[2 + vi]
+        o, n = sum(low[:vi]), N * 21 * v.h * v.w
+        v.d_cam_low = d_low[o:o + n].view(N, 21, v.h, v.w)
+        v.d_rvd = d_low[sum(low) + o:sum(low) + o + n].view(N, 21, v.h, v.w)
+    return res_min, d_low
+
+
+def _geom(v, N):
+    return dict(N=N, h=v.h, w=v.w, S=v.S, OS=128)
+
+
+def _maps_forward(views, label20, acc, N, res_min):
+    dev = label20.device
+    cam = [dict(_geom(v, N), low=v.cam_low, stats=v.st_cam, label20=label20) for v in views]
+    rv = [dict(_geom(v, N), low=v.rvd, stats=v.st_rv, label20=label20) for v in views]
+    L.up_plane_stats_multi([dict(j, label20=None) for j in cam] + rv)
+    L.cls_loss_multi([dict(N=N, S=v.S, stats=v.st_cam, label20=label20, loss_out=acc[0:1], out=v.bias, coef=0.5) for v in views])
+    L.up_rvmin_values_multi([dict(j, out=v.q, argc=v.argc) for j, v in zip(rv, views)])
+    groups = [dict(vals=v.q, rows=N, n=v.S * v.S, k=v.k_min, scale=0.5 / (v.k_min * N)) for v in views]
+    ws = torch.empty(L.select_workspace_bytes(2 * N), device=dev, dtype=torch.uint8)
+    L.select_kth_multi(groups, False, False, True, res_min, ws)
+    L.select_finish_multi(groups, res_min, True, acc[1:2])
+    L.up_norm_resize_forward_multi([dict(j, out=v.c) for j, v in zip(cam, views)] + [dict(j, out=v.r) for j, v in zip(rv, views)])
+
+
+def _maps_backward_cam(views, label20, N):
+    dev = label20.device
+    L.up_maps_backward_multi([dict(_geom(v, N), G=v.Gc, low=v.cam_low, stats=v.st_cam, label20=label20, plane_bias=v.bias,
+                                   wvec_y=_adjoint_ones(v.h, v.S, dev), wvec_x=_adjoint_ones(v.w, v.S, dev), out=v.d_cam_low) for v in views])
+
+
+def _maps_backward_rv(views, label20, N):
+    L.up_maps_backward_multi([dict(_geom(v, N), G=v.Gr, low=v.rvd, stats=v.st_rv, label20=label20, q=v.q, argc=v.argc, res=v.res_min,
+                                   k=v.k_min, coef=0.5 / (v.k_min * N), out=v.d_rvd) for v in views])
 
 
 _CAND_K = 256 // 8
@@ -148,8 +163,6 @@
     acc = torch.zeros(8, device=dev, dtype=torch.float32)
     main = torch.cuda.current_stream(dev)
     side = (eng.stream("side0", dev), eng.stream("side1", dev))
-    outs, ctx = eng.run_forward([img1, img2], save=True, lowres=True, prefix=prefix)
-    fork = main.record_event()
     pst = None
     if lookahead is not None:
         pst = eng.stream("prefix", dev)
@@ -157,7 +170,10 @@
         n2 = torch.empty(n1.shape[0], n1.shape[1], img2.shape[-2], img2.shape[-1], device=dev, dtype=torch.float32)
         rows, ch = eng.prefix_out_shape([n1, n2])
         t_next = torch.empty(rows, ch, device=dev, dtype=L.TORCH_DTYPE[DT_OF[model.precision]])
-        pst.wait_event(fork)
+    outs, ctx = eng.run_forward([img1, img2], save=True, lowres=True, prefix=prefix)
+    fork = main.record_event()
+    if lookahead is not None:
+        pst.wait_event(ctx["backbone_done"])
         with torch.cuda.stream(pst):
             L.resize_planar_fwd(n1, n2, n1.shape[0] * n1.shape[1], n1.shape[2], n1.shape[3], n2.shape[2], n2.shape[3], True)
             lookahead["img2"], lookahead["prefix"] = n2, eng.run_prefix([n1, n2], out=t_next)
@@ -176,10 +192,12 @@
         views.append(v)
     v1, v2 = views
     cand = _f32(2, _CAND_L, dev=dev)
-    for vi, v in enumerate(views):
-        side[vi].wait_event(fork)
-        with torch.cuda.stream(side[vi]):
-            _maps_forward(v, label20, acc, N)
+    res_min, d_low = _maps_alloc(views, N, dev)
+    est = side[0]
+    est.wait_event(fork)
+    with torch.cuda.stream(est):
+        d_low.zero_()
+        _maps_forward(views, label20, acc, N, res_min)
     for vi, v in enumerate(views):
         _candidates(v, label20, bg_threshold, tie_idx, N, cand[vi])
     gathered = cand
@@ -190,28 +208,21 @@
         _merge_prototypes(v, gathered, vi, world)
     npix = 128 * 128
     er_coef = 1.0 / (N * 20 * npix)
-    est = side[0]
-    est.wait_stream(side[1])
+    Gc = _f32(2, N, 21, 128, 128, dev=dev)
+    v1.Gc, v2.Gc = Gc[0], Gc[1]
+    dlt = _f32(2 * N, 21 * npix, dev=dev)
+    res = _f32(2 * N, 4, dev=dev)
+    Gr = _f32(2 * N, 21, 128, 128, dev=dev)
+    v1.Gr, v2.Gr = Gr[:N], Gr[N:]
     with torch.cuda.stream(est):
-        for v in views:
-            v.Gc = _f32(N, 21, 128, 128, dev=dev)
-        dlt = _f32(2 * N, 21 * npix, dev=dev)
         L.er_ecr_prep(v1.c, v2.c, v1.r, v2.r, v1.Gc, v2.Gc, dlt[:N], dlt[N:], acc[2:3], N, npix, er_coef)
         prep_done = est.record_event()
         K_ecr = int(21 * npix * 0.2)
         ws = torch.empty(L.select_workspace_bytes(2 * N), device=dev, dtype=torch.uint8)
-        res = _f32(2 * N, 4, dev=dev)
         L.select_kth(dlt, 2 * N, 21 * npix, K_ecr, True, True, False, res, ws)
         L.select_finish(res, 2 * N, K_ecr, False, 1.0 / (N * K_ecr), acc[3:4])
-        Gr = _f32(2 * N, 21, 128, 128, dev=dev)
         L.ecr_backward(dlt, res, Gr, 2 * N, 21 * npix, K_ecr, 1.0 / (N * K_ecr))
-        v1.Gr, v2.Gr = Gr[:N], Gr[N:]
-        ecr_done = est.record_event()
-        _maps_backward_rv(v1, label20, N)
-    side[1].wait_event(prep_done)
-    with torch.cuda.stream(side[1]):
-        _maps_backward_cam(v1, label20, N)
-        _maps_backward_cam(v2, label20, N)
+        _maps_backward_rv(views, label20, N)
     global_intra = distributed or not rng_parity
     rank = dist.get_rank() if distributed else 0
     nce_x3 = model.precision != "fp32"
@@ -238,8 +249,8 @@
     with torch.cuda.stream(side[1]):
         weights_of(1, v2)
         w2_done = side[1].record_event()
-        side[1].wait_event(ecr_done)
-        _maps_backward_rv(v2, label20, N)
+        side[1].wait_event(prep_done)
+        _maps_backward_cam(views, label20, N)
     main.wait_event(w2_done)
     for v in views:
         v.dF = _f32(P, 128, dev=dev)
```

Result: no change. 472.7 images/sec (median of 6 runs) (+0.4%).
